# LitLeo/3m-asr-inference

Hardware: AMD Instinct MI355X
Metric: encoder frames/sec, 18Lx32e Conformer-MoE, 206-frame utterance (higher is better)
Workload: dtype f32; 1 GPU; 18-layer 32-expert fp32 (v_mfma_f32_16x16x4_f32), batch=1x206 frames per GPU, all experts local (BASELINE.json configs[1]); layers=18, experts=32, frames=206, batch_per_gpu=1, parallelism=replicas x1, streams_per_gpu=4, hip_graph=True, kernels_per_forward=263, fold_pos_proj=True, routing=balanced, route_mode=staged, packed_rows=False, fork_embed=auto

## Files before the change

3m-asr-inference_amd/csrc/api.hip:

```cpp
#include <string.h>

#include <vector>

#include "../../include/m3asr.h"
#include "common.h"
#include "kernels.h"

namespace m3 {

static thread_local char g_err[512] = "";

void set_error(const char* fmt, ...) {
  va_list ap;
  va_start(ap, fmt);
  vsnprintf(g_err, sizeof(g_err), fmt, ap);
  va_end(ap);
}
const char* last_error() { return g_err; }

struct MoeWorkspace {
  int32_t* mapping;
  int32_t* acc;
  int32_t* pos;
  float* slab;
  size_t bytes;
};
MoeWorkspace carve_moe_workspace(void* base, int S, int E, int D, int F) {
  MoeWorkspace w;
  size_t off = 0;
  char* p = (char*)base;
  w.mapping = (int32_t*)(p + off); off += align_up((size_t)S * 4, 256);
  w.acc = (int32_t*)(p + off);     off += align_up((size_t)(E + 1) * 4, 256);
  w.pos = (int32_t*)(p + off);     off += align_up((size_t)S * 4, 256);
  w.slab = (float*)(p + off);      off += align_up(expert_ffn_slab_bytes(S, D, F), 256);
  w.bytes = off;
  return w;
}

int moe_expert_ffn_dt(const float* x, const int32_t* gate_idx, const float* w1, const float* b1, const float* w2,
                      const float* b2, int S, int E, int D, int F, const float* gate_value, const float* resid,
                      float alpha, const float* ln_gamma, const float* ln_beta, float ln_eps, float* y, void* ws,
                      size_t ws_bytes, hipStream_t stream, ExpertWeights weights, const float* s1 = nullptr, const float* s2 = nullptr, float h_scale = 0.f, const void* xq = nullptr,
                      const float* xq_scale = nullptr, int ldx = 0) {
  M3_REQUIRE(S >= 0 && E > 0 && D > 0 && F > 0, "fmoe_expert: bad sizes S=%d E=%d D=%d F=%d", S, E, D, F);
  if (S == 0) return 0;
  MoeWorkspace w = carve_moe_workspace(ws, S, E, D, F);
  M3_REQUIRE(ws != nullptr && ws_bytes >= w.bytes, "fmoe_expert: workspace %zu bytes < required %zu", ws_bytes,
             w.bytes);
  int rc = launch_moe_index(gate_idx, S, E, w.mapping, w.acc, w.pos, stream);
  if (rc) return rc;
  const ExpertFfnPlan plan = plan_expert_ffn(weights, S, E, D, F);
  ExpertFfnArgs a{};
  a.x = x; a.ldx = ldx > 0 ? ldx : D; a.pos = w.pos; a.acc_hist = w.acc; a.w1 = w1; a.w2 = w2; a.s1 = s1; a.s2 = s2; a.b1 = b1;
  a.h_scale = h_scale; a.slab = w.slab; a.xq = xq; a.xq_scale = xq_scale;
  rc = launch_expert_ffn(plan, S, E, D, F, a, stream);
  if (rc) return rc;
  return launch_moe_combine(plan.rows(w.slab), plan.slices, w.mapping, gate_idx, gate_value, b2, resid, alpha, ln_gamma, ln_beta, ln_eps,
                            y, S, D, stream);
}

int moe_expert_ffn(const float* x, const int32_t* gate_idx, const float* w1, const float* b1, const float* w2,
                   const float* b2, int S, int E, int D, int F, const float* gate_value, const float* resid,
                   float alpha, const float* ln_gamma, const float* ln_beta, float ln_eps, float* y, void* ws,
                   size_t ws_bytes, hipStream_t stream) {
  return moe_expert_ffn_dt(x, gate_idx, w1, b1, w2, b2, S, E, D, F, gate_value, resid, alpha, ln_gamma, ln_beta, ln_eps,
                           y, ws, ws_bytes, stream, ExpertWeights::F32);
}

}

using namespace m3;

static bool aligned16(const void* p) { return (reinterpret_cast<uintptr_t>(p) & 15) == 0; }

extern "C" {

int m3_abi_version(void) { return M3ASR_ABI_VERSION; }
const char* m3_last_error(void) { return m3::last_error(); }

int m3_moe_scatter_mapping(const int32_t* gate_idx, int S, int num_expert, int32_t* mapping, int32_t* acc_histogram,
                           int32_t* pos, m3_stream stream) {
  M3_REQUIRE(gate_idx && mapping && acc_histogram, "moe_scatter_mapping: null pointer");
  return launch_moe_index(gate_idx, S, num_expert, mapping, acc_histogram, pos, (hipStream_t)stream);
}
int m3_moe_local_scatter(const void* x, const int32_t* mapping, int S, int row_bytes, void* out, m3_stream stream) {
  return launch_local_scatter(x, mapping, S, row_bytes, out, (hipStream_t)stream);
}
int m3_moe_local_gather(const void* buf, const int32_t* mapping, int S, int row_bytes, void* out, m3_stream stream) {
  return launch_local_gather(buf, mapping, S, row_bytes, out, (hipStream_t)stream);
}
int m3_moe_expert_slice(void) { return kExpertSlice; }
size_t m3_moe_expert_workspace_size(int S, int num_expert, int idim, int hidden_units) {
  if (S <= 0 || hidden_units % kExpertSlice) return 0;
  return carve_moe_workspace(nullptr, S, num_expert, idim, hidden_units).bytes;
}
int m3_moe_expert_ffn(const float* x, const int32_t* gate_idx, const float* w1, const float* b1, const float* w2,
                      const float* b2, int S, int num_expert, int idim, int hidden_units, const float* gate_value,
                      const float* resid, float alpha, const float* ln_gamma, const float* ln_beta, float ln_eps,
                      float* y, void* workspace, size_t workspace_bytes, m3_stream stream) {
  return moe_expert_ffn(x, gate_idx, w1, b1, w2, b2, S, num_expert, idim, hidden_units, gate_value, resid, alpha,
                        ln_gamma, ln_beta, ln_eps, y, workspace, workspace_bytes, (hipStream_t)stream);
}
int m3_moe_expert_ffn_bf16(const float* x, const int32_t* gate_idx, const void* w1, const float* b1, const void* w2,
                           const float* b2, int S, int num_expert, int idim, int hidden_units, const float* gate_value,
                           const float* resid, float alpha, const float* ln_gamma, const float* ln_beta, float ln_eps,
                           float* y, void* workspace, size_t workspace_bytes, m3_stream stream) {
  return moe_expert_ffn_dt(x, gate_idx, (const float*)w1, b1, (const float*)w2, b2, S, num_expert, idim, hidden_units,
                           gate_value, resid, alpha, ln_gamma, ln_beta, ln_eps, y, workspace, workspace_bytes,
                           (hipStream_t)stream, ExpertWeights::BF16);
}
int m3_moe_expert_ffn_fp8(const float* x, const int32_t* gate_idx, const void* w1, const float* w1_scale, const float* b1,
                          const void* w2, const float* w2_scale, const float* b2, int S, int num_expert, int idim,
                          int hidden_units, const float* gate_value, const float* resid, float alpha,
                          const float* ln_gamma, const float* ln_beta, float ln_eps, float* y, void* workspace,
                          size_t workspace_bytes, m3_stream stream) {
  M3_REQUIRE(w1_scale && w2_scale, "fmoe_expert fp8: null scale");
  return moe_expert_ffn_dt(x, gate_idx, (const float*)w1, b1, (const float*)w2, b2, S, num_expert, idim, hidden_units,
                           gate_value, resid, alpha, ln_gamma, ln_beta, ln_eps, y, workspace, workspace_bytes,
                           (hipStream_t)stream, ExpertWeights::FP8, w1_scale, w2_scale);
}
int m3_moe_expert_ffn_mxfp4_ldx(const float* x, int ldx, const int32_t* gate_idx, const void* w1, const void* w1_scale, const float* b1,
                                const void* w2, const void* w2_scale, const float* b2, int S, int num_expert, int idim,
                                int hidden_units, const float* gate_value, const float* resid, float alpha,
                                const float* ln_gamma, const float* ln_beta, float ln_eps, float* y, void* workspace,
                                size_t workspace_bytes, m3_stream stream) {
  M3_REQUIRE(x && gate_idx && w1 && w2 && b1 && y, "fmoe_expert mxfp4: null pointer");
  M3_REQUIRE(w1_scale && w2_scale, "fmoe_expert mxfp4: null scale");
  M3_REQUIRE(idim > 0 && idim % 128 == 0 && hidden_units > 0 && hidden_units % 64 == 0,
             "fmoe_expert mxfp4: idim=%d must be a multiple of 128 and hidden_units=%d of 64", idim, hidden_units);
  M3_REQUIRE(ldx >= idim && (ldx & 3) == 0, "fmoe_expert mxfp4: ldx=%d must be a multiple of 4 and at least idim=%d", ldx, idim);
  M3_REQUIRE(aligned16(x) && aligned16(w1) && aligned16(w2), "fmoe_expert mxfp4: x / w1 / w2 must be 16-byte aligned");
  return moe_expert_ffn_dt(x, gate_idx, (const float*)w1, b1, (const float*)w2, b2, S, num_expert, idim, hidden_units,
                           gate_value, resid, alpha, ln_gamma, ln_beta, ln_eps, y, workspace, workspace_bytes,
                           (hipStream_t)stream, ExpertWeights::MXFP4, (const float*)w1_scale, (const float*)w2_scale, 0.f, nullptr,
// ... 193 lines not shown
    M3_REQUIRE(!rows || d->ldy >= n_out, "linear: ldy=%d is shorter than an output row of %d", d->ldy, n_out);
    if (p.y_bf16) M3_REQUIRE(d->ldy % 4 == 0, "linear: ldy=%d must be a multiple of 4 for a bf16 y", d->ldy);
    if (d->resid) M3_REQUIRE(!rows || d->ldr >= n_out, "linear: ldr=%d is shorter than an output row of %d", d->ldr, n_out);
    if (d->y_copy_bf16) M3_REQUIRE(d->ld_copy % 4 == 0 && (!rows || d->ld_copy >= n_out), "linear: ld_copy=%d must be a multiple of 4 and >= %d", d->ld_copy, n_out);
  }
  *out = p;
  return 0;
}
static int linear_pointers(const m3_linear_desc* d) {
  M3_REQUIRE(d->a && d->w && d->y, "linear: null a / w / y");
  M3_REQUIRE(aligned16(d->a) && aligned16(d->a2) && aligned16(d->y) && aligned16(d->resid) && aligned16(d->y_copy_bf16),
             "linear: a / a2 / y / resid / y_copy_bf16 must be 16-byte aligned");
  M3_REQUIRE((const void*)d->resid != (const void*)d->y || d->ldr == d->ldy, "linear: y == resid (in-place) needs ldr=%d == ldy=%d", d->ldr, d->ldy);
  return 0;
}
const char* m3_linear_kernel(const m3_linear_desc* d, int with_workspace) {
  GemmParams p;
  if (linear_params(d, &p)) return nullptr;
  const GemmPlan plan = plan_gemm(p, with_workspace ? SIZE_MAX : 0);
  if (plan.launches == 0) set_error("%s", plan.reason);
  return plan.launches ? plan.label : nullptr;
}
int m3_linear(const m3_linear_desc* d, m3_stream stream) { return m3_linear_ws(d, nullptr, 0, stream); }
size_t m3_linear_workspace_size(const m3_linear_desc* d) {
  GemmParams p;
  return linear_params(d, &p) == 0 ? plan_gemm(p, SIZE_MAX).ws_bytes : 0;
}
int m3_linear_ws(const m3_linear_desc* d, void* workspace, size_t workspace_bytes, m3_stream stream) {
  GemmParams p;
  if (int rc = linear_params(d, &p)) return rc;
  if (int rc = linear_pointers(d)) return rc;
  return launch_gemm(gemm_launch(p, (float*)workspace, workspace_bytes), (hipStream_t)stream);
}

int m3_layer_norm(const float* x, const float* gamma, const float* beta, float eps, float* y, int rows, int dim,
                  m3_stream stream) {
  return launch_layernorm(x, gamma, beta, eps, y, rows, dim, (hipStream_t)stream);
}
int m3_relpos_attention(const float* qkv, int ldq, const float* p, int ldp, const float* pos_u, const float* pos_v,
                        const int32_t* len, int B, int T, int H, int dk, float scale, float* out, int ldo,
                        m3_stream stream) {
  return attention_single(qkv, ldq, p, ldp, pos_u, pos_v, len, B, T, H, dk, scale, 0, -1, out, ldo, 0, stream);
}
int m3_relpos_attention_bf16(const void* qkv, int ldq, const float* p, int ldp, const float* pos_u, const float* pos_v,
                             const int32_t* len, int B, int T, int H, int dk, float scale, int chunk, int left_chunks,
                             void* out, int ldo, m3_stream stream) {
  return attention_single(qkv, ldq, p, ldp, pos_u, pos_v, len, B, T, H, dk, scale, chunk, left_chunks, out, ldo, 1, stream);
}
int m3_relpos_attention_chunk(const float* qkv, int ldq, const float* p, int ldp, const float* pos_u, const float* pos_v,
                              const int32_t* len, int B, int T, int H, int dk, float scale, int chunk, int left_chunks,
                              float* out, int ldo, m3_stream stream) {
  return attention_single(qkv, ldq, p, ldp, pos_u, pos_v, len, B, T, H, dk, scale, chunk, left_chunks, out, ldo, 0, stream);
}
static int dwconv_args_from_desc(const m3_dwconv_desc* d, const char* who, const char* zname, int pair, bool strict, DwArgs* q) {
  if (pair >= 0) M3_REQUIRE(d->B > 0 && d->T > 0 && d->D > 0 && d->K > 0, "%s: empty problem %d", who, pair);
  const bool ln_ok = strict ? (d->gamma == nullptr) == (d->beta == nullptr) : (d->gamma == nullptr || d->beta != nullptr);
  M3_REQUIRE((pair < 0 && (d->B <= 0 || d->T <= 0)) || (d->z && d->w_kc && d->bias && d->out && ln_ok),
             "%s: null %s / w_kc / bias / out, or gamma without beta", who, zname);
  M3_REQUIRE(!strict || (aligned16(d->z) && aligned16(d->w_kc) && aligned16(d->bias) && aligned16(d->gamma) && aligned16(d->beta) &&
                          aligned16(d->left_fill) && aligned16(d->out)), "%s: every operand must be 16-byte aligned", who);
  if (pair >= 0) {
    M3_REQUIRE(d->ldz >= 0 && (d->ldz > 0 || !d->gate_sigmoided), "%s: ldz=%d (sigmoided gate columns belong to the GLU-on-load form)", who, d->ldz);
    M3_REQUIRE(d->left_fill == nullptr || d->K >= 2, "%s: the causal conv needs K >= 2", who);
  }
  q->z = d->z; q->glu_ldz = d->ldz; q->glu_sig = d->gate_sigmoided != 0; q->w_kc = d->w_kc; q->bias = d->bias; q->gamma = d->gamma;
  q->beta = d->beta; q->eps = d->eps; q->causal_left_fill = d->left_fill; q->B = d->B; q->T = d->T; q->D = d->D; q->K = d->K; q->out = d->out;
// ... 170 lines not shown
    M3_REQUIRE(plans[i]->launches > 0, "%s", plans[i]->reason);
    M3_REQUIRE(plans[i]->kernel == GemmKernel::SplitKF32, "%s: problem %d is no split-K problem with its workspace (it runs %s)", who, i, plans[i]->label);
  }
  M3_REQUIRE(pa.conv == pb.conv, "%s: an implicit conv pairs with an implicit conv, a plain problem with a plain one", who);
  return 0;
}
static int splitk_pair_launch(const char* who, const GemmLaunch& a, const void* out_a, size_t out_bytes_a, const GemmLaunch& b, const void* out_b,
                              size_t out_bytes_b, int which, m3_stream stream) {
  M3_REQUIRE(which >= 1 && which <= 3, "%s: which=%d (1 the GEMM launch, 2 the reduce launch, 3 both)", who, which);
  if (int rc = splitk_pair_plans(who, a.plan, b.plan)) return rc;
  M3_REQUIRE(!ranges_overlap(a.ws, a.plan.ws_bytes, b.ws, b.plan.ws_bytes), "%s: each problem needs its own workspace", who);
  M3_REQUIRE(!ranges_overlap(out_a, out_bytes_a, out_b, out_bytes_b), "%s: the two outputs overlap", who);
  return launch_gemm_f32_splitk_dual(a, b, (hipStream_t)stream, which);
}
const char* m3_linear_pair_kernel(const m3_linear_desc* a, const m3_linear_desc* b, int with_workspace) {
  GemmParams pa, pb;
  if (linear_params(a, &pa) || linear_params(b, &pb)) return nullptr;
  const size_t ws = with_workspace ? SIZE_MAX : 0;
  const GemmLaunch qa{pa, plan_gemm(pa, ws)}, qb{pb, plan_gemm(pb, ws)};
  if (with_workspace) return splitk_pair_plans("linear pair (workspaces)", qa.plan, qb.plan) ? nullptr : "gemm_f32_splitk_dual_kernel";
  return linear_pair_plans(qa, qb) ? nullptr : "gemm_f32_dual_kernel";
}
int m3_linear_pair(const m3_linear_desc* a, const m3_linear_desc* b, m3_stream stream) {
  GemmParams pa, pb;
  if (int rc = linear_params(a, &pa)) return rc;
  if (int rc = linear_params(b, &pb)) return rc;
  if (int rc = linear_pointers(a)) return rc;
  if (int rc = linear_pointers(b)) return rc;
  const GemmLaunch qa = gemm_launch(pa, nullptr, 0), qb = gemm_launch(pb, nullptr, 0);
  if (int rc = linear_pair_plans(qa, qb)) return rc;
  M3_REQUIRE(!ranges_overlap(a->y, linear_out_bytes(a), b->y, linear_out_bytes(b)), "linear pair: the two outputs overlap");
  return launch_gemm_f32_dual(qa, qb, (hipStream_t)stream);
}
int m3_linear_ws_pair(const m3_linear_desc* a, void* workspace_a, size_t bytes_a, const m3_linear_desc* b, void* workspace_b,
                      size_t bytes_b, int which, m3_stream stream) {
  GemmParams pa, pb;
  if (int rc = linear_params(a, &pa)) return rc;
  if (int rc = linear_params(b, &pb)) return rc;
  if (int rc = linear_pointers(a)) return rc;
  if (int rc = linear_pointers(b)) return rc;
  return splitk_pair_launch("linear pair (workspaces)", gemm_launch(pa, (float*)workspace_a, bytes_a), a->y, linear_out_bytes(a),
                            gemm_launch(pb, (float*)workspace_b, bytes_b), b->y, linear_out_bytes(b), which, stream);
}
int m3_conv2d_3x3s2_ws_pair(const m3_conv2d_desc* a, void* workspace_a, size_t bytes_a, const m3_conv2d_desc* b, void* workspace_b,
                            size_t bytes_b, int which, m3_stream stream) {
  M3_REQUIRE(a != nullptr && b != nullptr, "conv2d pair: null descriptor");
  GemmParams pa, pb;
  if (int rc = conv2d_params(a->in, a->w, a->bias, a->B, a->T1, a->F1, a->C, a->act, a->out, &pa)) return rc;
  if (int rc = conv2d_params(b->in, b->w, b->bias, b->B, b->T1, b->F1, b->C, b->act, b->out, &pb)) return rc;
  M3_REQUIRE(a->in && a->w && a->out && b->in && b->w && b->out, "conv2d pair: null in / w / out");
  return splitk_pair_launch("conv2d pair", gemm_launch(pa, (float*)workspace_a, bytes_a), a->out, rows_bytes(pa.M, pa.ldy, pa.N),
                            gemm_launch(pb, (float*)workspace_b, bytes_b), b->out, rows_bytes(pb.M, pb.ldy, pb.N), which, stream);
}
int m3_relpos_attention_pair(const m3_attention_desc* a, const m3_attention_desc* b, m3_stream stream) {
  M3_REQUIRE(a != nullptr && b != nullptr, "attention pair: null descriptor");
  AttArgs qa, qb;
  if (int rc = attention_args_from_desc(a, "attention pair", 0, &qa)) return rc;
  if (int rc = attention_args_from_desc(b, "attention pair", 1, &qb)) return rc;
  M3_REQUIRE(relpos_attention_dual_fusable(qa, qb),
             "attention pair: head widths %d / %d (64 or 128 each) or row strides ldq %d / %d, ldp %d / %d (multiples of 4) are not a paired instantiation",
             a->dk, b->dk, a->ldq, b->ldq, a->ldp, b->ldp);
  M3_REQUIRE(!ranges_overlap(a->out, rows_bytes((long)a->B * a->T, a->ldo, a->H * a->dk), b->out, rows_bytes((long)b->B * b->T, b->ldo, b->H * b->dk)),
             "attention pair: the two outputs overlap");
  return launch_relpos_attention_dual(qa, qb, (hipStream_t)stream);
}
int m3_dwconv_ln_silu_pair(const m3_dwconv_desc* a, const m3_dwconv_desc* b, m3_stream stream) {
// ... 345 lines not shown
```

3m-asr-inference_amd/csrc/engine.hip:

```cpp
#include <assert.h>
#include <math.h>
#include <stdlib.h>
#include <string.h>

#include <functional>
#include <memory>
#include <string>
#include <unordered_map>
#include <variant>
#include <vector>

#include "../../include/m3asr.h"
#include "common.h"
#include "kernels.h"

namespace m3 {
struct MoeWorkspace {
  int32_t* mapping; int32_t* acc; int32_t* pos; float* slab; size_t bytes;
};
MoeWorkspace carve_moe_workspace(void* base, int S, int E, int D, int F);
}

using namespace m3;

namespace {

struct Norm { const float* g = nullptr; const float* b = nullptr; };
struct Lin { const float* w = nullptr; const float* b = nullptr; const float* wsum = nullptr; const float* wbeta = nullptr; };

struct BlockW {
  Norm n_ffm, n_mha, n_conv, n_ff, n_final, n_cnn;
  Lin mac1, mac2, qkv, pos, out, pw1, pw2, ff1, ff2;
  const float* pos_u = nullptr; const float* pos_v = nullptr;
  const float* dw_w = nullptr; const float* dw_b = nullptr;
  const float* left_fill = nullptr;
  Lin router;
  Lin router_x;
  const float *ew1 = nullptr, *eb1 = nullptr, *ew2 = nullptr, *eb2 = nullptr;
  const float *es1 = nullptr, *es2 = nullptr;
  float h_scale = 0.f;
};

struct SubW { const float* c1w; const float* c1b; const float* c2w; const float* c2b; Lin out; int in_ch = 1; };

using Launch = std::variant<std::monostate, GemmLaunch, Conv1Args, DwArgs, AttArgs>;

struct Stage {
  std::string name;
  std::function<int(hipStream_t)> run;
  m3_stage_info info;
  bool reads_embed = false;
  Launch launch;
  bool pairable = false;
  bool router_prefix = false;
  std::function<int(hipStream_t)> refresh_prefix;
};
const GemmLaunch& gemm_of(const Stage& st) { return std::get<GemmLaunch>(st.launch); }
bool is_splitk(const Stage& st) { return std::holds_alternative<GemmLaunch>(st.launch) && gemm_of(st).plan.kernel == GemmKernel::SplitKF32; }

m3_stage_info stage_info(const char* kernel, int launches, double bytes, double flops, bool per_row = true) {
  m3_stage_info i;
  i.kernel = kernel; i.launches = launches; i.per_row = per_row ? 1 : 0; i.alg_bytes = bytes; i.flops = flops;
  return i;
}

struct Buf { void* ptr; size_t bytes; };

struct BindKey {
  int B = 0, T = 0;
  const float* feat = nullptr; const int32_t* feat_len = nullptr; float* logits = nullptr;
  void* ws = nullptr; size_t ws_bytes = 0;
// ... 36 lines not shown
    std::shared_ptr<float> pfold;
    std::vector<Stage> stages;
    std::unordered_map<std::string, Buf> buffers;
    int n_kernels = 0;
    hipGraphExec_t graph_exec = nullptr;
    bool graph_valid = false;
    uint64_t last_use = 0;
    bool matches(const BindKey& k) const { return !stages.empty() && key == k; }
  };
  Bound cur;
  std::vector<Bound> parked;
  uint64_t use_clock = 0;
  int n_captures = 0;
  int ep_capacity = 0;
  hipStream_t side = nullptr;
  hipEvent_t ev_fork = nullptr, ev_join = nullptr;
  std::unordered_map<int, std::weak_ptr<float>> pfold_by_tp;
};

namespace {

struct Switches {
  int gate_index_max_rows;
  bool self_route;
  bool hfuse;
  int router_min_rows;
  bool router_xq;
  bool router_skip_xn;
  bool fused8_adapt;
  bool glu_defer;
  bool front_pair;
  bool router_prefix;
  bool glu_sig_epi;
};
const Switches& switches() {
  static const Switches sw = [] {
    auto num = [](const char* name, int dflt) { const char* v = getenv(name); return v ? atoi(v) : dflt; };
    Switches w;
    w.gate_index_max_rows = num("M3_GATE_INDEX_MAX_ROWS", 512);
    w.self_route = num("M3_SELF_ROUTE", 1) != 0;
    w.hfuse = num("M3_HFUSE", 1) != 0;
    w.router_min_rows = num("M3_ROUTER_MIN_ROWS", 2048);
    w.router_xq = num("M3_ROUTER_XQ", 1) != 0;
    w.router_skip_xn = num("M3_ROUTER_SKIP_XN", 0) != 0;
    w.fused8_adapt = num("M3_FUSED8_ADAPT", 0) != 0;
    w.glu_defer = num("M3_GLU_DEFER", 1) != 0;
    w.front_pair = num("M3_FRONT_PAIR", 1) != 0;
    w.router_prefix = num("M3_ROUTER_PREFIX", 1) != 0;
    w.glu_sig_epi = num("M3_GLU_SIG_EPI", 1) != 0;
    return w;
  }();
  return sw;
}

bool lookup(const m3_engine* e, const std::string& name, int64_t numel, const float** out, int dtype = M3_F32) {
  auto it = e->table.find(name);
  if (it == e->table.end()) {
    set_error("engine: weight '%s' missing from the plan", name.c_str());
    return false;
  }
  if (numel >= 0 && it->second.numel != numel) {
    set_error("engine: weight '%s' has %lld elements, expected %lld", name.c_str(), (long long)it->second.numel,
              (long long)numel);
    return false;
  }
  if (it->second.dtype != dtype) {
    set_error("engine: weight '%s' has dtype %d, the engine (weight_dtype=%d) expects %d", name.c_str(),
              (int)it->second.dtype, (int)e->cfg.weight_dtype, dtype);
    return false;
  }
  *out = (const float*)it->second.data;
  return true;
}

#define GET(dst, name, numel) \
  do { if (!lookup(e, (name), (numel), &(dst))) return false; } while (0)
#define GETW(dst, name, numel) \
  do { if (!lookup(e, (name), (numel), &(dst), e->cfg.weight_dtype == M3_F32 ? M3_F32 : M3_BF16)) return false; } while (0)
#define GETE(dst, name, numel) \
  do { if (!lookup(e, (name), (numel), &(dst), e->cfg.weight_dtype)) return false; } while (0)

bool load_norm(const m3_engine* e, const std::string& p, int d, Norm* n) {
  GET(n->g, p + "weight", d);
  GET(n->b, p + "bias", d);
  return true;
}
bool load_lin(const m3_engine* e, const std::string& p, int64_t n_out, int64_t n_in, bool bias, Lin* l) {
  GETW(l->w, p + "weight", n_out * n_in);
  if (bias) GET(l->b, p + "bias", n_out);
  return true;
}
bool load_lin_ln(const m3_engine* e, const std::string& p, int64_t n_out, int64_t n_in, bool wbeta, Lin* l,
                 bool fp32_only = false) {
  if (fp32_only) {
    GET(l->w, p + "ln.weight", n_out * n_in);
  } else {
    GETW(l->w, p + "ln.weight", n_out * n_in);
  }
  GET(l->b, p + "ln.bias", n_out);
  GET(l->wsum, p + "ln.wsum", n_out);
  if (wbeta) GET(l->wbeta, p + "ln.wbeta", n_out);
  return true;
}

bool load_block(const m3_engine* e, const std::string& p, int D, int F, int K, bool cnn_ln, bool moe, int De, BlockW* b, bool causal) {
  const m3_engine_config& c = e->cfg;
  if (!load_norm(e, p + "norm_final.", D, &b->n_final)) return false;
  if (moe && !load_norm(e, p + "norm_ff.", D, &b->n_ff)) return false;
  if (!load_lin_ln(e, p + "feed_forward_macaron.w_1.", F, D, false, &b->mac1) ||
      !load_lin(e, p + "feed_forward_macaron.w_2.", D, F, true, &b->mac2) ||
      !load_lin_ln(e, p + "self_attn.qkv.", 3 * D, D, false, &b->qkv) ||
      !load_lin(e, p + "self_attn.linear_out.", D, D, true, &b->out) ||
      !load_lin_ln(e, p + "conv_module.pointwise_conv1.", 2 * D, D, true, &b->pw1) ||
      !load_lin(e, p + "conv_module.pointwise_conv2.", D, D, true, &b->pw2))
    return false;
  GET(b->pos_u, p + "self_attn.pos_bias_u", D);
  GET(b->pos_v, p + "self_attn.pos_bias_v", D);
  GET(b->dw_w, p + "conv_module.depthwise_conv.weight_kc", (int64_t)K * D);
  GET(b->dw_b, p + "conv_module.depthwise_conv.bias", D);
  if (cnn_ln && !load_norm(e, p + "conv_module.norm.", D, &b->n_cnn)) return false;
  if (causal) GET(b->left_fill, p + "conv_module.left_fill", D);
  if (!moe) {
    if (!load_lin_ln(e, p + "feed_forward.w_1.", F, D, false, &b->ff1) ||
        !load_lin(e, p + "feed_forward.w_2.", D, F, true, &b->ff2))
      return false;
  } else {
    const int world = c.ep_world_size > 0 ? c.ep_world_size : 1;
    const int64_t Etot = (int64_t)c.num_experts * world;
    GET(b->router.w, p + "feed_forward.router_weights_t", Etot * (D + De));
    if (c.router_with_bias) GET(b->router.b, p + "feed_forward.router_bias", Etot);
    if (c.fuse_route && !load_lin_ln(e, p + "feed_forward.router_x.", Etot, D, false, &b->router_x, true)) return false;
    const int64_t E = c.num_experts;
    const int64_t ew_numel = c.weight_dtype == M3_MXFP4 ? E * F * D / 2 : E * F * D;
    GETE(b->ew1, p + "feed_forward.experts.w_1.weight", ew_numel);
    if (c.weight_dtype == M3_MXFP4) {
      GETE(b->es1, p + "feed_forward.experts.w_1.scale", E * F * D / 32);
      GETE(b->es2, p + "feed_forward.experts.w_2.scale", E * F * D / 32);
    }
    if (c.weight_dtype == M3_FP8) {
      GET(b->es1, p + "feed_forward.experts.w_1.scale", E * F);
      GET(b->es2, p + "feed_forward.experts.w_2.scale", E * D);
      if (c.fp8_activations) {
        const float* hs = nullptr;
        GET(hs, p + "feed_forward.experts.h_scale", 1);
        if (hipMemcpy(&b->h_scale, hs, sizeof(float), hipMemcpyDeviceToHost) != hipSuccess || !(b->h_scale > 0.f)) {
          set_error("engine: '%sfeed_forward.experts.h_scale' must hold one positive number", p.c_str());
          return false;
        }
      }
    }
    GET(b->eb1, p + "feed_forward.experts.w_1.bias", E * F);
    GETE(b->ew2, p + "feed_forward.experts.w_2.weight_sliced", ew_numel);
    GET(b->eb2, p + "feed_forward.experts.w_2.bias", E * D);
  }
  return true;
}

inline int sub_fc(int idim, int in_ch) { return idim / in_ch; }
inline int sub_f1(int fc) { return (fc - 3) / 2 + 1; }
inline int sub_f2(int fc) { return (sub_f1(fc) - 3) / 2 + 1; }

bool load_sub(const m3_engine* e, const std::string& p, int D, int idim, SubW* s) {
  auto it = e->table.find(p + "conv.0.weight_9c");
  const int64_t numel = it == e->table.end() ? 9 * (int64_t)D : it->second.numel;
  s->in_ch = (int)(numel / (9 * (int64_t)D));
  if (numel % (9 * (int64_t)D) || s->in_ch < 1 || s->in_ch > 3) {
    set_error("engine: '%sconv.0.weight_9c' has %lld elements: 9 * in_ch * %d with 1 to 3 input channels expected", p.c_str(), (long long)numel, D);
    return false;
  }
  if (idim % s->in_ch || sub_fc(idim, s->in_ch) < 7) {
    set_error("engine: '%sconv.0.weight_9c' has %d input channels: input_dim=%d must be a multiple of it with at least 7 bins per channel",
              p.c_str(), s->in_ch, idim);
    return false;
  }
  const int F2 = sub_f2(sub_fc(idim, s->in_ch));
  GET(s->c1w, p + "conv.0.weight_9c", 9 * (int64_t)s->in_ch * D);
  GET(s->c1b, p + "conv.0.bias", D);
  GETW(s->c2w, p + "conv.2.weight_ohwi", 9 * (int64_t)D * D);
  GET(s->c2b, p + "conv.2.bias", D);
  return load_lin(e, p + "out.0.", D, (int64_t)D * F2, true, &s->out);
}
#undef GET
#undef GETW
#undef GETE

inline int sub_len(int t) { return ((t - 3) / 2 + 1 - 3) / 2 + 1; }
// ... 265 lines not shown
  const float *tail_ln_g = nullptr, *tail_ln_b = nullptr; float tail_ln_eps = 0.f; float* tail_ln_out = nullptr;
  float* splitk_ws = nullptr; size_t splitk_bytes = 0;
};

}

static void add_stage(StageBuilder& sb, const std::string& name, int kernels, std::function<int(hipStream_t)> fn,
                      m3_stage_info info = stage_info("", 0, 0.0, 0.0)) {
  info.launches = kernels;
  sb.bd.stages.push_back(Stage{name, std::move(fn), info});
  sb.bd.n_kernels += kernels;
}

static m3_stage_info gemm_info(const GemmParams& p, const GemmPlan& plan) {
  const bool glu = p.act == ACT_GLU;
  const double M = p.M, N = p.N, K = p.K, Nout = glu ? N / 2 : N;
  const double wsz = p.w_bf16 ? 2 : 4, asz = p.a_bf16 ? 2 : 4, ysz = p.y_bf16 ? 2 : 4;
  double a_bytes = M * K * asz;
  if (p.mode == GEMM_A_CONV3X3S2)
    a_bytes = (double)(p.M / (p.conv_T2 * p.conv_F2)) * p.conv_T1 * p.conv_F1 * p.conv_C * asz;
  double bytes = N * K * wsz + a_bytes + M * Nout * ysz;
  if (p.resid) bytes += M * Nout * 4;
  if (p.Yb) bytes += M * Nout * 2;
  if (p.ln_out) bytes += M * (K - p.K1) * 4;
  return stage_info(plan.label, 1, bytes, 2.0 * M * N * K, p.mode != GEMM_A_CONV3X3S2);
}

static void add_launch(StageBuilder& sb, const std::string& name, Launch record, const m3_stage_info& info, bool pairable = false) {
  add_stage(sb, name, info.launches, nullptr, info);
  sb.bd.stages.back().launch = std::move(record);
  sb.bd.stages.back().pairable = pairable;
}

static void add_gemm(StageBuilder& sb, const std::string& name, GemmParams p, bool fp32_weights = false) {
  p.w_bf16 = (!fp32_weights && sb.eng.cfg.weight_dtype != M3_F32) ? 1 : 0;
  const GemmLaunch g = gemm_launch(p, sb.splitk_ws, sb.splitk_bytes);
  m3_stage_info info = gemm_info(p, g.plan);
  info.launches = g.plan.launches ? g.plan.launches : 1;
  add_launch(sb, name, g, info, g.plan.launches == 1);
}

static bool stages_fusable(const Stage& a, const Stage& b) {
  if (!a.pairable || !b.pairable || a.launch.index() != b.launch.index()) return false;
  if (std::holds_alternative<GemmLaunch>(a.launch))
    return is_splitk(a) ? gemm_splitk_dual_fusable(gemm_of(a), gemm_of(b)) : gemm_dual_fusable(gemm_of(a), gemm_of(b));
  if (auto* d = std::get_if<DwArgs>(&a.launch)) return dwconv_dual_fusable(*d, std::get<DwArgs>(b.launch));
  if (auto* t = std::get_if<AttArgs>(&a.launch)) return relpos_attention_dual_fusable(*t, std::get<AttArgs>(b.launch));
  return conv1_dual_fusable(std::get<Conv1Args>(a.launch), std::get<Conv1Args>(b.launch));
}
static Stage fused_stage(const Stage& a, const Stage& b, bool reduce_half = false) {
  Stage d;
  d.name = reduce_half ? a.name + ".reduce+" + b.name + ".reduce" : a.name + "+" + b.name;
  const char* label = "";
  std::visit([&](const auto& pa) {
    using R = std::decay_t<decltype(pa)>;
    if constexpr (std::is_same_v<R, GemmLaunch>) {
      const GemmLaunch& pb = gemm_of(b);
      if (is_splitk(a)) {
        d.run = [pa, pb, which = reduce_half ? 2 : 1](hipStream_t s) { return launch_gemm_f32_splitk_dual(pa, pb, s, which); };
        label = "gemm_f32_splitk_dual_kernel";
      } else {
        d.run = [pa, pb](hipStream_t s) { return launch_gemm_f32_dual(pa, pb, s); };
        label = "gemm_f32_dual_kernel";
      }
    } else if constexpr (std::is_same_v<R, Conv1Args>) {
      d.run = [pa, pb = std::get<R>(b.launch)](hipStream_t s) { return launch_conv1_relu_dual(pa, pb, s); };
      label = "conv1_relu_dual_kernel";
    } else if constexpr (std::is_same_v<R, DwArgs>) {
      d.run = [pa, pb = std::get<R>(b.launch)](hipStream_t s) { return launch_dwconv_ln_silu_dual(pa, pb, s); };
// ... 154 lines not shown
      const GemmPlan plan = gemm_of(st).plan;
      float* prefix = pl.rprefix; const int layer = m.layer;
      st.refresh_prefix = [plan, g, prefix, layer](hipStream_t s) {
        const float* wt[kRouterPrefixMaxLayers] = {};
        wt[layer] = g.W;
        return launch_router_embed_prefix(plan, g, wt, layer, 1, prefix, s);
      };
    }
  }
  sb.bd.stages.back().reads_embed = true;
}

static void add_moe_gate_index(StageBuilder& sb, const MoeLayer& m, int32_t* map, int32_t* acc, int32_t* pos) {
  add_stage(sb, m.pfx + "moe_gate_index", 1, [=](hipStream_t s) {
    return launch_moe_gate_index(m.rl, m.Etot, m.live_len, m.live_rpb, m.S, m.gidx, m.gval, map, acc, pos, s);
  }, stage_info("moe_index_kernel", 1, (double)m.S * (m.Etot * 4 + 16) + 4.0 * (m.Etot + 1), 0.0));
}

static void add_moe_top1(StageBuilder& sb, const MoeLayer& m) {
  add_stage(sb, m.pfx + "moe_top1", 1, [m](hipStream_t s) {
    return launch_softmax_top1(m.rl, m.Etot, m.live_len, m.live_rpb, m.S, m.Etot, m.gidx, m.gval, s);
  }, stage_info("softmax_top1_kernel", 1, (double)m.S * (m.Etot * 4 + 8), 0.0));
}

static void add_moe_local_index(StageBuilder& sb, const MoeLayer& m) {
  add_stage(sb, m.pfx + "moe_local.index", 1, [m](hipStream_t s) {
    return launch_moe_index(m.gidx, m.S, m.E, m.mw.mapping, m.mw.acc, m.mw.pos, s);
  }, stage_info("moe_index_kernel", 1, 12.0 * m.S + 4.0 * (m.E + 1), 0.0));
}

static ExpertFfnArgs expert_args(const BlockW& w, const float* x, const MoeWorkspace& mw, int D) {
  ExpertFfnArgs a{};
  a.x = x; a.ldx = D; a.pos = mw.pos; a.acc_hist = mw.acc; a.w1 = w.ew1; a.w2 = w.ew2; a.s1 = w.es1; a.s2 = w.es2; a.b1 = w.eb1;
  a.w2_sliced = 1; a.h_scale = w.h_scale; a.slab = mw.slab;
  return a;
}

static void add_moe_local_expert(StageBuilder& sb, const MoeLayer& m, const MoeRoute& r, const ExpertFfnPlan& f, const Plan& pl) {
  const bool norm = r.norm_in_expert();
  const float* xin = norm ? m.x : m.xn;
  const bool self_route = r.gate == GateForm::InExpert;
  const void* xq = r.use_xq ? pl.xq : nullptr; const float* xqs = r.use_xq ? pl.xq_scale : nullptr;
  int32_t* fs = r.fs_dev ? pl.moe_fs : nullptr;
  add_stage(sb, m.pfx + "moe_local.expert", f.launches, [=](hipStream_t s) {
    const BlockW& w = *m.w;
    const float* ln_g = norm ? w.n_ff.g : nullptr; const float* ln_b = norm ? w.n_ff.b : nullptr; const float ln_eps = norm ? m.eps : 0.f;
    if (self_route)
      return launch_expert_route_ffn_f32(xin, m.D, m.rl, m.live_len, m.live_rpb, m.S, m.E, m.D, m.F, w.ew1, w.eb1, w.ew2, 1, w.eb2,
                                         m.mw.slab, m.gidx, m.gval, m.mw.mapping, m.mw.acc, m.mw.pos, s, ln_g, ln_b, ln_eps);
    ExpertFfnArgs a = expert_args(w, xin, m.mw, m.D);
    a.ln_gamma = ln_g; a.ln_beta = ln_b; a.ln_eps = ln_eps; a.xq = xq; a.xq_scale = xqs; a.fs_dev = fs;
    return launch_expert_ffn(f, m.S, m.E, m.D, m.F, a, s);
  }, stage_info(f.label, 1, -1.0, 4.0 * m.D * m.F * m.S));
}

static void add_moe_local_combine(StageBuilder& sb, const MoeLayer& m, const MoeRoute& r, const ExpertFfnPlan& f, const Plan& pl) {
  const bool self_route = r.gate == GateForm::InExpert;
  const int32_t* cmap = self_route ? nullptr : m.mw.mapping;
  const float* cb2 = self_route ? nullptr : m.w->eb2;
  const int32_t* fs = r.fs_dev ? pl.moe_fs : nullptr;
  const double S = m.S, D = m.D;
  add_stage(sb, m.pfx + "moe_local.combine", 1, [=](hipStream_t s) {
    const BlockW& w = *m.w;
    return launch_moe_combine(f.rows(m.mw.slab), fs ? kExpertFusedFp8MaxSplit : f.slices, cmap, m.gidx, m.gv, cb2, m.x, 0.5f, w.n_final.g, w.n_final.b, m.eps, m.x,
                              m.S, m.D, s, m.xb_out, m.xstats_out, fs);
  }, stage_info("moe_combine_kernel", 1, S * D * 4 * (f.slices + 2) + (m.xb_out ? 2.0 * S * D : 0.0), S * D * (f.slices + 10)));
}

static void add_moe_ep(StageBuilder& sb, const MoeLayer& m, const MoeRoute& r, const Plan& pl) {
  const int S = m.S, E = m.E, Etot = m.Etot, D = m.D, F = m.F, world = m.world;
  const int cap = pl.ep_cap, R = pl.ep_rows;
  int32_t *g_acc = pl.ep_acc, *g_map = pl.ep_mapping, *g_pos = pl.ep_pos, *map_send = pl.ep_map_send, *gate_recv = pl.ep_gate_recv;
  int32_t* ep_overflow = pl.ep_overflow;
  float *wire_a = pl.wire_a, *wire_b = pl.wire_b;
  const MoeWorkspace rw = carve_moe_workspace(m.ws, R, E, D, F);
  if (r.gate == GateForm::GateIndex) add_moe_gate_index(sb, m, g_map, g_acc, g_pos);
  if (r.gate == GateForm::Top1Index) add_moe_top1(sb, m);
  const bool one_launch = r.gate == GateForm::GateIndex;
  const int32_t* gidx = m.gidx; const float* xn = m.xn;
  add_stage(sb, m.pfx + "moe_ep.send", one_launch ? 1 : 2, [=](hipStream_t s) {
    if (!one_launch)
      if (int rc = launch_moe_index(gidx, S, Etot, g_map, g_acc, g_pos, s)) return rc;
    return launch_ep_send_rows(gidx, g_map, g_acc, S, world, E, cap, map_send, xn, wire_a, D * 4, s, ep_overflow);
  }, stage_info("ep_send_rows_kernel", 1, (double)S * D * 8 + 24.0 * S, 0.0));
  auto exchange = [=, &sb](const char* name) {
    if (world == 1) add_stage(sb, m.pfx + name, 0, [=](hipStream_t s) {
      M3_CHECK_HIP(hipMemcpyAsync(wire_b, wire_a, (size_t)R * D * 4, hipMemcpyDeviceToDevice, s));
      return 0;
    });
  };
  exchange("moe_ep.exchange1");
  const ExpertFfnPlan f = plan_expert_ffn(expert_weights(sb.eng.cfg, *m.w), R, E, D, F, EXPERT_SCATTER_ROWS);
  const bool scatter2 = f.kernel == ExpertKernel::TiledBf16;
  const BlockW* wp = m.w;
  add_stage(sb, m.pfx + "moe_ep.expert", (scatter2 ? 2 : 3) + f.launches, [=](hipStream_t s) {
    const BlockW& w = *wp;
    if (int rc = launch_ep_recv_gate(wire_b, world, E, cap, D * 4, gate_recv, s)) return rc;
    if (int rc = launch_moe_index(gate_recv, R, E, rw.mapping, rw.acc, rw.pos, s)) return rc;
    ExpertFfnArgs a = expert_args(w, wire_b, rw, D);
    if (scatter2) { a.b2 = w.eb2; a.y_scatter = wire_a; }
    if (int rc = launch_expert_ffn(f, R, E, D, F, a, s)) return rc;
    if (scatter2) return 0;
    return launch_moe_combine(f.rows(rw.slab), f.slices, rw.mapping, gate_recv, nullptr, w.eb2, nullptr, 1.f, nullptr, nullptr, 0.f, wire_a, R, D, s);
  }, stage_info(f.label, 1, -1.0, 4.0 * D * F * S));
  exchange("moe_ep.exchange2");
  add_stage(sb, m.pfx + "moe_ep.combine", 1, [=](hipStream_t s) {
    const BlockW& w = *wp;
    return launch_moe_combine(wire_b, 1, map_send, nullptr, m.gv, nullptr, m.x, 0.5f, w.n_final.g, w.n_final.b, m.eps, m.x, S, D, s,
                              m.xb_out, m.xstats_out);
  }, stage_info("moe_combine_kernel", 1, (double)S * D * 12 + (m.xb_out ? 2.0 * S * D : 0.0), (double)S * D * 11));
  sb.bd.buffers["ep.wire_a"] = Buf{wire_a, (size_t)R * D * 4};
  sb.bd.buffers["ep.wire_b"] = Buf{wire_b, (size_t)R * D * 4};
}

static void build_block(StageBuilder& sb, const std::string& pfx, const BlockW& w, int D, int F, int H, int K, bool cnn_ln,
                        bool moe, int layer, int tap_index, const Plan& pl, bool causal) {
  auto add_gemm = [&](StageBuilder&, const std::string& name, GemmParams g, bool fp32_weights = false) {
    if (sb.bd.packed) g.m_dev = pl.row0 + sb.bd.key.B;
    ::add_gemm(sb, name, g, fp32_weights);
  };
  const m3_engine_config& c = sb.eng.cfg;
  const BindKey& key = sb.bd.key;
  const int B = key.B, Tp = sb.bd.Tp, S = sb.bd.S;
  const bool streaming = key.sstate != nullptr;
  const int32_t* step = key.s_slots ? sb.st.slot_pos : sb.st.step;
  const int slot_chunks = key.s_slots ? key.s_maxf / Tp : -1;
  float* x = pl.x;
  const int32_t* lens = pl.lens;
  const float eps = 1e-12f;

  const bool a16 = sb.bd.a16;
  void* xb = pl.xb;
  const bool dma = sb.bd.dma;
  float* xstats = pl.xstats;
  auto from_xb = [&](GemmParams& g) {
    if (a16) { g.A = (const float*)xb; g.a_bf16 = 1; }
    if (dma) { g.ln_stats = xstats; g.ln_stat_parts = kXbStatParts; }
  };
  auto also_xb = [&](GemmParams& g) {
    if (a16) { g.Yb = xb; g.ldyb = D; }
    if (dma) g.Yb_stats = xstats;
  };
  const bool packed = sb.bd.packed;
  const int32_t* row0 = packed ? pl.row0 : nullptr;
  const int32_t* pad_of = packed ? pl.pad_of : nullptr;
  const int32_t* pdev = packed ? pl.row0 + B : nullptr;
  const int32_t* live_len = packed ? pdev : lens;
  const int live_rpb = packed ? S : Tp;
  {
    GemmParams g;
    g.A = x; g.lda = D; g.W = w.mac1.w; g.bias = w.mac1.b; g.Y = pl.h1; g.ldy = F; g.M = S; g.N = F; g.K = D;
    g.ln_wsum = w.mac1.wsum; g.ln_eps = eps; g.act = ACT_SILU;
    from_xb(g); g.y_bf16 = a16;
    add_gemm(sb, pfx + "ffn_macaron.w1", g);
    GemmParams h;
    h.A = pl.h1; h.lda = F; h.W = w.mac2.w; h.bias = w.mac2.b; h.Y = x; h.ldy = D; h.M = S; h.N = D; h.K = F;
    h.alpha = 0.5f; h.resid = x; h.ldr = D;
    h.a_bf16 = a16; also_xb(h);
    add_gemm(sb, pfx + "ffn_macaron.w2", h);
  }
  {
    GemmParams g;
    g.A = x; g.lda = D; g.W = w.qkv.w; g.bias = w.qkv.b; g.Y = pl.qkv; g.ldy = 3 * D; g.M = S; g.N = 3 * D; g.K = D;
    g.ln_wsum = w.qkv.wsum; g.ln_eps = eps;
    from_xb(g);
    const bool att16 = a16 && relpos_attention_bf16_supports(Tp, D / H);
    g.y_bf16 = att16;
    add_gemm(sb, pfx + "att.qkv", g);
    const int ldp = (c.num_blocks + c.embed_blocks) * D;
    const float* pmat = pl.pbuf + (size_t)tap_index * D;
    const float* qkv = pl.qkv; float* ctx = pl.ctx;
    const float* pu = w.pos_u; const float* pv = w.pos_v;
    const int dk = D / H;
    const float scale = 1.f / sqrtf((float)dk);
    const int chunk = c.static_chunk_size, left_chunks = c.num_left_chunks;
    AttArgs aa;
    aa.qkv = qkv; aa.ldq = 3 * D; aa.pmat = pmat; aa.ldp = ldp; aa.pos_u = pu; aa.pos_v = pv; aa.row_len = lens; aa.B = B; aa.T = Tp; aa.H = H;
    aa.dk = dk; aa.scale = scale; aa.out = ctx; aa.ldo = D; aa.left_chunks = left_chunks;
    const char* label = att16 ? "relpos_attention_bf16_kernel" : "relpos_attention_kernel";
    double row_bytes = att16 ? 8 : (12 + (a16 ? 2 : 4));
    if (streaming) {
      aa.streaming = 1; aa.hist = sb.st.kv[tap_index]; aa.cap = key.s_hist; aa.step = step; aa.slot_max_chunks = slot_chunks;
      label = "relpos_attention_stream_kernel"; row_bytes = 24;
    } else {
      aa.rows_bf16 = att16; aa.out_bf16 = a16; aa.row0 = row0; aa.chunk = chunk;
    }
    add_launch(sb, pfx + "att.core", aa, stage_info(label, 1, (double)S * D * row_bytes + (double)Tp * D * 4, 6.0 * Tp * D * S), !streaming && !att16);
    GemmParams o;
    o.A = pl.ctx; o.lda = D; o.W = w.out.w; o.bias = w.out.b; o.Y = x; o.ldy = D; o.M = S; o.N = D; o.K = D;
    o.resid = x; o.ldr = D;
    o.a_bf16 = a16; also_xb(o);
    add_gemm(sb, pfx + "att.out", o);
  }
  {
    GemmParams g;
    g.A = x; g.lda = D; g.W = w.pw1.w; g.bias = w.pw1.b; g.Y = pl.glu; g.ldy = D; g.M = S; g.N = 2 * D; g.K = D;
    g.ln_wsum = w.pw1.wsum; g.ln_wbeta = w.pw1.wbeta; g.ln_eps = eps; g.act = ACT_GLU;
    g.row_len = live_len; g.rows_per_batch = live_rpb; g.mask_in = 1;
    from_xb(g);
    bool glu_deferred = false;
    if (switches().glu_defer && c.weight_dtype == M3_F32 && !a16 && !causal && !streaming &&
        dwconv_glu_in_supports(D, K, false, 0, 2 * D)) {
      GemmParams r = g;
      r.act = ACT_NONE; r.ldy = 2 * D;
      const GemmPlan rp = plan_gemm(r, 0);
      if (rp.launches == 1 && rp.kernel == GemmKernel::SkinnyF32 && rp.mt == 1) { g = r; glu_deferred = true; }
    }
    const bool glu_sig = glu_deferred && switches().glu_sig_epi && (D & 15) == 0;
    if (glu_sig) g.sig_col0 = D;
    add_gemm(sb, pfx + "conv.pw1_glu", g);
    const float* glu = pl.glu; float* dw = pl.dw;
    const float* dww = w.dw_w; const float* dwb = w.dw_b;
    const float* ng = cnn_ln ? w.n_cnn.g : nullptr; const float* nb = cnn_ln ? w.n_cnn.b : nullptr;
    const float* lfill = causal ? w.left_fill : nullptr;
    DwArgs da;
    da.z = glu; da.w_kc = dww; da.bias = dwb; da.gamma = ng; da.beta = nb; da.eps = 1e-5f; da.B = B; da.T = Tp; da.D = D; da.K = K;
    da.out = dw; da.out_bf16 = a16;
    double row_bytes = (glu_deferred ? 8 : 4) + (a16 ? 2 : 4), cache_bytes = 0.0;
    if (streaming) {
      da.streaming = 1; da.cache_pair = sb.st.conv[tap_index]; da.step = step; da.chunk_len = lens; da.slot_max_chunks = slot_chunks;
      row_bytes = 8; cache_bytes = 8.0 * B * (K - 1) * D;
    } else {
      da.pad_of = pad_of; da.row0 = row0; da.row_len = lens; da.causal_left_fill = lfill;
      da.glu_ldz = glu_deferred ? 2 * D : 0; da.glu_sig = glu_sig;
    }
    add_launch(sb, pfx + "conv.dw_ln_silu", da,
               stage_info("dwconv_ln_silu_kernel", 1, (double)S * D * row_bytes + (double)K * D * 4 + cache_bytes, 2.0 * K * D * S), !streaming);
    GemmParams h;
    h.A = pl.dw; h.lda = D; h.W = w.pw2.w; h.bias = w.pw2.b; h.Y = x; h.ldy = D; h.M = S; h.N = D; h.K = D;
    h.row_len = live_len; h.rows_per_batch = live_rpb; h.mask_out = 1; h.resid = x; h.ldr = D;
    h.a_bf16 = a16; also_xb(h);
    add_gemm(sb, pfx + "conv.pw2", h);
  }
  if (!moe) {
    GemmParams g;
    g.A = x; g.lda = D; g.W = w.ff1.w; g.bias = w.ff1.b; g.Y = pl.h1; g.ldy = F; g.M = S; g.N = F; g.K = D;
    g.ln_wsum = w.ff1.wsum; g.ln_eps = eps; g.act = ACT_SILU;
    from_xb(g); g.y_bf16 = a16;
    add_gemm(sb, pfx + "ffn.w1", g);
    GemmParams h;
    h.A = pl.h1; h.lda = F; h.W = w.ff2.w; h.bias = w.ff2.b; h.Y = x; h.ldy = D; h.M = S; h.N = D; h.K = F;
    h.alpha = 0.5f; h.resid = x; h.ldr = D;
    h.a_bf16 = a16;
    add_gemm(sb, pfx + "ffn.w2", h);
    const float* fg = w.n_final.g; const float* fb = w.n_final.b;
    void* xbo = a16 ? xb : nullptr;
    float* xso = dma ? xstats : nullptr;
    const float* g2 = sb.tail_ln_g; const float* b2 = sb.tail_ln_b; float* y2 = sb.tail_ln_out;
    const float eps2 = sb.tail_ln_eps;
    sb.tail_ln_g = nullptr;
    add_stage(sb, pfx + "norm_final", 1, [=](hipStream_t s) { return launch_layernorm(x, fg, fb, eps, x, S, D, s, xbo, xso, g2, b2, eps2, y2); },
              stage_info("layernorm_kernel", 1, (double)S * D * (a16 ? 10 : 8) + (g2 ? 4.0 * S * D : 0.0), (g2 ? 16.0 : 8.0) * S * D));
  } else {
    MoeLayer m;
    m.pfx = pfx; m.w = &w; m.S = S; m.Tp = Tp; m.D = D; m.F = F; m.De = c.embed_dim; m.E = c.num_experts;
    m.world = c.ep_world_size > 0 ? c.ep_world_size : 1; m.Etot = m.E * m.world; m.eps = eps;
    m.x = x; m.xn = pl.xn; m.rl = pl.rl;
    m.gidx = pl.gate_idx + (size_t)layer * S; m.gval = pl.gate_val + (size_t)layer * S;
    m.gv = c.keep_expert_output ? nullptr : m.gval;
    m.lens = lens; m.live_len = live_len; m.live_rpb = live_rpb; m.pdev = pdev;
    m.eall = pl.eall + (size_t)layer * m.E; m.ld_eall = c.num_blocks * m.E; m.layer = layer;
    m.xb_out = a16 ? xb : nullptr; m.xstats_out = dma ? xstats : nullptr;
    m.ws = (char*)pl.moe_ws + (c.debug_taps ? (size_t)layer * pl.moe_ws_bytes : 0);
    m.mw = carve_moe_workspace(m.ws, S, m.E, D, F);
    const MoeRoute r = choose_moe_route(c, S, w, pl);
    add_moe_router(sb, m, r, pl);
    if (r.ep) {
      add_moe_ep(sb, m, r, pl);
    } else {
      if (r.gate == GateForm::GateIndex) add_moe_gate_index(sb, m, m.mw.mapping, m.mw.acc, m.mw.pos);
      if (r.gate == GateForm::Top1Index) add_moe_top1(sb, m);
      if (r.gate == GateForm::Top1Index || r.gate == GateForm::RouterTail) add_moe_local_index(sb, m);
      const ExpertFfnPlan f = plan_expert_ffn(expert_weights(c, w), S, m.E, D, F, r.norm_in_expert() ? EXPERT_NORM_IN_KERNEL : 0);
      add_moe_local_expert(sb, m, r, f, pl);
      add_moe_local_combine(sb, m, r, f, pl);
    }
    const std::string b = pfx.substr(0, pfx.size() - 1);
// ... 600 lines not shown
```

3m-asr-inference_amd/csrc/gemm.hip:

```cpp
#include "common.h"
#include "gemm_epilogue.h"
#include "kernels.h"

#ifdef M3_GEMM_DIAG
#define M3_GDIAG(...) __VA_ARGS__
#else
#define M3_GDIAG(...)
#endif

namespace m3 {

M3_GDIAG(__device__ unsigned long long g_gemm_dbg[2048 * 8];)

enum { LN_NONE = GEMM_LN_NONE, LN_EPI = GEMM_LN_EPI, LN_PRO = GEMM_LN_PRO };

template <int MT, bool GLU, int NW, bool CONV, int LN, int NBUF, bool ACCI = false>
__device__ __forceinline__ void gemm_f32_body(const GemmParams& p, const int bid) {
  constexpr int NT = GLU ? 2 : 1;
  constexpr int G = gemm_group_steps(MT, NT, NW);
  constexpr int I0 = ACCI ? G / 2 : 0;
  static_assert(!ACCI || (MT == 1 && !GLU && !CONV && NBUF == 1 && G % 2 == 0), "acc_init: the one-group 16-row concat form only");
  constexpr int RW = (16 * MT) / NW;
  static_assert(RW >= 1, "more waves than rows");
  __shared__ float red[NW][MT * NT][256];
  __shared__ float stats[16 * MT][2];
  __shared__ float rsum[LN == LN_EPI ? NW : 1][16 * MT][2];
  __shared__ __attribute__((aligned(16))) float ln_g[LN == LN_PRO ? 1024 : 4], ln_b[LN == LN_PRO ? 1024 : 4];

  M3_GDIAG(unsigned long long dg[8]; dg[0] = __builtin_amdgcn_s_memtime();)
  asm volatile("" ::"s"(p.A), "s"(p.lda), "s"(p.W), "s"(p.bias), "s"(p.Y), "s"(p.ldy), "s"(p.M), "s"(p.N), "s"(p.K), "s"(p.mode),
               "s"(p.n_tiles), "s"(p.m_tiles), "s"(p.xcd_swizzle), "s"(p.m_dev), "s"(p.resid), "s"(p.ldr), "s"(p.act), "s"(p.alpha),
               "s"(p.mask_in), "s"(p.mask_out), "s"(p.row_len), "s"(p.rows_per_batch), "s"(p.sig_col0));
  if (ACCI) asm volatile("" ::"s"(p.acc_init));
  if (LN == LN_EPI) asm volatile("" ::"s"(p.ln_wsum), "s"(p.ln_wbeta), "s"(p.ln_eps));
  if (LN == LN_PRO) asm volatile("" ::"s"(p.ln_gamma), "s"(p.ln_beta), "s"(p.ln_eps), "s"(p.ln_out), "s"(p.ld_ln_out), "s"(p.ln_on_a2));
  if (!CONV) asm volatile("" ::"s"(p.A2), "s"(p.lda2), "s"(p.K1));
  if (CONV) asm volatile("" ::"s"(p.conv_T1), "s"(p.conv_F1), "s"(p.conv_T2), "s"(p.conv_F2), "s"(p.conv_C));
  const int lane = threadIdx.x & 63, wave = threadIdx.x >> 6;
  const int col = lane & 15, kq = lane >> 4;
  const int Nout = GLU ? (p.N >> 1) : p.N;

  int n_tile, m_tile;
  {
    const int id = bid;
    if (p.xcd_swizzle) {
      const int j = id >> 3;
      m_tile = j % p.m_tiles;
      n_tile = (j / p.m_tiles) * 8 + (id & 7);
    } else {
      n_tile = id % p.n_tiles;
      m_tile = id / p.n_tiles;
    }
  }
  const int n0 = n_tile * 16;
  const int m0 = m_tile * (16 * MT);
  if (p.m_dev != nullptr && m0 > *p.m_dev) return;
  const int ln_k0 = p.ln_on_a2 ? p.K1 : 0;
  const int Kl = p.K - ln_k0;

  const float* arow[MT];
  const float* arow2[MT];
#pragma unroll
  for (int mt = 0; mt < MT; ++mt) {
    const int m = min(m0 + 16 * mt + col, p.M - 1);
    arow2[mt] = nullptr;
    if (CONV) {
      const int f2 = m % p.conv_F2;
      const int t2 = (m / p.conv_F2) % p.conv_T2;
      const int b = m / (p.conv_F2 * p.conv_T2);
      arow[mt] = p.A + ((size_t)(b * p.conv_T1 + 2 * t2) * p.conv_F1 + 2 * f2) * p.conv_C + 4 * kq;
    } else {
      arow[mt] = p.A + (size_t)m * p.lda + 4 * kq;
      if (p.mode == GEMM_A_CONCAT2) arow2[mt] = p.A2 + (size_t)m * p.lda2 + 4 * kq;
    }
  }
  const float* wrow[NT];
#pragma unroll
  for (int t = 0; t < NT; ++t)
    wrow[t] = p.W + (size_t)min(n0 + t * Nout + col, p.N - 1) * p.K + 4 * kq;

  f32x4 acc[MT][NT];
#pragma unroll
  for (int mt = 0; mt < MT; ++mt)
#pragma unroll
    for (int t = 0; t < NT; ++t) acc[mt][t] = f32x4{0.f, 0.f, 0.f, 0.f};
  constexpr bool DUAL = MT * NT <= 2;
  f32x4 acc2[MT][NT];
#pragma unroll
  for (int mt = 0; mt < MT; ++mt)
#pragma unroll
    for (int t = 0; t < NT; ++t) acc2[mt][t] = f32x4{0.f, 0.f, 0.f, 0.f};
  float s1[MT], s2[MT];
#pragma unroll
  for (int mt = 0; mt < MT; ++mt) s1[mt] = s2[mt] = 0.f;

  const int nsteps = p.K >> 4;
  auto a_offset = [&](int k) -> int {
    if (CONV) {
      const int seg = k / p.conv_C, c = k - seg * p.conv_C;
      const int kh = seg / 3, kw = seg - kh * 3;
      return (kh * p.conv_F1 + kw) * p.conv_C + c;
    }
    return k;
  };

  f32x4 wbuf[NBUF][G][NT], abuf[NBUF][G][MT];
  auto load_group = [&](int g, int buf) {
#pragma unroll
    for (int i = I0; i < G; ++i) {
      const int s = min(wave + NW * (G * g + i), nsteps - 1);
      const int k = s << 4;
#pragma unroll
      for (int t = 0; t < NT; ++t) wbuf[buf][i][t] = ldg4_w(wrow[t] + k);
      const bool second = ACCI || (!CONV && p.mode == GEMM_A_CONCAT2 && k >= p.K1);
      const int off = second ? (k - p.K1) : a_offset(k);
#pragma unroll
      for (int mt = 0; mt < MT; ++mt) abuf[buf][i][mt] = ldg4((second ? arow2[mt] : arow[mt]) + off);
    }
  };

  const int ngroups = (nsteps + NW * G - 1) / (NW * G);
  M3_GDIAG(dg[1] = __builtin_amdgcn_s_memtime();)
  f32x4 ln_v[16];
  auto load_stat_rows = [&](int c) {
    const int l16 = lane & 15;
    const int rloc = wave * RW + 4 * c + (lane >> 4);
    const int m = min(m0 + min(rloc, 16 * MT - 1), p.M - 1);
    const float* row = (p.ln_on_a2 ? p.A2 : p.A) + (size_t)m * (p.ln_on_a2 ? p.lda2 : p.lda);
#pragma unroll
    for (int j = 0; j < 8; ++j) ln_v[j] = ldg4(row + min(4 * (l16 + 16 * j), Kl - 4));
    if (Kl > 512) {
#pragma unroll
      for (int j = 8; j < 16; ++j) ln_v[j] = ldg4(row + min(4 * (l16 + 16 * j), Kl - 4));
    } else {
#pragma unroll
      for (int j = 8; j < 16; ++j) ln_v[j] = f32x4{0.f, 0.f, 0.f, 0.f};
    }
  };
  if (LN == LN_PRO && ACCI) load_stat_rows(0);
  load_group(0, 0);
  if (ACCI) {
    const float* pre = p.acc_init + ((size_t)((m_tile * p.n_tiles + n_tile) * NW + wave) * 2) * 256 + 4 * lane;
    acc[0][0] = ldg4(pre);
    acc2[0][0] = ldg4(pre + 256);
  }
  M3_GDIAG(dg[2] = __builtin_amdgcn_s_memtime();)
// ... 196 lines not shown
        const int row = 16 * mt + 4 * kq + r;
        const int m = m0 + row;
        if (m >= p.M) continue;
        float y0 = v[0][r], y1 = v[NT - 1][r];
        const bool pad = pad4[r];
        if (LN != LN_EPI && p.mask_in && pad) y0 = y1 = 0.f;
        float mean = 0.f, rstd = 1.f;
        if (LN == LN_EPI) {
          float t1 = 0.f, t2 = 0.f;
#pragma unroll
          for (int w = 0; w < NW; ++w) {
            t1 += rsum[w][row][0];
            t2 += rsum[w][row][1];
          }
          ln_mean_rstd(t1, t2, Kl, p.ln_eps, mean, rstd);
        }
        float y = gemm_epilogue<GLU, LN == LN_EPI>(y0, y1, bias0, bias1, wsum0, wsum1, wbeta0, wbeta1, mean, rstd, pad, res[r], p);
        if (!GLU && p.sig_col0 >= 0 && n0 >= p.sig_col0) y = sigmoidf(y);
        p.Y[(size_t)m * p.ldy + ep_n] = y;
      }
    }
  }
  M3_GDIAG(dg[6] = __builtin_amdgcn_s_memtime();
           asm volatile("s_waitcnt vmcnt(0)" ::: "memory");
           dg[7] = __builtin_amdgcn_s_memtime();
           if (lane == 0 && wave == 0 && bid < 2048) {
             unsigned long long* o = g_gemm_dbg + (size_t)bid * 8;
             for (int i = 0; i < 8; ++i) o[i] = dg[i];
             const unsigned hw = __builtin_amdgcn_s_getreg((31 << 11) | 4), xcc = __builtin_amdgcn_s_getreg((31 << 11) | 20);
             o[7] = (dg[7] & 0xffffffffffull) | ((unsigned long long)(hw & 0xffff) << 40) | ((unsigned long long)(xcc & 0xf) << 56);
           })
}

template <int MT, bool GLU, int NW, bool CONV, int LN, int NBUF, bool ACCI = false>
__global__ __launch_bounds__(64 * NW) void gemm_f32_kernel(const GemmParams p) {
  gemm_f32_body<MT, GLU, NW, CONV, LN, NBUF, ACCI>(p, (int)blockIdx.x);
}

struct RouterPrefixArgs {
  const float* A; int lda; int M, N, K;
  int n_tiles, m_tiles, xcd_swizzle;
  const int32_t* m_dev;
  float* prefix; long layer_floats; int layer0;
  const float* w[kRouterPrefixMaxLayers];
};
template <int NW>
__global__ __launch_bounds__(64 * NW) void router_embed_prefix_kernel(const RouterPrefixArgs a) {
  constexpr int H = gemm_group_steps(1, 1, NW) / 2;
  asm volatile("" ::"s"(a.A), "s"(a.lda), "s"(a.M), "s"(a.N), "s"(a.K), "s"(a.n_tiles), "s"(a.m_tiles), "s"(a.xcd_swizzle), "s"(a.m_dev),
               "s"(a.prefix), "s"(a.layer_floats), "s"(a.layer0));
  const int lane = threadIdx.x & 63, wave = threadIdx.x >> 6;
  const int col = lane & 15, kq = lane >> 4;
  const int layer = a.layer0 + (int)blockIdx.y;
  int n_tile, m_tile;
  {
    const int id = (int)blockIdx.x;
    if (a.xcd_swizzle) {
      const int j = id >> 3;
      m_tile = j % a.m_tiles;
      n_tile = (j / a.m_tiles) * 8 + (id & 7);
    } else {
      n_tile = id % a.n_tiles;
      m_tile = id / a.n_tiles;
    }
  }
  const int n0 = n_tile * 16, m0 = m_tile * 16;
  if (a.m_dev != nullptr && m0 > *a.m_dev) return;
  const float* arow = a.A + (size_t)min(m0 + col, a.M - 1) * a.lda + 4 * kq;
  const float* wrow = a.w[layer] + (size_t)min(n0 + col, a.N - 1) * a.K + 4 * kq;
// ... 5 lines not shown
    ab[i] = ldg4(arow + k);
  }
  f32x4 acc = f32x4{0.f, 0.f, 0.f, 0.f}, acc2 = f32x4{0.f, 0.f, 0.f, 0.f};
#pragma unroll
  for (int i = 0; i < H; ++i)
#pragma unroll
    for (int j = 0; j < 4; j += 2) {
      acc = mfma16(ab[i][j], wb[i][j], acc);
      acc2 = mfma16(ab[i][j + 1], wb[i][j + 1], acc2);
    }
  float* o = a.prefix + (size_t)layer * a.layer_floats + ((size_t)((m_tile * a.n_tiles + n_tile) * NW + wave) * 2) * 256 + 4 * lane;
  stg4(o, acc);
  stg4(o + 256, acc2);
}

size_t router_prefix_floats(const GemmPlan& plan) { return (size_t)plan.m_tiles * plan.n_tiles * plan.nw * 2 * 256; }

int launch_router_embed_prefix(const GemmPlan& plan, const GemmParams& p, const float* const* w, int layer0, int n_layers, float* prefix,
                               hipStream_t stream) {
  M3_REQUIRE(plan.launches == 1 && plan.kernel == GemmKernel::SkinnyF32 && p.acc_init != nullptr && (plan.nw == 4 || plan.nw == 8),
             "router prefix: the consumer's plan does not take an accumulator prefix");
  M3_REQUIRE(layer0 >= 0 && n_layers > 0 && layer0 + n_layers <= kRouterPrefixMaxLayers && prefix != nullptr, "router prefix: bad layer range");
  RouterPrefixArgs a;
  a.A = p.A; a.lda = p.lda; a.M = p.M; a.N = p.N; a.K = p.K;
  a.n_tiles = plan.n_tiles; a.m_tiles = plan.m_tiles; a.xcd_swizzle = plan.xcd_swizzle;
  a.m_dev = p.m_dev; a.prefix = prefix; a.layer_floats = (long)router_prefix_floats(plan); a.layer0 = layer0;
  for (int l = 0; l < kRouterPrefixMaxLayers; ++l) a.w[l] = (l >= layer0 && l < layer0 + n_layers) ? w[l] : nullptr;
  const dim3 grid(plan.n_tiles * plan.m_tiles, n_layers);
  if (plan.nw == 8) hipLaunchKernelGGL((router_embed_prefix_kernel<8>), grid, dim3(512), 0, stream, a);
  else hipLaunchKernelGGL((router_embed_prefix_kernel<4>), grid, dim3(256), 0, stream, a);
  M3_LAUNCH_CHECK();
  return 0;
}
template <int MT, bool GLU, int NW, int LN>
__global__ __launch_bounds__(64 * NW) void gemm_f32_dual_kernel(const GemmParams p0, const GemmParams p1, const int n0) {
  if ((int)blockIdx.x < n0) {
    if ((int)blockIdx.x < p0.n_tiles * p0.m_tiles) gemm_f32_body<MT, GLU, NW, false, LN, 1>(p0, (int)blockIdx.x);
  } else {
    gemm_f32_body<MT, GLU, NW, false, LN, 1>(p1, (int)blockIdx.x - n0);
  }
}

int launch_gemm_f32_dual(const GemmLaunch& a, const GemmLaunch& b, hipStream_t stream) {
  M3_REQUIRE(gemm_dual_fusable(a, b), "gemm dual: the two problems do not share an instantiation");
  GemmParams q[2] = {a.p, b.p};
  const GemmPlan& pa = a.plan;
  const GemmPlan* const plans[2] = {&a.plan, &b.plan};
  for (int i = 0; i < 2; ++i) {
    q[i].n_tiles = plans[i]->n_tiles; q[i].m_tiles = plans[i]->m_tiles; q[i].xcd_swizzle = plans[i]->xcd_swizzle;
  }
  const int n0 = (int)align_up((size_t)q[0].n_tiles * q[0].m_tiles, 8);
  dim3 grid(n0 + q[1].n_tiles * q[1].m_tiles);
#define M3_DUAL(GLU_, NW_, LN_)                                                                                             \
  hipLaunchKernelGGL((gemm_f32_dual_kernel<1, GLU_, NW_, LN_>), grid, dim3(64 * NW_), 0, stream, q[0], q[1], n0)
  if (pa.glu) {
    if (pa.nw == 8) { if (pa.ln == LN_EPI) M3_DUAL(true, 8, LN_EPI); else M3_DUAL(true, 8, LN_NONE); }
    else { if (pa.ln == LN_EPI) M3_DUAL(true, 4, LN_EPI); else M3_DUAL(true, 4, LN_NONE); }
  } else {
    if (pa.nw == 8) { if (pa.ln == LN_EPI) M3_DUAL(false, 8, LN_EPI); else M3_DUAL(false, 8, LN_NONE); }
    else { if (pa.ln == LN_EPI) M3_DUAL(false, 4, LN_EPI); else M3_DUAL(false, 4, LN_NONE); }
  }
#undef M3_DUAL
  M3_LAUNCH_CHECK();
  return 0;
}

int launch_gemm_f32_skinny(const GemmPlan& plan, const GemmParams& pin, hipStream_t stream) {
  GemmParams p = pin;
  p.n_tiles = plan.n_tiles; p.m_tiles = plan.m_tiles; p.xcd_swizzle = plan.xcd_swizzle;
  dim3 grid(p.n_tiles * p.m_tiles);
  const int mt = plan.mt, nw = plan.nw, ln = plan.ln;
  if (p.acc_init != nullptr) {
    if (nw == 8) hipLaunchKernelGGL((gemm_f32_kernel<1, false, 8, false, LN_PRO, 1, true>), grid, dim3(512), 0, stream, p);
    else hipLaunchKernelGGL((gemm_f32_kernel<1, false, 4, false, LN_PRO, 1, true>), grid, dim3(256), 0, stream, p);
    M3_LAUNCH_CHECK();
    return 0;
  }

#define M3_GEMM_LAUNCH(MT_, GLU_, NW_, CONV_, LN_)                                                              \
  do {                                                                                                          \
    if (plan.nbuf == 1)                                                                                         \
      hipLaunchKernelGGL((gemm_f32_kernel<MT_, GLU_, NW_, CONV_, LN_, 1>), grid, dim3(64 * NW_), 0, stream, p); \
    else                                                                                                        \
      hipLaunchKernelGGL((gemm_f32_kernel<MT_, GLU_, NW_, CONV_, LN_, 2>), grid, dim3(64 * NW_), 0, stream, p); \
  } while (0)
#define M3_GEMM_MT(GLU_, NW_, CONV_, LN_)                                                              \
  do {                                                                                                 \
    if (mt == 1) M3_GEMM_LAUNCH(1, GLU_, NW_, CONV_, LN_);                                             \
    else if (mt == 2) M3_GEMM_LAUNCH(2, GLU_, NW_, CONV_, LN_);                                        \
    else M3_GEMM_LAUNCH(4, GLU_, NW_, CONV_, LN_);                                                     \
  } while (0)
#define M3_GEMM_LN(GLU_, NW_)                                                                          \
  do {                                                                                                 \
    if (ln == LN_EPI) M3_GEMM_MT(GLU_, NW_, false, LN_EPI);                                            \
    else if (ln == LN_PRO) M3_GEMM_MT(GLU_, NW_, false, LN_PRO);                                       \
    else M3_GEMM_MT(GLU_, NW_, false, LN_NONE);                                                        \
  } while (0)
  if (plan.conv) {
    if (nw == 16) M3_GEMM_MT(false, 16, true, LN_NONE); else if (nw == 8) M3_GEMM_MT(false, 8, true, LN_NONE);
    else M3_GEMM_MT(false, 4, true, LN_NONE);
  } else if (nw == 16) {
    M3_GEMM_MT(false, 16, false, LN_NONE);
  } else if (plan.glu) {
    if (nw == 8) M3_GEMM_LN(true, 8); else M3_GEMM_LN(true, 4);
  } else {
    if (nw == 8) M3_GEMM_LN(false, 8); else M3_GEMM_LN(false, 4);
  }
#undef M3_GEMM_LN
#undef M3_GEMM_MT
#undef M3_GEMM_LAUNCH
  M3_LAUNCH_CHECK();
  return 0;
}

// ... 8 lines not shown
```

3m-asr-inference_amd/csrc/gemm_plan.hip:

```cpp
#include <stdlib.h>

#include "common.h"
#include "kernels.h"

namespace m3 {

static int env_int(const char* name, int dflt) {
  const char* e = getenv(name);
  return e ? atoi(e) : dflt;
}

#define M3_PLAN_REQUIRE(cond, ...)                                  \
  do {                                                              \
    if (!(cond)) {                                                  \
      snprintf(plan.reason, sizeof(plan.reason), __VA_ARGS__);      \
      return false;                                                 \
    }                                                               \
  } while (0)

static bool operands_ok(const GemmParams& p, const char* who, GemmPlan& plan) {
  const int kmult = p.w_bf16 ? 32 : 16;
  M3_PLAN_REQUIRE(p.grp_acc == nullptr, "%s: grouped (per-expert) operands belong to the expert FFN's plan", who);
  M3_PLAN_REQUIRE(p.M > 0 && p.N > 0 && p.K > 0, "%s: empty problem M=%d N=%d K=%d", who, p.M, p.N, p.K);
  M3_PLAN_REQUIRE(p.K % kmult == 0, "%s: K=%d must be a multiple of %d", who, p.K, kmult);
// ... 99 lines not shown
  if (plan.ln != GEMM_LN_NONE) {
    M3_PLAN_REQUIRE(p.mode == GEMM_A_PLAIN || (concat && p.ln_on_a2), "%s: LayerNorm needs plain A (or the A2 half of a concat)", who);
    M3_PLAN_REQUIRE((p.ln_on_a2 ? p.K - p.K1 : p.K) <= 1024, "%s: LayerNorm supports rows up to 1024 wide", who);
    M3_PLAN_REQUIRE(p.K <= 2047, "%s: LayerNorm variants are built for K < 2048", who);
  }
  M3_PLAN_REQUIRE(!p.ln_on_a2 || concat, "%s: ln_on_a2 needs concat mode", who);
  M3_PLAN_REQUIRE(p.ln_out == nullptr || plan.ln == GEMM_LN_PRO, "%s: ln_out needs the affine LayerNorm prologue", who);
  if (long_batch && (p.K & 63) == 0 && (!conv || (p.conv_C & 63) == 0)) {
    plan.kernel = GemmKernel::TiledF32; plan.label = "gemm_f32_tiled_kernel";
    if (big) tiled_grid(p, plan, 128, 128, 32); else tiled_grid(p, plan, 64, 64, 64);
    return true;
  }
  plan.kernel = GemmKernel::SkinnyF32; plan.label = "gemm_f32_kernel";
  skinny_grid(p, plan, Nout);
  plan.dual_ok = plan.mt == 1 && (plan.nw == 4 || plan.nw == 8) && plan.nbuf == 1 && p.mode == GEMM_A_PLAIN &&
                 plan.ln != GEMM_LN_PRO && p.m_dev == nullptr && p.acc_init == nullptr;
  return true;
}

static bool extras_ok(const GemmParams& p, GemmPlan& plan) {
  if (p.sig_col0 >= 0) {
    M3_PLAN_REQUIRE(plan.kernel == GemmKernel::SkinnyF32 && !plan.glu, "gemm: sig_col0 needs the skinny fp32 kernel with a plain epilogue (M=%d N=%d K=%d)",
                    p.M, p.N, p.K);
    M3_PLAN_REQUIRE((p.sig_col0 & 15) == 0, "gemm: sig_col0=%d must be a multiple of 16", p.sig_col0);
  }
  if (p.acc_init != nullptr) {
    M3_PLAN_REQUIRE(plan.kernel == GemmKernel::SkinnyF32 && plan.mt == 1 && !plan.glu && p.mode == GEMM_A_CONCAT2 && (p.K1 & 15) == 0,
                    "gemm: acc_init needs the skinny fp32 kernel, 16-row tiles, concat operands with K1 %% 16 == 0");
    M3_PLAN_REQUIRE(plan.ln == GEMM_LN_PRO && p.ln_on_a2 && (plan.nw == 4 || plan.nw == 8) && plan.nbuf == 1 && 2 * p.K1 == p.K &&
                    p.K == 16 * plan.nw * gemm_group_steps(1, 1, plan.nw),
                    "gemm: acc_init is built for K1 = K / 2 = %d with the LayerNorm prologue on the A2 half (K1=%d K=%d)",
                    8 * plan.nw * gemm_group_steps(1, 1, plan.nw), p.K1, p.K);
  }
  return true;
}

GemmPlan plan_gemm(const GemmParams& p, size_t workspace_bytes_available) {
  GemmPlan plan{};
  plan.kernel = p.w_bf16 ? GemmKernel::SkinnyBf16 : GemmKernel::SkinnyF32;
  plan.label = "";
  plan.glu = p.act == ACT_GLU; plan.conv = p.mode == GEMM_A_CONV3X3S2;
  plan.ln = p.ln_wsum ? GEMM_LN_EPI : (p.ln_gamma ? GEMM_LN_PRO : GEMM_LN_NONE);
  if (operands_ok(p, p.w_bf16 ? "gemm_bf16w" : "gemm", plan) && choose_form(p, workspace_bytes_available, plan) && extras_ok(p, plan))
    plan.launches = plan.kernel == GemmKernel::SplitKF32 ? 2 : 1;
  return plan;
}

GemmLaunch gemm_launch(const GemmParams& p, float* ws, size_t ws_bytes) { return GemmLaunch{p, plan_gemm(p, ws != nullptr ? ws_bytes : 0), ws}; }
bool gemm_dual_fusable(const GemmLaunch& ga, const GemmLaunch& gb) {
  const GemmPlan &a = ga.plan, &b = gb.plan;
  return a.launches == 1 && b.launches == 1 && a.dual_ok && b.dual_ok && a.nw == b.nw && a.ln == b.ln && a.glu == b.glu;
}

int launch_gemm(const GemmLaunch& g, hipStream_t stream) {
  const GemmPlan& plan = g.plan; const GemmParams& p = g.p; float* const ws = g.ws;
  M3_REQUIRE(plan.launches > 0, "%s", plan.reason);
  switch (plan.kernel) {
    case GemmKernel::SkinnyF32: return launch_gemm_f32_skinny(plan, p, stream);
    case GemmKernel::SkinnyBf16: return launch_gemm_bf16w_skinny(plan, p, stream);
    case GemmKernel::TiledF32: return launch_gemm_f32_tiled(plan, p, stream);
    case GemmKernel::TiledBf16: return launch_gemm_bf16w_tiled(plan, p, stream);
    case GemmKernel::DmaBf16: return launch_gemm_bf16_dma(plan, p, stream);
    case GemmKernel::SplitKF32:
      M3_REQUIRE(ws != nullptr, "gemm split-K: the plan was made for a workspace of %zu bytes, none given", plan.ws_bytes);
      return launch_gemm_f32_splitk(plan, p, ws, stream);
  }
  return -2;
}

}
```

3m-asr-inference_amd/csrc/kernels.h:

```cpp
#pragma once
#include <hip/hip_runtime.h>
#include <stdint.h>

#include "../../include/m3asr.h"

namespace m3 {

enum { ACT_NONE = 0, ACT_RELU = 1, ACT_SILU = 2, ACT_GLU = 3 };
enum { GEMM_A_PLAIN = 0, GEMM_A_CONCAT2 = 1, GEMM_A_CONV3X3S2 = 2 };

struct GemmParams {
  const float* A = nullptr; int lda = 0;
  const float* A2 = nullptr; int lda2 = 0; int K1 = 0;
  const float* W = nullptr;
  int w_bf16 = 0;
  const float* bias = nullptr;
  float* Y = nullptr; int ldy = 0;
  int M = 0, N = 0, K = 0;
  int mode = GEMM_A_PLAIN;
  const float* ln_gamma = nullptr; const float* ln_beta = nullptr; float ln_eps = 0.f;
  const float* ln_wsum = nullptr; const float* ln_wbeta = nullptr;
  int ln_on_a2 = 0;
  float* ln_out = nullptr; int ld_ln_out = 0;
  const int32_t* row_len = nullptr; int rows_per_batch = 0;
  int mask_in = 0, mask_out = 0;
  int conv_T1 = 0, conv_F1 = 0, conv_T2 = 0, conv_F2 = 0, conv_C = 0;
  int act = ACT_NONE;
  float alpha = 1.f;
  const float* resid = nullptr; int ldr = 0;
  const int32_t* grp_acc = nullptr; int grp_E = 0; const int32_t* grp_pos = nullptr; int w_sliced = 0;
  const float* w_scale = nullptr;
  int a_bf16 = 0, y_bf16 = 0; void* Yb = nullptr; int ldyb = 0;
  float* Yb_stats = nullptr; const float* ln_stats = nullptr; int ln_stat_parts = 0;
  const int32_t* m_dev = nullptr;
  const int32_t* y_rows = nullptr;
  const int32_t* conv_len = nullptr;
  int sig_col0 = -1;
  const float* acc_init = nullptr;
  int n_tiles = 0, m_tiles = 0, xcd_swizzle = 0;
};
enum { GEMM_LN_NONE = 0, GEMM_LN_EPI = 1, GEMM_LN_PRO = 2 };
enum class GemmKernel { SkinnyF32, SkinnyBf16, TiledF32, TiledBf16, DmaBf16, SplitKF32 };
struct GemmPlan {
  GemmKernel kernel;
  const char* label;
  int launches;
  bool glu, conv; int ln;
  int mt, nw, nbuf;
  bool dual_ok;
  int bm, bn, bk;
  int stages;
  int m_tiles, n_tiles, xcd_swizzle;
  int splits; size_t ws_bytes;
  char reason[192];
};
GemmPlan plan_gemm(const GemmParams& p, size_t workspace_bytes_available);
struct GemmLaunch { GemmParams p; GemmPlan plan; float* ws = nullptr; };
GemmLaunch gemm_launch(const GemmParams& p, float* ws, size_t ws_bytes);
int launch_gemm(const GemmLaunch& g, hipStream_t stream);
bool gemm_dual_fusable(const GemmLaunch& a, const GemmLaunch& b);
int launch_gemm_f32_dual(const GemmLaunch& a, const GemmLaunch& b, hipStream_t stream);
constexpr int kRouterPrefixMaxLayers = 64;
size_t router_prefix_floats(const GemmPlan& plan);
int launch_router_embed_prefix(const GemmPlan& plan, const GemmParams& p, const float* const* w, int layer0, int n_layers, float* prefix,
                               hipStream_t stream);
constexpr int gemm_group_steps(int MT, int NT, int NW) {
  if (NW == 16) return MT == 1 ? (NT == 1 ? 4 : 2) : (MT == 2 ? 2 : 1);
  if (NW == 8) return MT == 1 ? 8 : (MT == 2 ? (NT == 1 ? 6 : 4) : (NT == 1 ? 3 : 2));
  return MT == 1 ? 8 : (MT == 2 ? 6 : 4);
}
constexpr int gemm16_group_steps(int MT, int NW) { return NW == 16 ? 2 : (MT == 4 ? 2 : 4); }
// ... 27 lines not shown
int launch_moe_router(const float* emb, int lde, int De, const float* x, int ldx, int D, const float* W, const float* bias,
                      const float* gamma, const float* beta, float eps, float* xn, int ldxn, float* Y, int ldy, int M, int N,
                      const int32_t* m_dev, hipStream_t stream, int32_t* gate_idx = nullptr, float* gate_val = nullptr,
                      const int32_t* row_len = nullptr, int rows_per_batch = 0, void* xq = nullptr, float* xq_scale = nullptr);
int launch_local_scatter(const void* x, const int32_t* mapping, int S, int row_bytes, void* out, hipStream_t stream);
int launch_local_gather(const void* buf, const int32_t* mapping, int S, int row_bytes, void* out, hipStream_t stream);

int launch_ep_send_map(const int32_t* gate_idx, const int32_t* mapping, const int32_t* acc_hist, int S, int world, int e_loc,
                       int capacity, int32_t* map_send, void* wire, int row_bytes, hipStream_t stream, int32_t* overflow = nullptr);
int launch_ep_send_rows(const int32_t* gate_idx, const int32_t* mapping, const int32_t* acc_hist, int S, int world, int e_loc,
                        int capacity, int32_t* map_send, const void* x, void* wire, int row_bytes, hipStream_t stream, int32_t* overflow = nullptr);
int launch_ep_recv_gate(const void* wire, int world, int e_loc, int capacity, int row_bytes, int32_t* gate_recv,
                        hipStream_t stream);

#ifndef M3_EXPERT_SLICE
#define M3_EXPERT_SLICE 64
#endif
constexpr int kExpertSliceW16 = 64;
constexpr int kExpertSlice = M3_EXPERT_SLICE;
size_t expert_ffn_slab_bytes(int S, int D, int F);
enum class ExpertWeights { F32, BF16, FP8, FP8A8, MXFP4 };
enum class ExpertKernel { SlabF32, TiledF32, SlabBf16, TiledBf16, G256Bf16, SlabW8, TiledW8, FusedFp8, SlabW4, TiledW4 };
struct ExpertFfnPlan {
  ExpertWeights weights; ExpertKernel kernel;
  const char* label;
  int launches, slices;
  int fsplit;
  size_t h_off, rows_off, xb_off;
  float* rows(float* slab) const { return (float*)((char*)slab + rows_off); }
};
enum { EXPERT_NORM_IN_KERNEL = 1,
       EXPERT_SCATTER_ROWS = 2 };
ExpertFfnPlan plan_expert_ffn(ExpertWeights w, int S, int E, int D, int F, unsigned flags = 0);
struct ExpertFfnArgs { const float* x; int ldx; const int32_t *pos, *acc_hist; const void *w1, *w2; const float *s1, *s2, *b1, *b2;
                       int w2_sliced; float h_scale; float* slab; const float *ln_gamma, *ln_beta; float ln_eps;
                       const void* xq; const float* xq_scale; int32_t* fs_dev; float* y_scatter; };
int launch_expert_ffn(const ExpertFfnPlan& plan, int S, int E, int D, int F, const ExpertFfnArgs& a, hipStream_t stream);
int init_expert_ffn_kernels();
int launch_expert_ffn_f32_slab(const float* x, int ldx, const int32_t* pos, const int32_t* acc_hist, int S, int E,
                               int D, int F, const float* w1, const float* b1, const float* w2, int w2_sliced, float* slab,
                               const float* ln_gamma, const float* ln_beta, float ln_eps, hipStream_t stream);
int init_expert_ffn_f32_tiled_kernels();
int launch_expert_tiled_f32(const float* x, int ldx, const int32_t* pos, const int32_t* acc_hist, int S, int E,
                            int D, int F, const float* w1, const float* b1, const float* w2, int w2_sliced,
                            float* hbuf, float* ybuf, hipStream_t stream);
int init_expert_ffn_bf16_kernels();
int launch_expert_ffn_bf16w_slab(const float* x, int ldx, const int32_t* pos, const int32_t* acc_hist, int S, int E,
                                 int D, int F, const void* w1, const float* b1, const void* w2, int w2_sliced, float* slab,
                                 hipStream_t stream);
int init_expert_ffn_w8_kernels();
int launch_expert_ffn_w8_slab(const float* x, int ldx, const int32_t* pos, const int32_t* acc_hist, int S, int E, int D, int F,
                              const void* w1, const float* s1, const float* b1, const void* w2, const float* s2, int w2_sliced,
                              float* slab, hipStream_t stream);
int init_expert_ffn_w4_kernels();
int launch_expert_ffn_w4_slab(const float* x, int ldx, const int32_t* pos, const int32_t* acc_hist, int S, int E, int D, int F,
                              const void* w1, const void* s1, const float* b1, const void* w2, const void* s2, int w2_sliced,
                              float* slab, hipStream_t stream);
constexpr int kExpertFusedFp8MaxSplit = 4;
int expert_ffn_fused_fp8_fsplit(int S, int E, int D, int F);
int init_expert_ffn_fused_fp8_kernels();
int launch_expert_ffn_fused_fp8(const float* x, int ldx, const int32_t* pos, const int32_t* acc_hist, int S, int E, int D, int F,
                                const void* w1, const float* s1, const float* b1, const void* w2, const float* s2, int w2_sliced,
                                float h_scale, int fsplit, float* ybuf, hipStream_t stream, const void* xq = nullptr,
                                const float* xq_scale = nullptr, int32_t* fs_dev = nullptr);
int launch_quantize_rows_e4m3(const float* x, int ldx, int S, int D, void* xq, float* scale, hipStream_t stream);
int launch_expert_tiled_w16(int w_fp8, const float* x, int ldx, const int32_t* pos, const int32_t* acc_hist, int S, int E,
// ... 317 lines not shown
```

3m-asr-inference_amd/csrc/moe_expert.hip:

```cpp
#include <stdlib.h>

#include "common.h"
#include "kernels.h"
#include "moe_gate.h"

namespace m3 {

struct ExpertRoute {
  const float* logits = nullptr;
  const int32_t* row_len = nullptr; int rows_per_batch = 0;
  int32_t* gate_idx = nullptr; float* gate_value = nullptr;
  int32_t* mapping = nullptr; int32_t* acc_hist = nullptr; int32_t* pos = nullptr;
  const float* b2 = nullptr;
  int wave_route = 0;
};

struct ExpertSwitches {
  bool route_wave;
};
static const ExpertSwitches& expert_switches() {
  static const ExpertSwitches sw = [] {
    auto num = [](const char* name, int dflt) { const char* v = getenv(name); return v ? atoi(v) : dflt; };
    ExpertSwitches w;
    w.route_wave = num("M3_ROUTE_WAVE", 1) != 0;
    return w;
  }();
  return sw;
}

template <int MT, bool LNS, int RE = 0>
__global__ __launch_bounds__(64 * (kExpertSlice / 16)) void expert_ffn_f32_kernel(const float* __restrict__ x, int ldx,
                                                             const int32_t* __restrict__ pos,
                                                             const int32_t* __restrict__ acc_hist, int S, int D,
                                                             int F, const float* __restrict__ w1,
                                                             const float* __restrict__ b1,
                                                             const float* __restrict__ w2, int w2_row_stride,
                                                             int w2_slice_stride, float* __restrict__ slab,
                                                             const float* __restrict__ ln_gamma,
                                                             const float* __restrict__ ln_beta, float ln_eps, ExpertRoute rt) {
  extern __shared__ __attribute__((aligned(16))) float lds[];
  const int e = blockIdx.y, slice = blockIdx.x;
  const int lane = threadIdx.x & 63, wave = threadIdx.x >> 6;
  const int col = lane & 15, kq = lane >> 4;

  const int xs_ld = D + 8;
  constexpr int hs_ld = kExpertSlice + 8;
  constexpr int NWV = kExpertSlice / 16;
  constexpr int KS2 = kExpertSlice / 16;
  constexpr int SPG = 8 / KS2;
  constexpr int NB = 2;
  static_assert(kExpertSlice == 16 || kExpertSlice == 32 || kExpertSlice == 64, "slice must be 16/32/64");
  float* xs = lds;
  float* hs = lds + 16 * MT * xs_ld;
  const int f0 = slice * kExpertSlice;
  const int ksteps1 = D >> 4;

  const float* w1row = w1 + ((size_t)e * F + f0 + 16 * wave + col) * D + 4 * kq;
  const float bias1 = b1[(size_t)e * F + f0 + 16 * wave + col];
  const int nsub = D >> 4;
  const float* w2_slice = w2 + (size_t)e * D * F + (size_t)slice * w2_slice_stride;

  const int g1 = (ksteps1 + 7) >> 3;
  const int g2 = ((nsub + NWV - 1) / NWV + SPG - 1) / SPG;
  const int total = g1 + g2;

  f32x4 wb[NB][8];
  float bb[NB][SPG];
  const bool add_b2 = RE > 0 && slice == 0 && rt.b2 != nullptr;
  auto load_group = [&](int g, int buf) {
    if (g < g1) {
#pragma unroll
      for (int i = 0; i < 8; ++i) {
        const int s = min(8 * g + i, ksteps1 - 1);
        wb[buf][i] = ldg4_w(w1row + (s << 4));
      }
    } else {
#pragma unroll
      for (int j = 0; j < SPG; ++j) {
        const int sub = min(wave + NWV * (SPG * (g - g1) + j), nsub - 1);
        const float* p = w2_slice + (size_t)(16 * sub + col) * w2_row_stride + 4 * kq;
#pragma unroll
        for (int st = 0; st < KS2; ++st) wb[buf][KS2 * j + st] = ldg4_w(p + 16 * st);
        if (RE > 0) bb[buf][j] = add_b2 ? rt.b2[(size_t)e * D + 16 * sub + col] : 0.f;
      }
    }
  };
  constexpr int REW = RE > 0 ? RE : 8;
  f32x4 lrow[REW / 4];
  const bool wroute = RE > 0 && MT == 1 && rt.wave_route != 0;
  const int rt_r = wroute ? lane : 64 * wave + lane;
  bool rt_live = false;
  if (RE > 0) {
    rt_live = rt_r < S && (rt.row_len == nullptr || (rt_r % rt.rows_per_batch) < rt.row_len[rt_r / rt.rows_per_batch]);
    const float* lp = rt.logits + (size_t)min(rt_r, S - 1) * RE;
#pragma unroll
    for (int j = 0; j < REW / 4; ++j) lrow[j] = ldg4(lp + 4 * j);
  }
  int row_lo, row_hi;
  int wrow = 0;
  __shared__ int32_t route_rows[RE > 0 ? 64 * (kExpertSlice / 16) : 1];
  __shared__ int route_cnt[RE > 0 ? 2 * (kExpertSlice / 16) : 1];
  if (wroute) {
    const int r = rt_r;
    const bool live = rt_live, taps = slice == 0 && wave == 0;
    int gi = -1;
    float gv = 0.f;
    gate_top1_regs<REW>(lrow, &gi, &gv, taps);
    if (!live) { gi = -1; gv = 0.f; }
    const unsigned long long mine = __ballot(gi == e), below = __ballot(live && gi < e);
    const unsigned long long lower = (1ull << lane) - 1ull;
    const int n_e = __popcll(mine), acc_e = __popcll(below);
    const int rank = __popcll(mine & lower);
    const int dest = gi == e ? rank : n_e + __popcll(~mine & lower);
    wrow = __builtin_amdgcn_ds_permute(dest << 2, lane);
    if (taps) {
// ... 181 lines not shown
                  if (i < nrows) slab_base[(size_t)i * D + 16 * sub + col] = acc2[r];
                }
              }
            }
          }
        }
      }
    };

#pragma unroll
    for (int b = 1; b < NB - 1; ++b)
      if (b < total) load_group(b, b);
    for (int g0 = 0; g0 < total; g0 += NB) {
#pragma unroll
      for (int b = 0; b < NB; ++b) {
        const int g = g0 + b;
        if (g < total) {
          if (g + NB - 1 < total) load_group(g + NB - 1, (b + NB - 1) % NB);
          if (g == g1) transition();
          compute(g, b);
        }
      }
    }
  }
}

int init_expert_ffn_kernels() {
  static PerDeviceOnce once;
  if (once.done()) return 0;
  M3_CHECK_HIP(hipFuncSetAttribute((const void*)expert_ffn_f32_kernel<2, false>, hipFuncAttributeMaxDynamicSharedMemorySize, 160 * 1024));
  M3_CHECK_HIP(hipFuncSetAttribute((const void*)expert_ffn_f32_kernel<4, false>, hipFuncAttributeMaxDynamicSharedMemorySize, 160 * 1024));
  M3_CHECK_HIP(hipFuncSetAttribute((const void*)expert_ffn_f32_kernel<2, true>, hipFuncAttributeMaxDynamicSharedMemorySize, 160 * 1024));
  M3_CHECK_HIP(hipFuncSetAttribute((const void*)expert_ffn_f32_kernel<4, true>, hipFuncAttributeMaxDynamicSharedMemorySize, 160 * 1024));
  once.mark();
  return 0;
}

size_t expert_ffn_slab_bytes(int S, int D, int F) {
  return (size_t)(F / kExpertSlice) * (size_t)S * (size_t)D * sizeof(float);
}

int launch_expert_ffn_f32_slab(const float* x, int ldx, const int32_t* pos, const int32_t* acc_hist, int S, int E, int D,
                               int F, const float* w1, const float* b1, const float* w2, int w2_sliced, float* slab,
                               const float* ln_gamma, const float* ln_beta, float ln_eps, hipStream_t stream) {
  M3_REQUIRE(S > 0 && E > 0, "expert_ffn: empty problem S=%d E=%d", S, E);
  M3_REQUIRE((D & 15) == 0 && D <= 2048, "expert_ffn: idim=%d must be a multiple of 16 (<=2048)", D);
  M3_REQUIRE(F % kExpertSlice == 0, "expert_ffn: hidden_units=%d must be a multiple of %d", F, kExpertSlice);
  M3_REQUIRE((ldx & 3) == 0, "expert_ffn: ldx=%d must be a multiple of 4", ldx);
  const int mt = S <= 64 ? 1 : (S <= 512 ? 2 : 4);
  const size_t lds_bytes = (size_t)16 * mt * ((D + 8) + (kExpertSlice + 8)) * sizeof(float);
  M3_REQUIRE(lds_bytes <= 160 * 1024, "expert_ffn: LDS tile of %zu bytes does not fit", lds_bytes);
  int zt = cdiv(S, 16 * mt);
  dim3 grid(F / kExpertSlice, E, zt < 8 ? zt : 8);
  const int w2_row_stride = w2_sliced ? kExpertSlice : F;
  const int w2_slice_stride = w2_sliced ? D * kExpertSlice : kExpertSlice;
  if (int rc = init_expert_ffn_kernels()) return rc;
#define M3_EXPERT_CASE2(MT_, LNS_)                                                                      \
  hipLaunchKernelGGL((expert_ffn_f32_kernel<MT_, LNS_>), grid, dim3(64 * (kExpertSlice / 16)), lds_bytes, stream, x, ldx, pos,    \
                     acc_hist, S, D, F, w1, b1, w2, w2_row_stride, w2_slice_stride, slab, ln_gamma, ln_beta, ln_eps, ExpertRoute())
#define M3_EXPERT_CASE(MT_) do { if (ln_gamma) M3_EXPERT_CASE2(MT_, true); else M3_EXPERT_CASE2(MT_, false); } while (0)
  if (mt == 1) M3_EXPERT_CASE(1); else if (mt == 2) M3_EXPERT_CASE(2); else M3_EXPERT_CASE(4);
#undef M3_EXPERT_CASE
#undef M3_EXPERT_CASE2
  M3_LAUNCH_CHECK();
  return 0;
}

bool expert_ffn_f32_self_routing(int S, int E) { return S >= 1 && S <= 64 * (kExpertSlice / 16) && (E == 8 || E == 16 || E == 32 || E == 64); }

int launch_expert_route_ffn_f32(const float* x, int ldx, const float* logits, const int32_t* row_len, int rows_per_batch, int S, int E,
                                int D, int F, const float* w1, const float* b1, const float* w2, int w2_sliced, const float* b2,
                                float* slab, int32_t* gate_idx, float* gate_value, int32_t* mapping, int32_t* acc_hist, int32_t* pos,
                                hipStream_t stream, const float* ln_gamma, const float* ln_beta, float ln_eps) {
  M3_REQUIRE(expert_ffn_f32_self_routing(S, E), "expert_route_ffn: needs 1 <= S <= %d rows and 8/16/32/64 experts (S=%d E=%d)", 64 * (kExpertSlice / 16), S, E);
  M3_REQUIRE((D & 15) == 0 && D <= 2048 && F % kExpertSlice == 0 && (ldx & 3) == 0, "expert_route_ffn: bad dims D=%d F=%d ldx=%d", D, F, ldx);
  M3_REQUIRE(logits && gate_idx && gate_value && slab, "expert_route_ffn: null pointer");
  M3_REQUIRE(row_len == nullptr || rows_per_batch > 0, "expert_route_ffn: rows_per_batch missing");
  const int mt = S <= 64 ? 1 : 2;
  const size_t lds_bytes = (size_t)16 * mt * ((D + 8) + (kExpertSlice + 8)) * sizeof(float);
  M3_REQUIRE(lds_bytes <= 150 * 1024, "expert_route_ffn: LDS tile of %zu bytes does not fit", lds_bytes);
  static PerDeviceOnce once;
  if (!once.done()) {
#define M3_ROUTE_ATTR(MT_, E_)                                                                                                                            \
  M3_CHECK_HIP(hipFuncSetAttribute((const void*)expert_ffn_f32_kernel<MT_, false, E_>, hipFuncAttributeMaxDynamicSharedMemorySize, 150 * 1024)); \
  M3_CHECK_HIP(hipFuncSetAttribute((const void*)expert_ffn_f32_kernel<MT_, true, E_>, hipFuncAttributeMaxDynamicSharedMemorySize, 150 * 1024))
    M3_ROUTE_ATTR(2, 8); M3_ROUTE_ATTR(2, 16); M3_ROUTE_ATTR(2, 32); M3_ROUTE_ATTR(2, 64);
#undef M3_ROUTE_ATTR
    once.mark();
  }
  ExpertRoute rt;
  rt.logits = logits; rt.row_len = row_len; rt.rows_per_batch = rows_per_batch; rt.gate_idx = gate_idx; rt.gate_value = gate_value;
  rt.mapping = mapping; rt.acc_hist = acc_hist; rt.pos = pos; rt.b2 = b2;
  rt.wave_route = S <= 64 && expert_switches().route_wave;
  dim3 grid(F / kExpertSlice, E, 1);
  const int w2_row_stride = w2_sliced ? kExpertSlice : F;
  const int w2_slice_stride = w2_sliced ? D * kExpertSlice : kExpertSlice;
#define M3_ROUTE_CASE(MT_, E_)                                                                                              \
  do {                                                                                                                      \
    if (ln_gamma != nullptr)                                                                                                \
      hipLaunchKernelGGL((expert_ffn_f32_kernel<MT_, true, E_>), grid, dim3(64 * (kExpertSlice / 16)), lds_bytes, stream, x, ldx, \
                         nullptr, nullptr, S, D, F, w1, b1, w2, w2_row_stride, w2_slice_stride, slab, ln_gamma, ln_beta, ln_eps, rt); \
    else                                                                                                                    \
      hipLaunchKernelGGL((expert_ffn_f32_kernel<MT_, false, E_>), grid, dim3(64 * (kExpertSlice / 16)), lds_bytes, stream, x, ldx, \
                         nullptr, nullptr, S, D, F, w1, b1, w2, w2_row_stride, w2_slice_stride, slab, nullptr, nullptr, 0.f, rt); \
  } while (0)
#define M3_ROUTE_E(E_) do { if (mt == 1) M3_ROUTE_CASE(1, E_); else M3_ROUTE_CASE(2, E_); } while (0)
  switch (E) {
    case 8: M3_ROUTE_E(8); break;
    case 16: M3_ROUTE_E(16); break;
    case 32: M3_ROUTE_E(32); break;
    default: M3_ROUTE_E(64); break;
  }
#undef M3_ROUTE_E
#undef M3_ROUTE_CASE
  M3_LAUNCH_CHECK();
  return 0;
}

template <int NV>
__global__ __launch_bounds__(256) void moe_combine_kernel(const float* __restrict__ slab, int n_slices,
                                                          const int32_t* __restrict__ mapping,
                                                          const int32_t* __restrict__ gate_idx,
                                                          const float* __restrict__ gate_value,
                                                          const float* __restrict__ b2,
                                                          const float* resid, float alpha,
                                                          const float* __restrict__ ln_gamma,
                                                          const float* __restrict__ ln_beta, float ln_eps,
                                                          float* out, int S, int D, bf16_t* out_b, float* out_stats,
                                                          const int32_t* __restrict__ n_slices_dev) {
  const int lane = threadIdx.x & 63, wave = threadIdx.x >> 6;
  const int s = blockIdx.x * 4 + wave;
  if (s >= S) return;
  if (n_slices_dev != nullptr) n_slices = min(n_slices, *n_slices_dev);
  constexpr int NG = NV <= 2 ? NV : 1;
  const bool one_trip = NV <= 2 && mapping == nullptr && n_slices_dev == nullptr && n_slices >= 1 && n_slices <= 16;
  const int g = gate_idx ? gate_idx[s] : 0;
  const float gv_early = (one_trip && gate_value) ? gate_value[s] : 1.f;
  const int m = mapping ? mapping[s] : (g >= 0 ? s : -1);
  const float gate = (m >= 0) ? (one_trip ? gv_early : (gate_value ? gate_value[s] : 1.f)) : 0.f;
  f32x4 v[NV];
  float sum = 0.f;
  f32x4 ga[NG], be[NG];
  if (NV <= 2 && one_trip) {
    f32x4 t[NG][16], rs[NG];
#pragma unroll
    for (int i = 0; i < NG; ++i) {
// ... 130 lines not shown
```

3m-asr-inference_amd/csrc/moe_expert_plan.hip:

```cpp
#include <stdlib.h>

#include "common.h"
#include "kernels.h"

namespace m3 {

static int env_int(const char* name, int dflt) {
  const char* e = getenv(name);
  return e ? atoi(e) : dflt;
}

ExpertFfnPlan plan_expert_ffn(ExpertWeights w, int S, int E, int D, int F, unsigned flags) {
  static const int tiled_min_rows = env_int("M3_EXPERT_TILED_MIN_ROWS", 1024);
  static const int fused_min_rows = env_int("M3_EXPERT_FUSED_FP8_MIN_ROWS", 4096);
  static const int g256_min_rows_per_expert = env_int("M3_G256_MIN_ROWS_PER_EXPERT", 512);
  const bool f32 = w == ExpertWeights::F32, bf16 = w == ExpertWeights::BF16, w4 = w == ExpertWeights::MXFP4;
  ExpertFfnPlan p{};
  p.weights = w;
  p.label = "";
  if (S <= 0 || E <= 0 || D <= 0 || F <= 0) return p;
  const size_t room = expert_ffn_slab_bytes(S, D, F);

  if (w == ExpertWeights::FP8A8 && S >= fused_min_rows) {
    if (const int fs = expert_ffn_fused_fp8_fsplit(S, E, D, F)) {
// ... 1 lines not shown
      p.launches = 1; p.slices = p.fsplit = fs;
      return p;
    }
  }
  const size_t h_bytes = align_up((size_t)S * F * (f32 ? 4 : 2), 256), y_bytes = (size_t)S * D * 4;
  const int tile = f32 ? 64 : 128;
  const bool norm_in_kernel = f32 && (flags & EXPERT_NORM_IN_KERNEL);
  if (!norm_in_kernel && S >= tiled_min_rows && D % tile == 0 && F % tile == 0 && h_bytes + y_bytes <= room) {
    p.launches = 2; p.slices = 1; p.rows_off = h_bytes;
    const size_t xb_off = h_bytes + align_up(y_bytes, 256);
    if (bf16 && !(flags & EXPERT_SCATTER_ROWS) && expert_gemm_g256_takes(S, E, D, F) && S / E >= g256_min_rows_per_expert &&
        xb_off + (size_t)S * D * 2 <= room) {
      p.kernel = ExpertKernel::G256Bf16; p.label = "expert_gemm_g256_kernel";
      p.launches = 3; p.xb_off = xb_off;
    } else if (f32) {
      p.kernel = ExpertKernel::TiledF32; p.label = "expert_gemm_f32_tiled_kernel";
    } else {
      p.kernel = bf16 ? ExpertKernel::TiledBf16 : w4 ? ExpertKernel::TiledW4 : ExpertKernel::TiledW8;
      p.label = bf16 ? "gemm_bf16w_tiled_kernel<grouped>" : w4 ? "gemm_bf16w_tiled_kernel<grouped,mxfp4>" : "gemm_bf16w_tiled_kernel<grouped,fp8>";
    }
    return p;
  }
  p.kernel = f32 ? ExpertKernel::SlabF32 : bf16 ? ExpertKernel::SlabBf16 : w4 ? ExpertKernel::SlabW4 : ExpertKernel::SlabW8;
  p.label = f32 ? "expert_ffn_f32_kernel" : bf16 ? "expert_ffn_bf16w_kernel" : w4 ? "expert_ffn_w4_kernel" : "expert_ffn_w8_kernel";
  const int slice = f32 ? kExpertSlice : kExpertSliceW16, d_mult = f32 ? 16 : bf16 ? 32 : w4 ? 128 : 64;
  p.slices = F / slice;
  p.launches = D % d_mult == 0 && D <= 2048 && F % slice == 0 ? 1 : 0;
  return p;
}

int launch_expert_ffn(const ExpertFfnPlan& plan, int S, int E, int D, int F, const ExpertFfnArgs& a, hipStream_t stream) {
  M3_REQUIRE(a.ln_gamma == nullptr || plan.kernel == ExpertKernel::SlabF32, "expert_ffn: LayerNorm while gathering exists in the fp32 slab form only (S=%d E=%d)", S, E);
  M3_REQUIRE(a.y_scatter == nullptr || plan.kernel == ExpertKernel::TiledBf16, "expert_ffn: the scattering epilogue exists in the bf16 tiled form only (S=%d E=%d)", S, E);
  char* const region = (char*)a.slab;
  void* const hbuf = region + plan.h_off;
  float* const ybuf = (float*)(region + plan.rows_off);
  switch (plan.kernel) {
    case ExpertKernel::SlabF32:
      return launch_expert_ffn_f32_slab(a.x, a.ldx, a.pos, a.acc_hist, S, E, D, F, (const float*)a.w1, a.b1, (const float*)a.w2, a.w2_sliced,
                                        ybuf, a.ln_gamma, a.ln_beta, a.ln_eps, stream);
    case ExpertKernel::TiledF32:
      return launch_expert_tiled_f32(a.x, a.ldx, a.pos, a.acc_hist, S, E, D, F, (const float*)a.w1, a.b1, (const float*)a.w2, a.w2_sliced,
                                     (float*)hbuf, ybuf, stream);
    case ExpertKernel::SlabBf16:
      return launch_expert_ffn_bf16w_slab(a.x, a.ldx, a.pos, a.acc_hist, S, E, D, F, a.w1, a.b1, a.w2, a.w2_sliced, ybuf, stream);
    case ExpertKernel::TiledBf16:
      return launch_expert_tiled_w16(0, a.x, a.ldx, a.pos, a.acc_hist, S, E, D, F, a.w1, nullptr, a.b1, a.w2, nullptr, a.w2_sliced,
                                     hbuf, ybuf, stream, a.b2, a.y_scatter);
    case ExpertKernel::G256Bf16: {
      void* const xb = region + plan.xb_off;
      if (int rc = launch_rows_to_bf16(a.x, a.ldx, S, D, xb, stream)) return rc;
      return launch_expert_ffn_bf16_g256(xb, D, a.pos, a.acc_hist, S, E, D, F, a.w1, a.b1, a.w2, a.w2_sliced, hbuf, ybuf, stream);
    }
    case ExpertKernel::SlabW8:
      return launch_expert_ffn_w8_slab(a.x, a.ldx, a.pos, a.acc_hist, S, E, D, F, a.w1, a.s1, a.b1, a.w2, a.s2, a.w2_sliced, ybuf, stream);
    case ExpertKernel::TiledW8:
      return launch_expert_tiled_w16(1, a.x, a.ldx, a.pos, a.acc_hist, S, E, D, F, a.w1, a.s1, a.b1, a.w2, a.s2, a.w2_sliced, hbuf,
                                     ybuf, stream);
    case ExpertKernel::SlabW4:
      return launch_expert_ffn_w4_slab(a.x, a.ldx, a.pos, a.acc_hist, S, E, D, F, a.w1, a.s1, a.b1, a.w2, a.s2, a.w2_sliced, ybuf, stream);
    case ExpertKernel::TiledW4:
      return launch_expert_tiled_w16(2, a.x, a.ldx, a.pos, a.acc_hist, S, E, D, F, a.w1, a.s1, a.b1, a.w2, a.s2, a.w2_sliced, hbuf,
                                     ybuf, stream);
    case ExpertKernel::FusedFp8:
      return launch_expert_ffn_fused_fp8(a.x, a.ldx, a.pos, a.acc_hist, S, E, D, F, a.w1, a.s1, a.b1, a.w2, a.s2, a.w2_sliced, a.h_scale,
                                         plan.fsplit, ybuf, stream, a.xq, a.xq_scale, a.fs_dev);
// ... 6 lines not shown
```

3m-asr-inference_amd/m3asr/_lib.py:

```python
import ctypes as C
import os

_HERE = os.path.dirname(os.path.abspath(__file__))
LIB_PATH = os.environ.get("M3ASR_LIB") or os.path.join(_HERE, "libm3asr_hip.so")


class M3Error(RuntimeError):
    pass


class Tensor(C.Structure):
    _fields_ = [("data", C.c_void_p), ("dtype", C.c_int32), ("ndim", C.c_int32), ("shape", C.c_int64 * 8)]


class Field(C.Structure):
    _fields_ = [("name", C.c_char_p), ("data", C.c_void_p), ("type", C.c_int32), ("length", C.c_int32)]


class LinearDesc(C.Structure):
    _fields_ = [("a", C.c_void_p), ("lda", C.c_int32),
                ("a2", C.c_void_p), ("lda2", C.c_int32), ("k1", C.c_int32),
                ("w", C.c_void_p), ("bias", C.c_void_p),
                ("y", C.c_void_p), ("ldy", C.c_int32),
                ("M", C.c_int32), ("N", C.c_int32), ("K", C.c_int32),
# ... 96 lines not shown

_vp, _i, _f, _sz, _i64, _cp, _d = C.c_void_p, C.c_int, C.c_float, C.c_size_t, C.c_int64, C.c_char_p, C.c_double
_P = C.POINTER

class StageInfo(C.Structure):
    _fields_ = [("kernel", C.c_char_p), ("launches", C.c_int32), ("per_row", C.c_int32),
                ("alg_bytes", C.c_double), ("flops", C.c_double)]


SIGNATURES = {
    "m3_abi_version": (_i, []),
    "m3_last_error": (_cp, []),
    "m3_registry_lookup": (_i, [_cp, _cp]),
    "m3_registry_count": (_i, []),
    "m3_registry_name": (_cp, [_i]),
    "m3_plugin_create": (_vp, [_cp, _cp, _P(Field), _i]),
    "m3_plugin_clone": (_vp, [_vp]),
    "m3_plugin_destroy": (None, [_vp]),
    "m3_plugin_type": (_cp, [_vp]),
    "m3_plugin_num_outputs": (_i, [_vp]),
    "m3_plugin_output_dims": (_i, [_vp, _P(Tensor), _i, _P(Tensor), _i]),
    "m3_plugin_workspace_size": (_sz, [_vp, _P(Tensor), _i, _P(Tensor), _i]),
    "m3_plugin_enqueue": (_i, [_vp, _P(Tensor), _i, _P(Tensor), _i, _vp, _sz, _vp]),
    "m3_plugin_serialization_size": (_sz, [_vp]),
    "m3_plugin_serialize": (_i, [_vp, _vp, _sz]),
    "m3_plugin_deserialize": (_vp, [_cp, _cp, _vp, _sz]),
    "m3_moe_scatter_mapping": (_i, [_vp, _i, _i, _vp, _vp, _vp, _vp]),
    "m3_moe_local_scatter": (_i, [_vp, _vp, _i, _i, _vp, _vp]),
    "m3_moe_local_gather": (_i, [_vp, _vp, _i, _i, _vp, _vp]),
    "m3_moe_expert_slice": (_i, []),
    "m3_moe_expert_workspace_size": (_sz, [_i, _i, _i, _i]),
    "m3_moe_expert_ffn": (_i, [_vp, _vp, _vp, _vp, _vp, _vp, _i, _i, _i, _i, _vp, _vp, _f, _vp, _vp, _f, _vp,
                               _vp, _sz, _vp]),
    "m3_moe_expert_ffn_bf16": (_i, [_vp, _vp, _vp, _vp, _vp, _vp, _i, _i, _i, _i, _vp, _vp, _f, _vp, _vp, _f, _vp,
                                    _vp, _sz, _vp]),
    "m3_moe_expert_ffn_fp8": (_i, [_vp, _vp, _vp, _vp, _vp, _vp, _vp, _vp, _i, _i, _i, _i, _vp, _vp, _f, _vp, _vp, _f, _vp,
                                   _vp, _sz, _vp]),
    "m3_moe_expert_ffn_mxfp4": (_i, [_vp, _vp, _vp, _vp, _vp, _vp, _vp, _vp, _i, _i, _i, _i, _vp, _vp, _f, _vp, _vp, _f, _vp,
                                     _vp, _sz, _vp]),
    "m3_moe_expert_ffn_mxfp4_ldx": (_i, [_vp, _i, _vp, _vp, _vp, _vp, _vp, _vp, _vp, _i, _i, _i, _i, _vp, _vp, _f, _vp, _vp, _f, _vp,
                                         _vp, _sz, _vp]),
    "m3_moe_expert_ffn_fp8a8": (_i, [_vp, _vp, _vp, _vp, _vp, _vp, _vp, _vp, _f, _i, _i, _i, _i, _vp, _vp, _f, _vp, _vp, _f, _vp,
                                     _vp, _sz, _vp]),
    "m3_moe_expert_ffn_fp8a8_active": (_i, [_i, _i, _i, _i]),
    "m3_moe_expert_ffn_kernel": (C.c_char_p, [_i, _i, _i, _i, _i, _i, _vp, _vp]),
    "m3_moe_expert_ffn_fp8a8_xq": (_i, [_vp, _vp, _vp, _vp, _vp, _vp, _vp, _vp, _vp, _vp, _f, _i, _i, _i, _i, _vp, _vp, _f, _vp, _vp,
                                        _f, _vp, _vp, _sz, _vp]),
    "m3_quantize_rows_e4m3": (_i, [_vp, _i, _i, _i, _vp, _vp, _vp]),
    "m3_moe_combine": (_i, [_vp, _vp, _vp, _vp, _f, _vp, _vp, _f, _vp, _i, _i, _vp]),
    "m3_moe_combine_bf16": (_i, [_vp, _vp, _vp, _vp, _f, _vp, _vp, _f, _vp, _vp, _i, _i, _vp]),
    "m3_softmax_top1": (_i, [_vp, _i, _vp, _i, _i, _i, _vp, _vp, _vp]),
    "m3_moe_router": (_i, [_vp, _i, _i, _vp, _i, _i, _vp, _vp, _vp, _vp, _f, _vp, _i, _vp, _i, _i, _i, _vp]),
    "m3_moe_gate_index": (_i, [_vp, _vp, _i, _i, _i, _vp, _vp, _vp, _vp, _vp, _vp]),
    "m3_moe_route": (_i, [_vp, _i, _i, _vp, _vp, _vp, _vp, _i, _f, _vp, _i, _i, _i, _vp, _vp, _vp, _vp, _vp, _vp]),
    "m3_moe_route_expert_workspace_size": (_sz, [_i, _i, _i, _i]),
    "m3_moe_route_expert_ffn": (_i, [_vp, _i, _vp, _vp, _i, _vp, _vp, _vp, _i, _vp, _i, _i, _i, _i, _vp, _vp, _f, _i, _vp, _f,
                                     _vp, _vp, _f, _vp, _vp, _vp, _vp, _vp, _vp, _vp, _sz, _vp]),
    "m3_linear": (_i, [_P(LinearDesc), _vp]),
    "m3_linear_workspace_size": (_sz, [_P(LinearDesc)]),
    "m3_linear_kernel": (C.c_char_p, [_P(LinearDesc), _i]),
    "m3_linear_ws": (_i, [_P(LinearDesc), _vp, _sz, _vp]),
    "m3_linear_pair": (_i, [_P(LinearDesc), _P(LinearDesc), _vp]),
    "m3_linear_ws_pair": (_i, [_P(LinearDesc), _vp, _sz, _P(LinearDesc), _vp, _sz, _i, _vp]),
    "m3_linear_pair_kernel": (C.c_char_p, [_P(LinearDesc), _P(LinearDesc), _i]),
    "m3_conv2d_3x3s2_workspace_size": (_sz, [_i, _i, _i, _i, _i]),
    "m3_conv2d_3x3s2_ws": (_i, [_vp, _vp, _vp, _i, _i, _i, _i, _i, _vp, _vp, _sz, _vp]),
    "m3_conv2d_3x3s2_ws_pair": (_i, [_P(Conv2dDesc), _vp, _sz, _P(Conv2dDesc), _vp, _sz, _i, _vp]),
    "m3_relpos_attention_pair": (_i, [_P(AttentionDesc), _P(AttentionDesc), _vp]),
    "m3_dwconv_ln_silu_pair": (_i, [_P(DwconvDesc), _P(DwconvDesc), _vp]),
    "m3_subsample_conv1_pair": (_i, [_P(Conv1Desc), _P(Conv1Desc), _vp]),
    "m3_subsample_conv1_ch": (_i, [_P(Conv1ChDesc), _vp]),
    "m3_subsample_conv1_ch_pair": (_i, [_P(Conv1ChDesc), _P(Conv1ChDesc), _vp]),
    "m3_conv2d_3x3s2_first": (_i, [_vp, _vp, _vp, _i, _i, _i, _i, _i, _vp, _vp]),
    "m3_conv2d_3x3s2": (_i, [_vp, _vp, _vp, _i, _i, _i, _i, _i, _vp, _vp]),
    "m3_layer_norm": (_i, [_vp, _vp, _vp, _f, _vp, _i, _i, _vp]),
    "m3_relpos_attention": (_i, [_vp, _i, _vp, _i, _vp, _vp, _vp, _i, _i, _i, _i, _f, _vp, _i, _vp]),
    "m3_relpos_attention_bf16": (_i, [_vp, _i, _vp, _i, _vp, _vp, _vp, _i, _i, _i, _i, _f, _i, _i, _vp, _i, _vp]),
    "m3_relpos_attention_chunk": (_i, [_vp, _i, _vp, _i, _vp, _vp, _vp, _i, _i, _i, _i, _f, _i, _i, _vp, _i, _vp]),
    "m3_dwconv_ln_silu": (_i, [_vp, _vp, _vp, _vp, _vp, _f, _i, _i, _i, _i, _vp, _vp]),
    "m3_dwconv_glu_ln_silu": (_i, [_vp, _i, _vp, _vp, _vp, _vp, _f, _i, _i, _i, _i, _vp, _vp]),
    "m3_relpos_attention_stream": (_i, [_vp, _i, _vp, _i, _vp, _i, _i, _vp, _vp, _vp, _vp, _i, _i, _i, _i, _f, _i, _i, _vp, _i, _vp]),
    "m3_dwconv_ln_silu_stream": (_i, [_vp, _vp, _vp, _vp, _vp, _f, _i, _i, _i, _i, _vp, _vp, _vp, _i, _vp, _vp]),
    "m3_dwconv_ln_silu_causal": (_i, [_vp, _vp, _vp, _vp, _vp, _f, _vp, _i, _i, _i, _i, _vp, _vp]),
    "m3_subsample_conv1": (_i, [_vp, _vp, _vp, _i, _i, _i, _i, _vp, _vp]),
    "m3_subsample_conv1_cmvn": (_i, [_vp, _vp, _vp, _vp, _vp, _i, _i, _i, _i, _vp, _vp]),
    "m3_cmvn": (_i, [_vp, _vp, _vp, _vp, _i, _i, _i, _vp, _vp]),
    "m3_log_softmax_bias": (_i, [_vp, _vp, _vp, _sz, _i, _vp]),
    "m3_subsample_conv2": (_i, [_vp, _vp, _vp, _i, _i, _i, _i, _vp, _vp]),
    "m3_ctc_greedy": (_i, [_vp, _vp, _i, _i, _i, _i, _vp, _vp, _vp, _vp]),
    "m3_ctc_topk": (_i, [_vp, _sz, _i, _i, _vp, _vp, _vp]),
    "m3_ctc_prefix_beam_search": (_i, [_vp, _vp, _i, _i, _i, _i, _vp, _vp, _vp, _vp]),
    "m3_ctc_beam_state_size": (_sz, [_P(CtcBeamDesc)]),
    "m3_ctc_beam_reset": (_i, [_P(CtcBeamDesc), _vp, _sz, _vp]),
    "m3_ctc_beam_reset_slots": (_i, [_P(CtcBeamDesc), _vp, _sz, _vp, _i, _vp]),
# ... 148 lines not shown
```

3m-asr-inference_amd/m3asr/config.py:

```python
from dataclasses import dataclass, field, asdict
import json


@dataclass
class EncoderConfig:
    input_dim: int = 40
    output_dim: int = 1434
    attention_dim: int = 512
    attention_heads: int = 8
    num_blocks: int = 18
    cnn_module_kernel: int = 15
    cnn_module_norm: str = "layer_norm"
    embed_heads: int = 4
    embed_dim: int = 512
    embed_linear_units: int = 1024
    embed_blocks: int = 6
    embed_cnn_module_norm: str = "layer_norm"
    num_experts: int = 32
    hidden_units: int = 1024
    router_with_bias: bool = False
    keep_expert_output: bool = False
    ep_world_size: int = 1
    ep_rank: int = 0
    max_len: int = 5000
    weight_dtype: str = "f32"
    fp8_activations: bool = False
    log_softmax_out: bool = False
    static_chunk_size: int = 0
    num_decoding_left_chunks: int = -1
    causal: bool = False
    embed_causal: bool = False
    conv_subsample_in_ch: int = 1
    embed_conv_subsample_in_ch: int = 1
    delta_order: int = 0
    delta_window: int = 2

    _LATE_FIELDS = ("conv_subsample_in_ch", "embed_conv_subsample_in_ch", "delta_order", "delta_window")

    def __post_init__(self):
        if not 0 <= self.delta_order <= 2:
            raise ValueError("EncoderConfig: delta_order=%d outside [0, 2]" % self.delta_order)
        if not 1 <= self.delta_window <= 4:
            raise ValueError("EncoderConfig: delta_window=%d outside [1, 4]" % self.delta_window)
        if self.input_dim % (1 + self.delta_order):
            raise ValueError("EncoderConfig: input_dim=%d is no multiple of 1 + delta_order = %d blocks of mel bins" % (
                self.input_dim, 1 + self.delta_order))
        for name in ("conv_subsample_in_ch", "embed_conv_subsample_in_ch"):
            ch = getattr(self, name)
            if not 1 <= ch <= 3:
                raise ValueError("EncoderConfig: %s=%d outside [1, 3]" % (name, ch))
            if self.input_dim % ch or self.input_dim // ch < 7:
                raise ValueError("EncoderConfig: %s=%d: input_dim=%d must be a multiple of it with at least 7 bins per channel" % (
                    name, ch, self.input_dim))
        if self.weight_dtype == "mxfp4" and self.fp8_activations:
            raise ValueError("EncoderConfig: fp8_activations needs weight_dtype 'fp8'; 'mxfp4' is a weight-only mode (W4A16)")

    def fp8_label(self):
        if self.fp8_activations:
            return ("fp8 arithmetic (e4m3 weights x e4m3 activations, v_mfma_f32_32x32x16_fp8_fp8) in the grouped expert FFN where "
                    "the fused fp8 kernel applies, e4m3 weight-only (W8A16) elsewhere")
        return "fp8 e4m3 weight-only (W8A16: dequantised to bf16 at the MFMA input, bf16 MFMA)"

    @property
    def d_k(self):
        return self.attention_dim // self.attention_heads

    @property
    def sub_freq(self):
        return ((self.input_dim // self.conv_subsample_in_ch - 1) // 2 - 1) // 2

# ... 102 lines not shown
```

3m-asr-inference_amd/m3asr/engine.py:

```python
import collections
import ctypes as C

import torch

from . import _lib
from ._lib import check
from .config import EncoderConfig, subsampled_len
from .plan import pack_weights


_TORCH_DTYPE = {torch.float32: _lib.F32, torch.bfloat16: _lib.BF16, torch.int32: _lib.I32, torch.float8_e4m3fn: _lib.FP8,
                torch.uint8: _lib.MXFP4}


def _engine_config(cfg: EncoderConfig, fold_pos_proj, debug_taps, fuse_route=False, bf16_activations=True, packed_rows=None,
                   ep_stages=False, fork_embed=None):
    ec = _lib.EngineConfig()
    ec.input_dim, ec.output_dim = cfg.input_dim, cfg.output_dim
    ec.attention_dim, ec.attention_heads, ec.num_blocks = cfg.attention_dim, cfg.attention_heads, cfg.num_blocks
    ec.embed_dim, ec.embed_heads = cfg.embed_dim, cfg.embed_heads
    ec.embed_linear_units, ec.embed_blocks = cfg.embed_linear_units, cfg.embed_blocks
    ec.num_experts, ec.hidden_units = cfg.num_experts, cfg.hidden_units
    ec.cnn_module_kernel = cfg.cnn_module_kernel
    ec.cnn_layer_norm = int(cfg.cnn_module_norm == "layer_norm")
    ec.embed_cnn_layer_norm = int(cfg.embed_cnn_module_norm == "layer_norm")
    ec.router_with_bias, ec.keep_expert_output = int(cfg.router_with_bias), int(cfg.keep_expert_output)
    ec.ep_world_size, ec.ep_rank = cfg.ep_world_size, cfg.ep_rank
    ec.fold_pos_proj, ec.debug_taps, ec.fuse_route = int(fold_pos_proj), int(debug_taps), int(fuse_route)
    ec.log_softmax_out = int(cfg.log_softmax_out)
    ec.bf16_activations = 0 if bf16_activations else -1
    ec.weight_dtype = {"f32": _lib.F32, "bf16": _lib.BF16, "fp8": _lib.FP8, "mxfp4": _lib.MXFP4}[cfg.weight_dtype]
    ec.packed_rows = 0 if packed_rows is None else (1 if packed_rows else -1)
    ec.fp8_activations = int(bool(getattr(cfg, "fp8_activations", False)) and cfg.weight_dtype == "fp8")
    ec.ep_stages = int(bool(ep_stages))
    ec.fork_embed = 0 if fork_embed is None else (1 if fork_embed else -1)
    ec.static_chunk_size = int(getattr(cfg, "static_chunk_size", 0))
    ec.num_left_chunks = int(getattr(cfg, "num_decoding_left_chunks", -1))
    ec.causal, ec.embed_causal = int(bool(getattr(cfg, "causal", False))), int(bool(getattr(cfg, "embed_causal", False)))
    return ec


class Engine:
    def __init__(self, cfg: EncoderConfig, packed, device="cuda:0", fold_pos_proj=True, debug_taps=False,
                 fuse_route=False, bf16_activations=True, packed_rows=None, max_shapes=8, ep_stages=False, fork_embed=None):
        self.lib = _lib.load()
        from .plan import EXPERT_SLICE
        assert self.lib.m3_moe_expert_slice() == EXPERT_SLICE, "plan.EXPERT_SLICE out of sync with libm3asr_hip.so"
        self.cfg = cfg
        self.device = torch.device(device)
        torch.cuda.set_device(self.device)
        self.weights = {k: (v if v.is_cuda else v.to(self.device, non_blocking=False)).contiguous() for k, v in packed.items()
                        if not k.startswith("decoder.")}
        names = [n for n in self.weights if not n.startswith("after_norm.")]
        table = (_lib.WeightEntry * len(names))()
        self._keep = [n.encode() for n in names]
        for i, n in enumerate(names):
            table[i].name = self._keep[i]
            table[i].data = self.weights[n].data_ptr()
            table[i].numel = self.weights[n].numel()
            table[i].dtype = _TORCH_DTYPE[self.weights[n].dtype]
        self.ep_stages = bool(ep_stages) or cfg.ep_world_size > 1
        ec = _engine_config(cfg, fold_pos_proj, debug_taps, int(fuse_route) if not self.ep_stages else 0, bf16_activations, packed_rows,
                            ep_stages=ep_stages, fork_embed=fork_embed)
        self.handle = self.lib.m3_engine_create(C.byref(ec), table, len(names))
        if not self.handle:
            raise _lib.M3Error("m3_engine_create failed: " + _lib.last_error())
        self.stream = torch.cuda.Stream(device=self.device)
        self.max_shapes = max(1, int(max_shapes))
        self._ws = collections.OrderedDict()
        self._static = collections.OrderedDict()
        self._bound = None
        self._ep_capacity = 0

    def set_ep_capacity(self, rows_per_chunk):
        check(self.lib.m3_engine_set_ep_capacity(self.handle, int(rows_per_chunk)), "m3_engine_set_ep_capacity")
        self._ep_capacity = int(rows_per_chunk)

    @classmethod
    def from_state_dict(cls, cfg, state_dict, **kw):
        return cls(cfg, pack_weights(state_dict, cfg), **kw)

    def clone_context(self, **kw):
        return Engine(self.cfg, self.weights, device=str(self.device), **kw)

    def __del__(self):
# ... 304 lines not shown
```

3m-asr-inference_amd/m3asr/ops.py:

```python
import ctypes as C
import math

import torch

from . import _lib
from ._lib import check


def _stream():
    return C.c_void_p(torch.cuda.current_stream().cuda_stream)


def _p(t):
    if t is None:
        return None
    assert t.is_cuda and t.is_contiguous(), "m3asr ops need contiguous device tensors"
    return C.c_void_p(t.data_ptr())


def _f32(t):
    assert t is None or t.dtype == torch.float32, "fp32 tensor expected"
    return _p(t)


# ... 48 lines not shown
    row_bytes = wire.shape[-1] * wire.element_size()
    check(lib.m3_ep_recv_gate(_p(wire), world, e_loc, capacity, row_bytes, _p(gate_recv), _stream()), "m3_ep_recv_gate")
    return gate_recv


def moe_local_gather(buf, mapping):
    lib = _lib.load()
    S = mapping.numel()
    row_bytes = buf[0].numel() * buf.element_size()
    out = torch.empty((S,) + tuple(buf.shape[1:]), dtype=buf.dtype, device=buf.device)
    check(lib.m3_moe_local_gather(_p(buf), _i32(mapping), S, row_bytes, _p(out), _stream()), "m3_moe_local_gather")
    return out


def moe_expert_workspace_size(S, E, D, F):
    return _lib.load().m3_moe_expert_workspace_size(S, E, D, F)


def quantize_rows_e4m3(x):
    lib = _lib.load()
    S, D = x.shape
    xp, ldx = _rows(x)
    xq = torch.empty(S, D, dtype=torch.uint8, device=x.device)
    scale = torch.empty(S, dtype=torch.float32, device=x.device)
    check(lib.m3_quantize_rows_e4m3(xp, ldx, S, D, _p(xq), _p(scale), _stream()), "m3_quantize_rows_e4m3")
    return xq, scale


def moe_expert_ffn(x, gate_idx, w1, b1, w2, b2, gate_value=None, resid=None, alpha=1.0, ln=None, workspace=None,
                   w1_scale=None, w2_scale=None, out=None, h_scale=None, xq=None, xq_scale=None):
    lib = _lib.load()
    assert w1.dtype == w2.dtype and w1.is_contiguous() and w2.is_contiguous()
    S, D = x.shape
    E, F = w1.shape[0], w1.shape[1]
    if workspace is None:
        workspace = torch.empty(max(moe_expert_workspace_size(S, E, D, F), 1), dtype=torch.uint8, device=x.device)
    y = out if out is not None else torch.empty_like(x)
    g, b, eps = ln if ln is not None else (None, None, 0.0)
    gate = _f32(gate_value.reshape(-1) if gate_value is not None else None)
    tail = (S, E, D, F, gate, _f32(resid), float(alpha), _f32(g), _f32(b), float(eps), _p(y), _p(workspace),
            workspace.numel(), _stream())
    xi, gi = _f32(x), _i32(gate_idx.reshape(-1))
    if w1.dtype == torch.float8_e4m3fn and h_scale is not None:
        assert w1_scale is not None and w2_scale is not None, "fp8 expert weights need their per-row scales"
        if xq is not None:
            assert xq.dtype in (torch.uint8, torch.float8_e4m3fn) and xq.is_contiguous() and xq.shape == x.shape and xq_scale is not None
            check(lib.m3_moe_expert_ffn_fp8a8_xq(xi, _p(xq), _f32(xq_scale), gi, _p(w1), _f32(w1_scale), _f32(b1), _p(w2),
                                                 _f32(w2_scale), _f32(b2), float(h_scale), *tail), "m3_moe_expert_ffn_fp8a8_xq")
            return y
        check(lib.m3_moe_expert_ffn_fp8a8(xi, gi, _p(w1), _f32(w1_scale), _f32(b1), _p(w2), _f32(w2_scale), _f32(b2),
                                          float(h_scale), *tail), "m3_moe_expert_ffn_fp8a8")
    elif w1.dtype == torch.float8_e4m3fn:
        assert w1_scale is not None and w2_scale is not None, "fp8 expert weights need their per-row scales"
        check(lib.m3_moe_expert_ffn_fp8(xi, gi, _p(w1), _f32(w1_scale), _f32(b1), _p(w2), _f32(w2_scale), _f32(b2), *tail),
              "m3_moe_expert_ffn_fp8")
    elif w1.dtype == torch.uint8:
        assert w1_scale is not None and w2_scale is not None and w1_scale.dtype == torch.uint8 and w2_scale.dtype == torch.uint8, \
            "mxfp4 expert weights need their uint8 block scales"
        assert w1.shape[2] * 2 == D and tuple(w2.shape) == (E, D, F // 2), "mxfp4 expert weights: two codes per byte along K"
        assert tuple(w1_scale.shape) == (E, F, D // 32) and tuple(w2_scale.shape) == (E, D, F // 32)
        assert w1_scale.is_contiguous() and w2_scale.is_contiguous()
        check(lib.m3_moe_expert_ffn_mxfp4(xi, gi, _p(w1), _p(w1_scale), _f32(b1), _p(w2), _p(w2_scale), _f32(b2), *tail),
              "m3_moe_expert_ffn_mxfp4")
    elif w1.dtype == torch.bfloat16:
        check(lib.m3_moe_expert_ffn_bf16(xi, gi, _p(w1), _f32(b1), _p(w2), _f32(b2), *tail), "m3_moe_expert_ffn_bf16")
    else:
        check(lib.m3_moe_expert_ffn(xi, gi, _f32(w1), _f32(b1), _f32(w2), _f32(b2), *tail), "m3_moe_expert_ffn")
    return y


def moe_combine(rows, mapping, gate_value=None, resid=None, alpha=1.0, ln=None, out=None, out_bf16=None):
    lib = _lib.load()
    S, D = mapping.numel(), rows.shape[-1]
    y = out if out is not None else torch.empty(S, D, dtype=torch.float32, device=rows.device)
    g, b, eps = ln if ln is not None else (None, None, 0.0)
    if out_bf16 is not None:
        assert out_bf16.dtype == torch.bfloat16 and out_bf16.numel() >= S * D and out_bf16.is_contiguous()
        check(lib.m3_moe_combine_bf16(_f32(rows), _i32(mapping), _f32(gate_value.reshape(-1) if gate_value is not None else None),
                                      _f32(resid), float(alpha), _f32(g), _f32(b), float(eps), _p(y), _p(out_bf16), S, D, _stream()),
              "m3_moe_combine_bf16")
        return y
    check(lib.m3_moe_combine(_f32(rows), _i32(mapping), _f32(gate_value.reshape(-1) if gate_value is not None else None),
                             _f32(resid), float(alpha), _f32(g), _f32(b), float(eps), _p(y), S, D, _stream()),
          "m3_moe_combine")
    return y


def moe_router(embed, x, w, ln, bias=None, want_xn=True, out=None, xn_out=None):
    lib = _lib.load()
    S, De = embed.shape
    D = x.shape[1]
    E = w.shape[0]
    assert w.shape[1] == De + D and w.is_contiguous()
    logits = out if out is not None else torch.empty(S, E, dtype=torch.float32, device=x.device)
    xn = xn_out if xn_out is not None else (torch.empty(S, D, dtype=torch.float32, device=x.device) if want_xn else None)
    assert tuple(logits.shape) == (S, E) and (xn is None or tuple(xn.shape) == (S, D))
    (ep, lde), (xp, ldx), (lp, ldl) = _rows(embed), _rows(x), _rows(logits)
    xnp, ldxn = _rows(xn) if xn is not None else (None, D)
# ... 24 lines not shown
    return taps, (_i32(gi), _f32(gv), _i32(mp), _i32(acc), _i32(pos))


def moe_gate_index(logits, row_len=None, rows_per_batch=0, taps=None):
    lib = _lib.load()
    S, E = logits.shape
    taps, ptrs = _route_taps(S, E, logits.device, taps)
    check(lib.m3_moe_gate_index(_f32(logits), _i32(row_len), rows_per_batch, S, E, *ptrs, _stream()), "m3_moe_gate_index")
    return taps


def moe_route(x, wx, wsum, bias=None, eall=None, ln_eps=1e-12, row_len=None, rows_per_batch=0, taps=None):
    lib = _lib.load()
    S, D = x.shape
    E = wx.shape[0]
    assert tuple(wx.shape) == (E, D) and wsum.numel() == E and (bias is None or bias.numel() == E)
    xp, ldx = _rows(x)
    ep, lde = _rows(eall) if eall is not None else (None, E)
    assert eall is None or tuple(eall.shape) == (S, E)
    taps, ptrs = _route_taps(S, E, x.device, taps)
    check(lib.m3_moe_route(xp, ldx, D, _f32(wx), _f32(wsum), _f32(bias), ep, lde, float(ln_eps), _i32(row_len), rows_per_batch,
                           S, E, *ptrs, _stream()), "m3_moe_route")
    return taps


def moe_route_expert_workspace_size(S, E, D, F):
    return _lib.load().m3_moe_route_expert_workspace_size(S, E, D, F)


def moe_route_expert_ffn(x, logits, w1, b1, w2, b2, row_len=None, rows_per_batch=0, w2_sliced=False, norm=None,
                         use_gate_value=True, resid=None, alpha=1.0, ln=None, workspace=None, out=None, taps=None):
    lib = _lib.load()
    S, D = x.shape
    E, F = w1.shape[0], w1.shape[1]
    assert tuple(logits.shape) == (S, E) and w1.is_contiguous()
    if w2_sliced and w2.dim() == 3:
        from .plan import slice_major_w2
        w2 = slice_major_w2(w2)
    if workspace is None:
        workspace = torch.empty(max(moe_route_expert_workspace_size(S, E, D, F), 1), dtype=torch.uint8, device=x.device)
    y = out if out is not None else torch.empty(S, D, dtype=torch.float32, device=x.device)
    xp, ldx = _rows(x)
    ng, nb, neps = norm if norm is not None else (None, None, 0.0)
    g, b, eps = ln if ln is not None else (None, None, 0.0)
    taps, ptrs = _route_taps(S, E, x.device, taps)
    check(lib.m3_moe_route_expert_ffn(xp, ldx, _f32(logits), _i32(row_len), rows_per_batch, _f32(w1), _f32(b1), _f32(w2),
                                      1 if w2_sliced else 0, _f32(b2), S, E, D, F, _f32(ng), _f32(nb), float(neps),
                                      1 if use_gate_value else 0, _f32(resid), float(alpha), _f32(g), _f32(b), float(eps),
                                      *ptrs, _p(y), _p(workspace), workspace.numel() * workspace.element_size(), _stream()),
          "m3_moe_route_expert_ffn")
    return y, taps


def linear(a, w, bias=None, act=_lib.ACT_NONE, a2=None, ln=None, lens=None, rows_per_batch=0, mask_in=False,
           mask_out=False, alpha=1.0, resid=None, out=None, ln_folded=None, split_k=False, out_dtype=torch.float32,
           copy_bf16=None, copy_stats=None, ln_stats=None, workspace=None, _kernel_only=False, _desc_only=False):
    lib = _lib.load()
    M, K1 = a.shape
    N, K = w.shape
    n_out = N // 2 if act == _lib.ACT_GLU else N
    y = out if out is not None else torch.empty(M, n_out, dtype=out_dtype, device=a.device)
    for t in (a, a2, y, resid, copy_bf16):
        assert t is None or (t.is_cuda and t.dim() == 2 and t.stride(1) == 1), "row-strided 2-D device tensor expected"
    assert tuple(y.shape) == (M, n_out) and (resid is None or tuple(resid.shape) == (M, n_out))
    d = _lib.LinearDesc()
    d.a, d.lda = a.data_ptr(), a.stride(0)
    assert a.dtype in (torch.float32, torch.bfloat16) and y.dtype in (torch.float32, torch.bfloat16)
    d.a_dtype = _lib.BF16 if a.dtype == torch.bfloat16 else _lib.F32
    d.y_dtype = _lib.BF16 if y.dtype == torch.bfloat16 else _lib.F32
    if copy_bf16 is not None:
        assert copy_bf16.dtype == torch.bfloat16 and tuple(copy_bf16.shape) == (M, n_out)
        d.y_copy_bf16, d.ld_copy = copy_bf16.data_ptr(), copy_bf16.stride(0)
    if copy_stats is not None:
        assert copy_bf16 is not None and copy_stats.dtype == torch.float32 and copy_stats.is_contiguous()
        d.y_copy_stats = copy_stats.data_ptr()
    if ln_stats is not None:
        assert ln_stats.dtype == torch.float32 and ln_stats.is_contiguous() and ln_stats.shape[0] == M
        d.ln_stats, d.ln_stat_parts = ln_stats.data_ptr(), ln_stats.shape[1]
    if a2 is not None:
        d.a2, d.lda2, d.k1 = a2.data_ptr(), a2.stride(0), K1
        assert K1 + a2.shape[1] == K
    else:
        assert K1 == K
    assert w.dtype in (torch.float32, torch.bfloat16) and w.is_contiguous()
    d.w, d.bias = w.data_ptr(), (bias.data_ptr() if bias is not None else None)
    d.weight_dtype = _lib.BF16 if w.dtype == torch.bfloat16 else _lib.F32
    d.y, d.ldy = y.data_ptr(), y.stride(0)
    d.M, d.N, d.K = M, N, K
    if ln is not None:
        d.ln_gamma, d.ln_beta, d.ln_eps = ln[0].data_ptr(), ln[1].data_ptr(), float(ln[2])
    if ln_folded is not None:
        d.ln_wsum, d.ln_eps = ln_folded[0].data_ptr(), float(ln_folded[2])
        if ln_folded[1] is not None:
            d.ln_wbeta = ln_folded[1].data_ptr()
    if lens is not None:
        d.len, d.rows_per_batch = lens.data_ptr(), rows_per_batch
    d.mask_in, d.mask_out = int(mask_in), int(mask_out)
    d.act, d.alpha = act, float(alpha)
    if resid is not None:
        d.resid, d.ldr = resid.data_ptr(), resid.stride(0)
    if _desc_only:
        return d, y
    if _kernel_only:
        name = lib.m3_linear_kernel(C.byref(d), int(bool(split_k)))
        return name.decode() if name else None
    if split_k:
        need = lib.m3_linear_workspace_size(C.byref(d))
        ws = workspace if workspace is not None else torch.empty(max(need, 1), dtype=torch.uint8, device=a.device)
        assert ws.dtype == torch.uint8 and ws.numel() >= need
        check(lib.m3_linear_ws(C.byref(d), _p(ws), need, _stream()), "m3_linear_ws")
        return y
    check(lib.m3_linear(C.byref(d), _stream()), "m3_linear")
    return y


def linear_kernel(*args, **kw):
    return linear(*args, _kernel_only=True, **kw)


def _linear_desc(kw):
    kw = dict(kw)
    return linear(kw.pop("a"), kw.pop("w"), _desc_only=True, **kw)


def linear_workspace_size(**kw):
    return _lib.load().m3_linear_workspace_size(C.byref(_linear_desc(kw)[0]))


def linear_pair(a, b):
    (da, ya), (db, yb) = _linear_desc(a), _linear_desc(b)
    check(_lib.load().m3_linear_pair(C.byref(da), C.byref(db), _stream()), "m3_linear_pair")
    return ya, yb


def linear_pair_kernel(a, b, with_workspace=False):
    name = _lib.load().m3_linear_pair_kernel(C.byref(_linear_desc(a)[0]), C.byref(_linear_desc(b)[0]), int(bool(with_workspace)))
    return name.decode() if name else None


def linear_ws_pair(a, ws_a, b, ws_b, which=3):
    (da, ya), (db, yb) = _linear_desc(a), _linear_desc(b)
    check(_lib.load().m3_linear_ws_pair(C.byref(da), _p(ws_a), ws_a.numel(), C.byref(db), _p(ws_b), ws_b.numel(), int(which), _stream()),
          "m3_linear_ws_pair")
    return ya, yb


def _attention_desc(qkv, p, pos_u, pos_v, lens, B, T, H, dk, chunk=0, left_chunks=-1, out=None):
    D = H * dk
    if out is None:
        out = torch.empty(B * T, D, dtype=torch.float32, device=qkv.device)
    assert tuple(qkv.shape) == (B * T, 3 * D) and tuple(p.shape)[1] == D and p.shape[0] >= T and tuple(out.shape) == (B * T, D)
    d = _lib.AttentionDesc()
    (d.qkv, d.ldq), (d.p, d.ldp), (d.out, d.ldo) = [(q.value, ld) for q, ld in (_rows(qkv), _rows(p), _rows(out))]
    d.pos_u, d.pos_v, d.len = _f32(pos_u).value, _f32(pos_v).value, (_i32(lens).value if lens is not None else None)
    d.B, d.T, d.H, d.dk, d.scale, d.chunk, d.left_chunks = B, T, H, dk, 1.0 / math.sqrt(dk), int(chunk), int(left_chunks)
    return d, out


def relpos_attention_pair(a, b):
    (da, oa), (db, ob) = _attention_desc(**a), _attention_desc(**b)
    check(_lib.load().m3_relpos_attention_pair(C.byref(da), C.byref(db), _stream()), "m3_relpos_attention_pair")
    return oa, ob


# ... 1090 lines not shown
```

3m-asr-inference_amd/m3asr/plan.py:

```python
import json
import re
import math
import struct
from collections import OrderedDict

import numpy as np
import torch

from .config import DecoderConfig, EncoderConfig

MAGIC = b"M3ASRPL1"
EXPERT_SLICE = 64


def positional_table(max_len, d):
    pe = torch.zeros(max_len, d)
    position = torch.arange(0, max_len, dtype=torch.float32).unsqueeze(1)
    div_term = torch.exp(torch.arange(0, d, 2, dtype=torch.float32) * -(math.log(10000.0) / d))
    pe[:, 0::2] = torch.sin(position * div_term)
    pe[:, 1::2] = torch.cos(position * div_term)
    return pe


def slice_major_w2(t):
    E_, D_, F_ = t.shape
    return t.reshape(E_, D_, F_ // EXPERT_SLICE, EXPERT_SLICE).permute(0, 2, 1, 3).contiguous()


def _pack_subsampling(sd, p, out):
    w0 = sd[p + "conv.0.weight"]
    C = w0.shape[0]
    out[p + "conv.0.weight_9c"] = w0.reshape(C, w0.shape[1] * 9).t().contiguous()
    out[p + "conv.0.bias"] = sd[p + "conv.0.bias"]
    out[p + "conv.2.weight_ohwi"] = sd[p + "conv.2.weight"].permute(0, 2, 3, 1).contiguous()
    out[p + "conv.2.bias"] = sd[p + "conv.2.bias"]
    wl = sd[p + "out.0.weight"]
    F2 = wl.shape[1] // C
    out[p + "out.0.weight"] = wl.view(-1, C, F2).permute(0, 2, 1).reshape(wl.shape[0], F2 * C).contiguous()
    out[p + "out.0.bias"] = sd[p + "out.0.bias"]


def fold_layernorm(weight, bias, gamma, beta):
    w64, g64, b64 = weight.double(), gamma.double(), beta.double()
    wf = (w64 * g64.unsqueeze(0)).float()
    return {"ln.weight": wf, "ln.bias": (bias.double() + w64 @ b64).float(),
            "ln.wsum": wf.double().sum(1).float(),
            "ln.wbeta": (w64 @ b64).float()}


def _put_folded(out, prefix, folded, keep_wbeta=False):
    for k, v in folded.items():
        if k != "ln.wbeta" or keep_wbeta:
            out[prefix + k] = v


def _pack_block(sd, p, out, norm, moe, cfg):
    folded = ["norm_ff_macaron", "norm_mha", "norm_conv"] + ([] if moe else ["norm_ff"])
    for n in ("norm_ff_macaron", "norm_mha", "norm_conv", "norm_ff", "norm_final"):
        if n not in folded:
# ... 236 lines not shown

def cast_gemm_weights(packed, cfg: EncoderConfig):
    if cfg.weight_dtype == "f32":
        return packed
    assert cfg.weight_dtype in ("bf16", "fp8", "mxfp4"), cfg.weight_dtype
    out = OrderedDict()
    for k, v in packed.items():
        if cfg.weight_dtype == "mxfp4" and v.dtype == torch.float32 and k.endswith("experts.w_1.weight"):
            out[k], out[k[:-len("weight")] + "scale"] = quantize_mxfp4(v, dim=2)
        elif cfg.weight_dtype == "mxfp4" and v.dtype == torch.float32 and k.endswith("experts.w_2.weight_sliced"):
            out[k], out[k[:-len("weight_sliced")] + "scale"] = quantize_mxfp4(v, dim=3)
        elif cfg.weight_dtype == "fp8" and v.dtype == torch.float32 and k.endswith("experts.w_1.weight"):
            q, sc = quantize_fp8_rows(v, dims=(2,))
            out[k], out[k[:-len("weight")] + "scale"] = q, sc
        elif cfg.weight_dtype == "fp8" and v.dtype == torch.float32 and k.endswith("experts.w_2.weight_sliced"):
            q, sc = quantize_fp8_rows(v, dims=(1, 3))
            out[k], out[k[:-len("weight_sliced")] + "scale"] = q, sc
        elif is_gemm_weight(k) and v.dtype == torch.float32:
            out[k] = v.to(torch.bfloat16).contiguous()
        else:
            out[k] = v
    for k in list(out):
        if k.endswith(".ln.weight") and out[k].dtype == torch.bfloat16:
            out[k[:-len("weight")] + "wsum"] = out[k].double().sum(1).float()
    return out


_DTYPES = {"f32": (torch.float32, "<f4", 4), "bf16": (torch.bfloat16, "<u2", 2), "i32": (torch.int32, "<i4", 4),
           "fp8": (torch.float8_e4m3fn, "u1", 1), "u8": (torch.uint8, "u1", 1)}
_DTYPE_NAME = {torch.float32: "f32", torch.bfloat16: "bf16", torch.int32: "i32", torch.float8_e4m3fn: "fp8", torch.uint8: "u8"}


def save_plan(path, cfg: EncoderConfig, packed, extra=None):
    index, off = {}, 0
    for k, v in packed.items():
        name = _DTYPE_NAME[v.dtype]
        index[k] = [off, list(v.shape)] + ([name] if name != "f32" else [])
        off += (v.numel() * _DTYPES[name][2] + 255) // 256 * 256
    header = json.dumps({"config": json.loads(cfg.to_json()), "tensors": index, "extra": extra or {}}).encode()
    with open(path, "wb") as f:
        f.write(MAGIC)
        f.write(struct.pack("<Q", len(header)))
        f.write(header)
        pad = (-(16 + len(header))) % 256
        f.write(b"\0" * pad)
        for k, v in packed.items():
            if v.dtype == torch.bfloat16:
                b = v.contiguous().view(torch.int16).numpy().astype("<i2", copy=False).tobytes()
            elif v.dtype == torch.float8_e4m3fn:
                b = v.contiguous().view(torch.uint8).numpy().tobytes()
            else:
                b = v.contiguous().numpy().astype(_DTYPES[_DTYPE_NAME[v.dtype]][1], copy=False).tobytes()
            f.write(b)
            f.write(b"\0" * ((-len(b)) % 256))


def load_plan(path):
    with open(path, "rb") as f:
        if f.read(8) != MAGIC:
            raise ValueError("%s is not an m3asr plan" % path)
        (hl,) = struct.unpack("<Q", f.read(8))
        header = json.loads(f.read(hl).decode())
    base = 16 + hl
    base += (-base) % 256
    mm = np.memmap(path, dtype=np.uint8, mode="r")
    packed = OrderedDict()
# ... 15 lines not shown
```

include/m3asr.h:

```cpp
#ifndef M3ASR_H_
#define M3ASR_H_
#include <stddef.h>
#include <stdint.h>

#ifdef __cplusplus
extern "C" {
#endif

#define M3ASR_ABI_VERSION 10

typedef void* m3_stream;

enum m3_dtype { M3_F32 = 0, M3_F16 = 1, M3_I8 = 2, M3_I32 = 3, M3_BF16 = 4, M3_FP8 = 5 ,
                M3_MXFP4 = 6  };

enum m3_act { M3_ACT_NONE = 0, M3_ACT_RELU = 1, M3_ACT_SILU = 2, M3_ACT_GLU = 3, M3_ACT_SIGMOID = 4, M3_ACT_LOG = 5 };
enum m3_binop { M3_OP_SUM = 0, M3_OP_PROD = 1 };

int m3_abi_version(void);
const char* m3_last_error(void);
int m3_registry_lookup(const char* plugin_name, const char* plugin_version);
int m3_registry_count(void);
const char* m3_registry_name(int index);

// ... 14 lines not shown

typedef struct m3_plugin m3_plugin;

m3_plugin* m3_plugin_create(const char* plugin_name, const char* plugin_version, const m3_field* fields,
                            int n_fields);
m3_plugin* m3_plugin_clone(const m3_plugin* plugin);
void m3_plugin_destroy(m3_plugin* plugin);
const char* m3_plugin_type(const m3_plugin* plugin);
int m3_plugin_num_outputs(const m3_plugin* plugin);
int m3_plugin_output_dims(const m3_plugin* plugin, const m3_tensor* inputs, int n_in, m3_tensor* outputs,
                          int n_out);
size_t m3_plugin_workspace_size(const m3_plugin* plugin, const m3_tensor* inputs, int n_in,
                                const m3_tensor* outputs, int n_out);
int m3_plugin_enqueue(m3_plugin* plugin, const m3_tensor* inputs, int n_in, m3_tensor* outputs, int n_out,
                      void* workspace, size_t workspace_bytes, m3_stream stream);
size_t m3_plugin_serialization_size(const m3_plugin* plugin);
int m3_plugin_serialize(const m3_plugin* plugin, void* buffer, size_t bytes);
m3_plugin* m3_plugin_deserialize(const char* plugin_name, const char* plugin_version, const void* buffer,
                                 size_t bytes);

int m3_moe_scatter_mapping(const int32_t* gate_idx, int S, int num_expert, int32_t* mapping,
                           int32_t* acc_histogram, int32_t* pos, m3_stream stream);
int m3_moe_local_scatter(const void* x, const int32_t* mapping, int S, int row_bytes, void* out,
                         m3_stream stream);
int m3_moe_local_gather(const void* buf, const int32_t* mapping, int S, int row_bytes, void* out,
                        m3_stream stream);
int m3_moe_expert_slice(void);
size_t m3_moe_expert_workspace_size(int S, int num_expert, int idim, int hidden_units);
int m3_moe_expert_ffn(const float* x, const int32_t* gate_idx, const float* w1, const float* b1,
                      const float* w2, const float* b2, int S, int num_expert, int idim, int hidden_units,
                      const float* gate_value, const float* resid, float alpha, const float* ln_gamma,
                      const float* ln_beta, float ln_eps, float* y, void* workspace, size_t workspace_bytes,
                      m3_stream stream);
int m3_moe_expert_ffn_bf16(const float* x, const int32_t* gate_idx, const void* w1, const float* b1,
                           const void* w2, const float* b2, int S, int num_expert, int idim, int hidden_units,
                           const float* gate_value, const float* resid, float alpha, const float* ln_gamma,
                           const float* ln_beta, float ln_eps, float* y, void* workspace, size_t workspace_bytes,
                           m3_stream stream);
int m3_moe_expert_ffn_fp8(const float* x, const int32_t* gate_idx, const void* w1, const float* w1_scale,
                          const float* b1, const void* w2, const float* w2_scale, const float* b2, int S, int num_expert,
                          int idim, int hidden_units, const float* gate_value, const float* resid, float alpha,
                          const float* ln_gamma, const float* ln_beta, float ln_eps, float* y, void* workspace,
                          size_t workspace_bytes, m3_stream stream);
int m3_moe_expert_ffn_mxfp4(const float* x, const int32_t* gate_idx, const void* w1, const void* w1_scale,
                            const float* b1, const void* w2, const void* w2_scale, const float* b2, int S, int num_expert,
                            int idim, int hidden_units, const float* gate_value, const float* resid, float alpha,
                            const float* ln_gamma, const float* ln_beta, float ln_eps, float* y, void* workspace,
                            size_t workspace_bytes, m3_stream stream);
int m3_moe_expert_ffn_mxfp4_ldx(const float* x, int ldx, const int32_t* gate_idx, const void* w1, const void* w1_scale,
                                const float* b1, const void* w2, const void* w2_scale, const float* b2, int S, int num_expert,
                                int idim, int hidden_units, const float* gate_value, const float* resid, float alpha,
                                const float* ln_gamma, const float* ln_beta, float ln_eps, float* y, void* workspace,
                                size_t workspace_bytes, m3_stream stream);
int m3_moe_expert_ffn_fp8a8(const float* x, const int32_t* gate_idx, const void* w1, const float* w1_scale,
                            const float* b1, const void* w2, const float* w2_scale, const float* b2, float h_scale, int S,
                            int num_expert, int idim, int hidden_units, const float* gate_value, const float* resid,
                            float alpha, const float* ln_gamma, const float* ln_beta, float ln_eps, float* y,
                            void* workspace, size_t workspace_bytes, m3_stream stream);
int m3_moe_expert_ffn_fp8a8_active(int S, int num_expert, int idim, int hidden_units);
const char* m3_moe_expert_ffn_kernel(int weight_dtype, int fp8_activations, int S, int num_expert, int idim, int hidden_units,
                                     int32_t* launches, int32_t* slices);
int m3_moe_expert_ffn_fp8a8_xq(const float* x, const void* xq, const float* xq_scale, const int32_t* gate_idx, const void* w1,
                               const float* w1_scale, const float* b1, const void* w2, const float* w2_scale, const float* b2,
                               float h_scale, int S, int num_expert, int idim, int hidden_units, const float* gate_value,
                               const float* resid, float alpha, const float* ln_gamma, const float* ln_beta, float ln_eps,
                               float* y, void* workspace, size_t workspace_bytes, m3_stream stream);
// ... 19 lines not shown
                 int ld_e, float ln_eps, const int32_t* row_len, int rows_per_batch, int S, int num_expert, int32_t* gate_idx,
                 float* gate_value, int32_t* mapping, int32_t* acc_histogram, int32_t* pos, m3_stream stream);
size_t m3_moe_route_expert_workspace_size(int S, int num_expert, int idim, int hidden_units);
int m3_moe_route_expert_ffn(const float* x, int ldx, const float* logits, const int32_t* row_len, int rows_per_batch,
                            const float* w1, const float* b1, const float* w2, int w2_sliced, const float* b2, int S,
                            int num_expert, int idim, int hidden_units, const float* norm_gamma, const float* norm_beta,
                            float norm_eps, int use_gate_value, const float* resid, float alpha, const float* ln_gamma,
                            const float* ln_beta, float ln_eps, int32_t* gate_idx, float* gate_value, int32_t* mapping,
                            int32_t* acc_histogram, int32_t* pos, float* y, void* workspace, size_t workspace_bytes,
                            m3_stream stream);

typedef struct m3_linear_desc {
  const float* a; int32_t lda;
  const float* a2; int32_t lda2; int32_t k1;
  const void* w;
  const float* bias;
  float* y; int32_t ldy;
  int32_t M, N, K;
  const float* ln_gamma; const float* ln_beta; float ln_eps;
  const float* ln_wsum; const float* ln_wbeta;
  const int32_t* len; int32_t rows_per_batch; int32_t mask_in; int32_t mask_out;
  int32_t act; float alpha;
  const float* resid; int32_t ldr;
  int32_t weight_dtype;
  int32_t a_dtype, y_dtype;
  void* y_copy_bf16; int32_t ld_copy;
  float* y_copy_stats;
  const float* ln_stats; int32_t ln_stat_parts;
} m3_linear_desc;
int m3_linear(const m3_linear_desc* desc, m3_stream stream);
size_t m3_linear_workspace_size(const m3_linear_desc* desc);
const char* m3_linear_kernel(const m3_linear_desc* desc, int with_workspace);
int m3_linear_ws(const m3_linear_desc* desc, void* workspace, size_t workspace_bytes, m3_stream stream);

int m3_layer_norm(const float* x, const float* gamma, const float* beta, float eps, float* y, int rows, int dim,
                  m3_stream stream);
int m3_relpos_attention(const float* qkv, int ldq, const float* p, int ldp, const float* pos_u,
                        const float* pos_v, const int32_t* len, int B, int T, int H, int dk, float scale,
                        float* out, int ldo, m3_stream stream);
int m3_relpos_attention_bf16(const void* qkv, int ldq, const float* p, int ldp, const float* pos_u, const float* pos_v,
                             const int32_t* len, int B, int T, int H, int dk, float scale, int chunk, int left_chunks,
                             void* out, int ldo, m3_stream stream);
int m3_relpos_attention_chunk(const float* qkv, int ldq, const float* p, int ldp, const float* pos_u, const float* pos_v,
                              const int32_t* len, int B, int T, int H, int dk, float scale, int chunk, int left_chunks,
                              float* out, int ldo, m3_stream stream);
int m3_dwconv_ln_silu(const float* z, const float* w_kc, const float* bias, const float* gamma,
                      const float* beta, float eps, int B, int T, int D, int K, float* out, m3_stream stream);
int m3_dwconv_glu_ln_silu(const float* vg, int ldz, const float* w_kc, const float* bias, const float* gamma,
                          const float* beta, float eps, int B, int T, int D, int K, float* out, m3_stream stream);
int m3_relpos_attention_stream(const float* qkv, int ldq, float* hist, int cap, const float* p, int ldp, int p_rows, const float* pos_u,
                               const float* pos_v, const int32_t* chunk_len, const int32_t* step, int B, int C, int H, int dk,
                               float scale, int left_chunks, int slot_max_chunks, float* out, int ldo, m3_stream stream);
int m3_dwconv_ln_silu_stream(const float* z, const float* w_kc, const float* bias, const float* gamma, const float* beta, float eps, int B,
                             int T, int D, int K, float* cache_pair, const int32_t* step, const int32_t* chunk_len, int slot_max_chunks,
                             float* out, m3_stream stream);
int m3_dwconv_ln_silu_causal(const float* z, const float* w_kc, const float* bias, const float* gamma, const float* beta, float eps,
                             const float* left_fill, int B, int T, int D, int K, float* out, m3_stream stream);
int m3_subsample_conv1(const float* feat, const float* w9c, const float* bias, int B, int T, int idim, int C,
                       float* out, m3_stream stream);
int m3_subsample_conv1_cmvn(const float* feat, const float* w9c, const float* bias, const float* cmvn_mean,
                            const float* cmvn_istd, int B, int T, int idim, int C, float* out, m3_stream stream);
int m3_conv2d_3x3s2_first(const float* feat, const float* w9c, const float* bias, int B, int T, int idim, int C, int act,
                          float* out, m3_stream stream);
int m3_conv2d_3x3s2(const float* in, const float* w, const float* bias, int B, int T1, int F1, int C, int act, float* out,
                    m3_stream stream);
int m3_subsample_conv2(const float* in, const float* w, const float* bias, int B, int T1, int F1, int C,
// ... 396 lines not shown
```

Measured before the change: 158,400 frames/s.

## Add fragment-ordered fp32 weight layout for skinny GEMMs and expert FFN

Result: faster. 171,500 frames/s (median of 6 runs) (+8.3%).

```diff
diff --git a/3m-asr-inference_amd/csrc/api.hip b/3m-asr-inference_amd/csrc/api.hip
--- a/3m-asr-inference_amd/csrc/api.hip
+++ b/3m-asr-inference_amd/csrc/api.hip
@@ -41,7 +41,7 @@
                       const float* b2, int S, int E, int D, int F, const float* gate_value, const float* resid,
                       float alpha, const float* ln_gamma, const float* ln_beta, float ln_eps, float* y, void* ws,
                       size_t ws_bytes, hipStream_t stream, ExpertWeights weights, const float* s1 = nullptr, const float* s2 = nullptr, float h_scale = 0.f, const void* xq = nullptr,
-                      const float* xq_scale = nullptr, int ldx = 0) {
+                      const float* xq_scale = nullptr, int ldx = 0, int w_layout = EXPERT_W_REF) {
   M3_REQUIRE(S >= 0 && E > 0 && D > 0 && F > 0, "fmoe_expert: bad sizes S=%d E=%d D=%d F=%d", S, E, D, F);
   if (S == 0) return 0;
   MoeWorkspace w = carve_moe_workspace(ws, S, E, D, F);
@@ -52,7 +52,7 @@
   const ExpertFfnPlan plan = plan_expert_ffn(weights, S, E, D, F);
   ExpertFfnArgs a{};
   a.x = x; a.ldx = ldx > 0 ? ldx : D; a.pos = w.pos; a.acc_hist = w.acc; a.w1 = w1; a.w2 = w2; a.s1 = s1; a.s2 = s2; a.b1 = b1;
-  a.h_scale = h_scale; a.slab = w.slab; a.xq = xq; a.xq_scale = xq_scale;
+  a.h_scale = h_scale; a.slab = w.slab; a.xq = xq; a.xq_scale = xq_scale; a.w2_sliced = w_layout;
   rc = launch_expert_ffn(plan, S, E, D, F, a, stream);
   if (rc) return rc;
   return launch_moe_combine(plan.rows(w.slab), plan.slices, w.mapping, gate_idx, gate_value, b2, resid, alpha, ln_gamma, ln_beta, ln_eps,
@@ -100,6 +100,14 @@
                       float* y, void* workspace, size_t workspace_bytes, m3_stream stream) {
   return moe_expert_ffn(x, gate_idx, w1, b1, w2, b2, S, num_expert, idim, hidden_units, gate_value, resid, alpha,
                         ln_gamma, ln_beta, ln_eps, y, workspace, workspace_bytes, (hipStream_t)stream);
+}
+int m3_moe_expert_ffn_wfrag(const float* x, const int32_t* gate_idx, const float* w1, const float* b1, const float* w2,
+                            const float* b2, int S, int num_expert, int idim, int hidden_units, const float* gate_value,
+                            const float* resid, float alpha, const float* ln_gamma, const float* ln_beta, float ln_eps,
+                            float* y, void* workspace, size_t workspace_bytes, m3_stream stream) {
+  return moe_expert_ffn_dt(x, gate_idx, w1, b1, w2, b2, S, num_expert, idim, hidden_units, gate_value, resid, alpha, ln_gamma, ln_beta,
+                           ln_eps, y, workspace, workspace_bytes, (hipStream_t)stream, ExpertWeights::F32, nullptr, nullptr, 0.f, nullptr,
+                           nullptr, 0, EXPERT_W_FRAG);
 }
 int m3_moe_expert_ffn_bf16(const float* x, const int32_t* gate_idx, const void* w1, const float* b1, const void* w2,
                            const float* b2, int S, int num_expert, int idim, int hidden_units, const float* gate_value,
@@ -359,6 +367,34 @@
   if (int rc = linear_pointers(d)) return rc;
   return launch_gemm(gemm_launch(p, (float*)workspace, workspace_bytes), (hipStream_t)stream);
 }
+int m3_linear_wfrag(const m3_linear_desc* d, m3_stream stream) {
+  GemmParams p;
+  if (int rc = linear_params(d, &p)) return rc;
+  if (int rc = linear_pointers(d)) return rc;
+  M3_REQUIRE(aligned16(d->w), "linear: fragment-ordered w must be 16-byte aligned");
+  p.w_frag = 1;
+  return launch_gemm(gemm_launch(p, nullptr, 0), (hipStream_t)stream);
+}
+const char* m3_linear_wfrag_kernel(const m3_linear_desc* d) {
+  GemmParams p;
+  if (linear_params(d, &p)) return nullptr;
+  p.w_frag = 1;
+  const GemmPlan plan = plan_gemm(p, 0);
+  if (plan.launches == 0) set_error("%s", plan.reason);
+  return plan.launches ? plan.label : nullptr;
+}
+int m3_pack_wfrag_host(const float* w, int N, int K, float* wf) {
+  M3_REQUIRE(w != nullptr && wf != nullptr && N > 0 && K > 0 && N % 16 == 0 && K % 16 == 0,
+             "pack_wfrag: N=%d and K=%d must be positive multiples of 16", N, K);
+  const int nsteps = K / 16;
+  for (int nt = 0; nt < N / 16; ++nt)
+    for (int s = 0; s < nsteps; ++s)
+      for (int kq = 0; kq < 4; ++kq)
+        for (int col = 0; col < 16; ++col)
+          for (int j = 0; j < 4; ++j)
+            wf[((((size_t)nt * nsteps + s) * 4 + kq) * 16 + col) * 4 + j] = w[(size_t)(16 * nt + col) * K + 16 * s + 4 * kq + j];
+  return 0;
+}
 
 int m3_layer_norm(const float* x, const float* gamma, const float* beta, float eps, float* y, int rows, int dim,
                   m3_stream stream) {
@@ -595,6 +631,19 @@
   M3_REQUIRE(!ranges_overlap(a->y, linear_out_bytes(a), b->y, linear_out_bytes(b)), "linear pair: the two outputs overlap");
   return launch_gemm_f32_dual(qa, qb, (hipStream_t)stream);
 }
+int m3_linear_pair_wfrag(const m3_linear_desc* a, const m3_linear_desc* b, m3_stream stream) {
+  GemmParams pa, pb;
+  if (int rc = linear_params(a, &pa)) return rc;
+  if (int rc = linear_params(b, &pb)) return rc;
+  if (int rc = linear_pointers(a)) return rc;
+  if (int rc = linear_pointers(b)) return rc;
+  M3_REQUIRE(aligned16(a->w) && aligned16(b->w), "linear pair: fragment-ordered w must be 16-byte aligned");
+  pa.w_frag = pb.w_frag = 1;
+  const GemmLaunch qa = gemm_launch(pa, nullptr, 0), qb = gemm_launch(pb, nullptr, 0);
+  if (int rc = linear_pair_plans(qa, qb)) return rc;
+  M3_REQUIRE(!ranges_overlap(a->y, linear_out_bytes(a), b->y, linear_out_bytes(b)), "linear pair: the two outputs overlap");
+  return launch_gemm_f32_dual(qa, qb, (hipStream_t)stream);
+}
 int m3_linear_ws_pair(const m3_linear_desc* a, void* workspace_a, size_t bytes_a, const m3_linear_desc* b, void* workspace_b,
                       size_t bytes_b, int which, m3_stream stream) {
   GemmParams pa, pb;
diff --git a/3m-asr-inference_amd/csrc/engine.hip b/3m-asr-inference_amd/csrc/engine.hip
--- a/3m-asr-inference_amd/csrc/engine.hip
+++ b/3m-asr-inference_amd/csrc/engine.hip
@@ -26,7 +26,7 @@
 namespace {
 
 struct Norm { const float* g = nullptr; const float* b = nullptr; };
-struct Lin { const float* w = nullptr; const float* b = nullptr; const float* wsum = nullptr; const float* wbeta = nullptr; };
+struct Lin { const float* w = nullptr; const float* b = nullptr; const float* wsum = nullptr; const float* wbeta = nullptr; const float* wf = nullptr; };
 
 struct BlockW {
   Norm n_ffm, n_mha, n_conv, n_ff, n_final, n_cnn;
@@ -37,6 +37,7 @@
   Lin router;
   Lin router_x;
   const float *ew1 = nullptr, *eb1 = nullptr, *ew2 = nullptr, *eb2 = nullptr;
+  const float *ew1f = nullptr, *ew2f = nullptr;
   const float *es1 = nullptr, *es2 = nullptr;
   float h_scale = 0.f;
 };
@@ -139,6 +140,7 @@
   bool front_pair;
   bool router_prefix;
   bool glu_sig_epi;
+  bool w_frag;
 };
 const Switches& switches() {
   static const Switches sw = [] {
@@ -155,6 +157,7 @@
     w.front_pair = num("M3_FRONT_PAIR", 1) != 0;
     w.router_prefix = num("M3_ROUTER_PREFIX", 1) != 0;
     w.glu_sig_epi = num("M3_GLU_SIG_EPI", 1) != 0;
+    w.w_frag = num("M3_W_FRAG", 1) != 0;
     return w;
   }();
   return sw;
@@ -192,8 +195,14 @@
   GET(n->b, p + "bias", d);
   return true;
 }
+const float* lookup_frag(const m3_engine* e, const std::string& name, int64_t numel) {
+  if (!switches().w_frag || e->cfg.weight_dtype != M3_F32) return nullptr;
+  auto it = e->table.find(name + "_frag");
+  return it != e->table.end() && it->second.numel == numel && it->second.dtype == M3_F32 ? (const float*)it->second.data : nullptr;
+}
 bool load_lin(const m3_engine* e, const std::string& p, int64_t n_out, int64_t n_in, bool bias, Lin* l) {
   GETW(l->w, p + "weight", n_out * n_in);
+  l->wf = lookup_frag(e, p + "weight", n_out * n_in);
   if (bias) GET(l->b, p + "bias", n_out);
   return true;
 }
@@ -204,6 +213,7 @@
   } else {
     GETW(l->w, p + "ln.weight", n_out * n_in);
   }
+  if (!fp32_only) l->wf = lookup_frag(e, p + "ln.weight", n_out * n_in);
   GET(l->b, p + "ln.bias", n_out);
   GET(l->wsum, p + "ln.wsum", n_out);
   if (wbeta) GET(l->wbeta, p + "ln.wbeta", n_out);
@@ -259,6 +269,9 @@
     GET(b->eb1, p + "feed_forward.experts.w_1.bias", E * F);
     GETE(b->ew2, p + "feed_forward.experts.w_2.weight_sliced", ew_numel);
     GET(b->eb2, p + "feed_forward.experts.w_2.bias", E * D);
+    b->ew1f = lookup_frag(e, p + "feed_forward.experts.w_1.weight", ew_numel);
+    b->ew2f = lookup_frag(e, p + "feed_forward.experts.w_2.weight", ew_numel);
+    if (!b->ew1f || !b->ew2f) b->ew1f = b->ew2f = nullptr;
   }
   return true;
 }
@@ -590,9 +603,15 @@
   sb.bd.stages.back().pairable = pairable;
 }
 
-static void add_gemm(StageBuilder& sb, const std::string& name, GemmParams p, bool fp32_weights = false) {
+static void add_gemm(StageBuilder& sb, const std::string& name, GemmParams p, bool fp32_weights = false, const float* wfrag = nullptr) {
   p.w_bf16 = (!fp32_weights && sb.eng.cfg.weight_dtype != M3_F32) ? 1 : 0;
-  const GemmLaunch g = gemm_launch(p, sb.splitk_ws, sb.splitk_bytes);
+  GemmLaunch g = gemm_launch(p, sb.splitk_ws, sb.splitk_bytes);
+  if (wfrag != nullptr && g.plan.launches == 1 && g.plan.kernel == GemmKernel::SkinnyF32) {
+    GemmParams q = p;
+    q.W = wfrag; q.w_frag = 1;
+    const GemmLaunch gf = gemm_launch(q, sb.splitk_ws, sb.splitk_bytes);
+    if (gf.plan.launches == 1) g = gf;
+  }
   m3_stage_info info = gemm_info(p, g.plan);
   info.launches = g.plan.launches ? g.plan.launches : 1;
   add_launch(sb, name, g, info, g.plan.launches == 1);
@@ -813,7 +832,7 @@
 static ExpertFfnArgs expert_args(const BlockW& w, const float* x, const MoeWorkspace& mw, int D) {
   ExpertFfnArgs a{};
   a.x = x; a.ldx = D; a.pos = mw.pos; a.acc_hist = mw.acc; a.w1 = w.ew1; a.w2 = w.ew2; a.s1 = w.es1; a.s2 = w.es2; a.b1 = w.eb1;
-  a.w2_sliced = 1; a.h_scale = w.h_scale; a.slab = mw.slab;
+  a.w2_sliced = EXPERT_W2_SLICED; a.h_scale = w.h_scale; a.slab = mw.slab;
   return a;
 }
 
@@ -826,11 +845,13 @@
   add_stage(sb, m.pfx + "moe_local.expert", f.launches, [=](hipStream_t s) {
     const BlockW& w = *m.w;
     const float* ln_g = norm ? w.n_ff.g : nullptr; const float* ln_b = norm ? w.n_ff.b : nullptr; const float ln_eps = norm ? m.eps : 0.f;
+    const bool wf = w.ew1f != nullptr;
     if (self_route)
-      return launch_expert_route_ffn_f32(xin, m.D, m.rl, m.live_len, m.live_rpb, m.S, m.E, m.D, m.F, w.ew1, w.eb1, w.ew2, 1, w.eb2,
-                                         m.mw.slab, m.gidx, m.gval, m.mw.mapping, m.mw.acc, m.mw.pos, s, ln_g, ln_b, ln_eps);
+      return launch_expert_route_ffn_f32(xin, m.D, m.rl, m.live_len, m.live_rpb, m.S, m.E, m.D, m.F, wf ? w.ew1f : w.ew1, w.eb1,
+                                         wf ? w.ew2f : w.ew2, wf ? EXPERT_W_FRAG : EXPERT_W2_SLICED, w.eb2, m.mw.slab, m.gidx, m.gval, m.mw.mapping, m.mw.acc, m.mw.pos, s, ln_g, ln_b, ln_eps);
     ExpertFfnArgs a = expert_args(w, xin, m.mw, m.D);
     a.ln_gamma = ln_g; a.ln_beta = ln_b; a.ln_eps = ln_eps; a.xq = xq; a.xq_scale = xqs; a.fs_dev = fs;
+    if (wf && f.kernel == ExpertKernel::SlabF32) { a.w1 = w.ew1f; a.w2 = w.ew2f; a.w2_sliced = EXPERT_W_FRAG; }
     return launch_expert_ffn(f, m.S, m.E, m.D, m.F, a, s);
   }, stage_info(f.label, 1, -1.0, 4.0 * m.D * m.F * m.S));
 }
@@ -896,9 +917,9 @@
 
 static void build_block(StageBuilder& sb, const std::string& pfx, const BlockW& w, int D, int F, int H, int K, bool cnn_ln,
                         bool moe, int layer, int tap_index, const Plan& pl, bool causal) {
-  auto add_gemm = [&](StageBuilder&, const std::string& name, GemmParams g, bool fp32_weights = false) {
+  auto add_gemm = [&](StageBuilder&, const std::string& name, GemmParams g, bool fp32_weights = false, const float* wfrag = nullptr) {
     if (sb.bd.packed) g.m_dev = pl.row0 + sb.bd.key.B;
-    ::add_gemm(sb, name, g, fp32_weights);
+    ::add_gemm(sb, name, g, fp32_weights, wfrag);
   };
   const m3_engine_config& c = sb.eng.cfg;
   const BindKey& key = sb.bd.key;
@@ -933,12 +954,12 @@
     g.A = x; g.lda = D; g.W = w.mac1.w; g.bias = w.mac1.b; g.Y = pl.h1; g.ldy = F; g.M = S; g.N = F; g.K = D;
     g.ln_wsum = w.mac1.wsum; g.ln_eps = eps; g.act = ACT_SILU;
     from_xb(g); g.y_bf16 = a16;
-    add_gemm(sb, pfx + "ffn_macaron.w1", g);
+    add_gemm(sb, pfx + "ffn_macaron.w1", g, false, w.mac1.wf);
     GemmParams h;
     h.A = pl.h1; h.lda = F; h.W = w.mac2.w; h.bias = w.mac2.b; h.Y = x; h.ldy = D; h.M = S; h.N = D; h.K = F;
     h.alpha = 0.5f; h.resid = x; h.ldr = D;
     h.a_bf16 = a16; also_xb(h);
-    add_gemm(sb, pfx + "ffn_macaron.w2", h);
+    add_gemm(sb, pfx + "ffn_macaron.w2", h, false, w.mac2.wf);
   }
   {
     GemmParams g;
@@ -947,7 +968,7 @@
     from_xb(g);
     const bool att16 = a16 && relpos_attention_bf16_supports(Tp, D / H);
     g.y_bf16 = att16;
-    add_gemm(sb, pfx + "att.qkv", g);
+    add_gemm(sb, pfx + "att.qkv", g, false, w.qkv.wf);
     const int ldp = (c.num_blocks + c.embed_blocks) * D;
     const float* pmat = pl.pbuf + (size_t)tap_index * D;
     const float* qkv = pl.qkv; float* ctx = pl.ctx;
@@ -971,7 +992,7 @@
     o.A = pl.ctx; o.lda = D; o.W = w.out.w; o.bias = w.out.b; o.Y = x; o.ldy = D; o.M = S; o.N = D; o.K = D;
     o.resid = x; o.ldr = D;
     o.a_bf16 = a16; also_xb(o);
-    add_gemm(sb, pfx + "att.out", o);
+    add_gemm(sb, pfx + "att.out", o, false, w.out.wf);
   }
   {
     GemmParams g;
@@ -989,7 +1010,7 @@
     }
     const bool glu_sig = glu_deferred && switches().glu_sig_epi && (D & 15) == 0;
     if (glu_sig) g.sig_col0 = D;
-    add_gemm(sb, pfx + "conv.pw1_glu", g);
+    add_gemm(sb, pfx + "conv.pw1_glu", g, false, w.pw1.wf);
     const float* glu = pl.glu; float* dw = pl.dw;
     const float* dww = w.dw_w; const float* dwb = w.dw_b;
     const float* ng = cnn_ln ? w.n_cnn.g : nullptr; const float* nb = cnn_ln ? w.n_cnn.b : nullptr;
@@ -1011,19 +1032,19 @@
     h.A = pl.dw; h.lda = D; h.W = w.pw2.w; h.bias = w.pw2.b; h.Y = x; h.ldy = D; h.M = S; h.N = D; h.K = D;
     h.row_len = live_len; h.rows_per_batch = live_rpb; h.mask_out = 1; h.resid = x; h.ldr = D;
     h.a_bf16 = a16; also_xb(h);
-    add_gemm(sb, pfx + "conv.pw2", h);
+    add_gemm(sb, pfx + "conv.pw2", h, false, w.pw2.wf);
   }
   if (!moe) {
     GemmParams g;
     g.A = x; g.lda = D; g.W = w.ff1.w; g.bias = w.ff1.b; g.Y = pl.h1; g.ldy = F; g.M = S; g.N = F; g.K = D;
     g.ln_wsum = w.ff1.wsum; g.ln_eps = eps; g.act = ACT_SILU;
     from_xb(g); g.y_bf16 = a16;
-    add_gemm(sb, pfx + "ffn.w1", g);
+    add_gemm(sb, pfx + "ffn.w1", g, false, w.ff1.wf);
     GemmParams h;
     h.A = pl.h1; h.lda = F; h.W = w.ff2.w; h.bias = w.ff2.b; h.Y = x; h.ldy = D; h.M = S; h.N = D; h.K = F;
     h.alpha = 0.5f; h.resid = x; h.ldr = D;
     h.a_bf16 = a16;
-    add_gemm(sb, pfx + "ffn.w2", h);
+    add_gemm(sb, pfx + "ffn.w2", h, false, w.ff2.wf);
     const float* fg = w.n_final.g; const float* fb = w.n_final.b;
     void* xbo = a16 ? xb : nullptr;
     float* xso = dma ? xstats : nullptr;
diff --git a/3m-asr-inference_amd/csrc/gemm.hip b/3m-asr-inference_amd/csrc/gemm.hip
--- a/3m-asr-inference_amd/csrc/gemm.hip
+++ b/3m-asr-inference_amd/csrc/gemm.hip
@@ -14,8 +14,9 @@
 
 enum { LN_NONE = GEMM_LN_NONE, LN_EPI = GEMM_LN_EPI, LN_PRO = GEMM_LN_PRO };
 
-template <int MT, bool GLU, int NW, bool CONV, int LN, int NBUF, bool ACCI = false>
+template <int MT, bool GLU, int NW, bool CONV, int LN, int NBUF, bool ACCI = false, bool WF = false>
 __device__ __forceinline__ void gemm_f32_body(const GemmParams& p, const int bid) {
+  static_assert(!WF || (!CONV && !ACCI), "fragment-ordered W: plain A only");
   constexpr int NT = GLU ? 2 : 1;
   constexpr int G = gemm_group_steps(MT, NT, NW);
   constexpr int I0 = ACCI ? G / 2 : 0;
@@ -77,7 +78,8 @@
   const float* wrow[NT];
 #pragma unroll
   for (int t = 0; t < NT; ++t)
-    wrow[t] = p.W + (size_t)min(n0 + t * Nout + col, p.N - 1) * p.K + 4 * kq;
+    wrow[t] = WF ? p.W + (size_t)(n_tile + t * (Nout >> 4)) * ((size_t)p.K << 4) + 4 * lane
+                 : p.W + (size_t)min(n0 + t * Nout + col, p.N - 1) * p.K + 4 * kq;
 
   f32x4 acc[MT][NT];
 #pragma unroll
@@ -111,7 +113,7 @@
       const int s = min(wave + NW * (G * g + i), nsteps - 1);
       const int k = s << 4;
 #pragma unroll
-      for (int t = 0; t < NT; ++t) wbuf[buf][i][t] = ldg4_w(wrow[t] + k);
+      for (int t = 0; t < NT; ++t) wbuf[buf][i][t] = ldg4_w(wrow[t] + (WF ? (s << 8) : k));
       const bool second = ACCI || (!CONV && p.mode == GEMM_A_CONCAT2 && k >= p.K1);
       const int off = second ? (k - p.K1) : a_offset(k);
 #pragma unroll
@@ -374,9 +376,9 @@
            })
 }
 
-template <int MT, bool GLU, int NW, bool CONV, int LN, int NBUF, bool ACCI = false>
+template <int MT, bool GLU, int NW, bool CONV, int LN, int NBUF, bool ACCI = false, bool WF = false>
 __global__ __launch_bounds__(64 * NW) void gemm_f32_kernel(const GemmParams p) {
-  gemm_f32_body<MT, GLU, NW, CONV, LN, NBUF, ACCI>(p, (int)blockIdx.x);
+  gemm_f32_body<MT, GLU, NW, CONV, LN, NBUF, ACCI, WF>(p, (int)blockIdx.x);
 }
 
 struct RouterPrefixArgs {
@@ -448,12 +450,12 @@
   M3_LAUNCH_CHECK();
   return 0;
 }
-template <int MT, bool GLU, int NW, int LN>
+template <int MT, bool GLU, int NW, int LN, bool WF = false>
 __global__ __launch_bounds__(64 * NW) void gemm_f32_dual_kernel(const GemmParams p0, const GemmParams p1, const int n0) {
   if ((int)blockIdx.x < n0) {
-    if ((int)blockIdx.x < p0.n_tiles * p0.m_tiles) gemm_f32_body<MT, GLU, NW, false, LN, 1>(p0, (int)blockIdx.x);
+    if ((int)blockIdx.x < p0.n_tiles * p0.m_tiles) gemm_f32_body<MT, GLU, NW, false, LN, 1, false, WF>(p0, (int)blockIdx.x);
   } else {
-    gemm_f32_body<MT, GLU, NW, false, LN, 1>(p1, (int)blockIdx.x - n0);
+    gemm_f32_body<MT, GLU, NW, false, LN, 1, false, WF>(p1, (int)blockIdx.x - n0);
   }
 }
 
@@ -468,7 +470,10 @@
   const int n0 = (int)align_up((size_t)q[0].n_tiles * q[0].m_tiles, 8);
   dim3 grid(n0 + q[1].n_tiles * q[1].m_tiles);
 #define M3_DUAL(GLU_, NW_, LN_)                                                                                             \
-  hipLaunchKernelGGL((gemm_f32_dual_kernel<1, GLU_, NW_, LN_>), grid, dim3(64 * NW_), 0, stream, q[0], q[1], n0)
+  do {                                                                                                                      \
+    if (q[0].w_frag) hipLaunchKernelGGL((gemm_f32_dual_kernel<1, GLU_, NW_, LN_, true>), grid, dim3(64 * NW_), 0, stream, q[0], q[1], n0); \
+    else hipLaunchKernelGGL((gemm_f32_dual_kernel<1, GLU_, NW_, LN_>), grid, dim3(64 * NW_), 0, stream, q[0], q[1], n0);    \
+  } while (0)
   if (pa.glu) {
     if (pa.nw == 8) { if (pa.ln == LN_EPI) M3_DUAL(true, 8, LN_EPI); else M3_DUAL(true, 8, LN_NONE); }
     else { if (pa.ln == LN_EPI) M3_DUAL(true, 4, LN_EPI); else M3_DUAL(true, 4, LN_NONE); }
@@ -495,7 +500,12 @@
 
 #define M3_GEMM_LAUNCH(MT_, GLU_, NW_, CONV_, LN_)                                                              \
   do {                                                                                                          \
-    if (plan.nbuf == 1)                                                                                         \
+    constexpr bool kWf = !(CONV_);         \
+    if (p.w_frag && plan.nbuf == 1)                                                                              \
+      hipLaunchKernelGGL((gemm_f32_kernel<MT_, GLU_, NW_, CONV_, LN_, 1, false, kWf>), grid, dim3(64 * NW_), 0, stream, p); \
+    else if (p.w_frag)                                                                                           \
+      hipLaunchKernelGGL((gemm_f32_kernel<MT_, GLU_, NW_, CONV_, LN_, 2, false, kWf>), grid, dim3(64 * NW_), 0, stream, p); \
+    else if (plan.nbuf == 1)                                                                                    \
       hipLaunchKernelGGL((gemm_f32_kernel<MT_, GLU_, NW_, CONV_, LN_, 1>), grid, dim3(64 * NW_), 0, stream, p); \
     else                                                                                                        \
       hipLaunchKernelGGL((gemm_f32_kernel<MT_, GLU_, NW_, CONV_, LN_, 2>), grid, dim3(64 * NW_), 0, stream, p); \
diff --git a/3m-asr-inference_amd/csrc/gemm_plan.hip b/3m-asr-inference_amd/csrc/gemm_plan.hip
--- a/3m-asr-inference_amd/csrc/gemm_plan.hip
+++ b/3m-asr-inference_amd/csrc/gemm_plan.hip
@@ -155,6 +155,15 @@
                     "gemm: acc_init is built for K1 = K / 2 = %d with the LayerNorm prologue on the A2 half (K1=%d K=%d)",
                     8 * plan.nw * gemm_group_steps(1, 1, plan.nw), p.K1, p.K);
   }
+  if (p.w_frag) {
+    M3_PLAN_REQUIRE(!p.w_bf16, "gemm: fragment-ordered weights are fp32-only");
+    M3_PLAN_REQUIRE(p.mode == GEMM_A_PLAIN, "gemm: fragment-ordered weights need plain A (no concat, no implicit conv)");
+    const int Nout = plan.glu ? p.N / 2 : p.N;
+    M3_PLAN_REQUIRE((Nout & 15) == 0 && (p.K & 15) == 0, "gemm: fragment-ordered weights need N%s=%d and K=%d to be multiples of 16",
+                    plan.glu ? " / 2" : "", Nout, p.K);
+    M3_PLAN_REQUIRE(plan.kernel == GemmKernel::SkinnyF32, "gemm: fragment-ordered weights need the skinny fp32 kernel; M=%d N=%d K=%d plans as %s",
+                    p.M, p.N, p.K, plan.label);
+  }
   return true;
 }
 
@@ -172,7 +181,8 @@
 GemmLaunch gemm_launch(const GemmParams& p, float* ws, size_t ws_bytes) { return GemmLaunch{p, plan_gemm(p, ws != nullptr ? ws_bytes : 0), ws}; }
 bool gemm_dual_fusable(const GemmLaunch& ga, const GemmLaunch& gb) {
   const GemmPlan &a = ga.plan, &b = gb.plan;
-  return a.launches == 1 && b.launches == 1 && a.dual_ok && b.dual_ok && a.nw == b.nw && a.ln == b.ln && a.glu == b.glu;
+  return a.launches == 1 && b.launches == 1 && a.dual_ok && b.dual_ok && a.nw == b.nw && a.ln == b.ln && a.glu == b.glu &&
+         !ga.p.w_frag == !gb.p.w_frag;
 }
 
 int launch_gemm(const GemmLaunch& g, hipStream_t stream) {
diff --git a/3m-asr-inference_amd/csrc/kernels.h b/3m-asr-inference_amd/csrc/kernels.h
--- a/3m-asr-inference_amd/csrc/kernels.h
+++ b/3m-asr-inference_amd/csrc/kernels.h
@@ -37,6 +37,7 @@
   const int32_t* conv_len = nullptr;
   int sig_col0 = -1;
   const float* acc_init = nullptr;
+  int w_frag = 0;
   int n_tiles = 0, m_tiles = 0, xcd_swizzle = 0;
 };
 enum { GEMM_LN_NONE = 0, GEMM_LN_EPI = 1, GEMM_LN_PRO = 2 };
@@ -130,6 +131,7 @@
 enum { EXPERT_NORM_IN_KERNEL = 1,
        EXPERT_SCATTER_ROWS = 2 };
 ExpertFfnPlan plan_expert_ffn(ExpertWeights w, int S, int E, int D, int F, unsigned flags = 0);
+enum { EXPERT_W_REF = 0, EXPERT_W2_SLICED = 1, EXPERT_W_FRAG = 2 };
 struct ExpertFfnArgs { const float* x; int ldx; const int32_t *pos, *acc_hist; const void *w1, *w2; const float *s1, *s2, *b1, *b2;
                        int w2_sliced; float h_scale; float* slab; const float *ln_gamma, *ln_beta; float ln_eps;
                        const void* xq; const float* xq_scale; int32_t* fs_dev; float* y_scatter; };
diff --git a/3m-asr-inference_amd/csrc/moe_expert.hip b/3m-asr-inference_amd/csrc/moe_expert.hip
--- a/3m-asr-inference_amd/csrc/moe_expert.hip
+++ b/3m-asr-inference_amd/csrc/moe_expert.hip
@@ -28,7 +28,7 @@
   return sw;
 }
 
-template <int MT, bool LNS, int RE = 0>
+template <int MT, bool LNS, int RE = 0, bool WF = false>
 __global__ __launch_bounds__(64 * (kExpertSlice / 16)) void expert_ffn_f32_kernel(const float* __restrict__ x, int ldx,
                                                              const int32_t* __restrict__ pos,
                                                              const int32_t* __restrict__ acc_hist, int S, int D,
@@ -55,7 +55,8 @@
   const int f0 = slice * kExpertSlice;
   const int ksteps1 = D >> 4;
 
-  const float* w1row = w1 + ((size_t)e * F + f0 + 16 * wave + col) * D + 4 * kq;
+  const float* w1row = WF ? w1 + (size_t)e * F * D + (size_t)((f0 >> 4) + wave) * ((size_t)D << 4) + 4 * lane
+                          : w1 + ((size_t)e * F + f0 + 16 * wave + col) * D + 4 * kq;
   const float bias1 = b1[(size_t)e * F + f0 + 16 * wave + col];
   const int nsub = D >> 4;
   const float* w2_slice = w2 + (size_t)e * D * F + (size_t)slice * w2_slice_stride;
@@ -72,15 +73,15 @@
 #pragma unroll
       for (int i = 0; i < 8; ++i) {
         const int s = min(8 * g + i, ksteps1 - 1);
-        wb[buf][i] = ldg4_w(w1row + (s << 4));
+        wb[buf][i] = ldg4_w(w1row + (s << (WF ? 8 : 4)));
       }
     } else {
 #pragma unroll
       for (int j = 0; j < SPG; ++j) {
         const int sub = min(wave + NWV * (SPG * (g - g1) + j), nsub - 1);
-        const float* p = w2_slice + (size_t)(16 * sub + col) * w2_row_stride + 4 * kq;
-#pragma unroll
-        for (int st = 0; st < KS2; ++st) wb[buf][KS2 * j + st] = ldg4_w(p + 16 * st);
+        const float* p = WF ? w2_slice + (size_t)sub * (KS2 * 256) + 4 * lane : w2_slice + (size_t)(16 * sub + col) * w2_row_stride + 4 * kq;
+#pragma unroll
+        for (int st = 0; st < KS2; ++st) wb[buf][KS2 * j + st] = ldg4_w(p + (WF ? 256 : 16) * st);
         if (RE > 0) bb[buf][j] = add_b2 ? rt.b2[(size_t)e * D + 16 * sub + col] : 0.f;
       }
     }
@@ -328,6 +329,10 @@
   M3_CHECK_HIP(hipFuncSetAttribute((const void*)expert_ffn_f32_kernel<4, false>, hipFuncAttributeMaxDynamicSharedMemorySize, 160 * 1024));
   M3_CHECK_HIP(hipFuncSetAttribute((const void*)expert_ffn_f32_kernel<2, true>, hipFuncAttributeMaxDynamicSharedMemorySize, 160 * 1024));
   M3_CHECK_HIP(hipFuncSetAttribute((const void*)expert_ffn_f32_kernel<4, true>, hipFuncAttributeMaxDynamicSharedMemorySize, 160 * 1024));
+  M3_CHECK_HIP(hipFuncSetAttribute((const void*)expert_ffn_f32_kernel<2, false, 0, true>, hipFuncAttributeMaxDynamicSharedMemorySize, 160 * 1024));
+  M3_CHECK_HIP(hipFuncSetAttribute((const void*)expert_ffn_f32_kernel<4, false, 0, true>, hipFuncAttributeMaxDynamicSharedMemorySize, 160 * 1024));
+  M3_CHECK_HIP(hipFuncSetAttribute((const void*)expert_ffn_f32_kernel<2, true, 0, true>, hipFuncAttributeMaxDynamicSharedMemorySize, 160 * 1024));
+  M3_CHECK_HIP(hipFuncSetAttribute((const void*)expert_ffn_f32_kernel<4, true, 0, true>, hipFuncAttributeMaxDynamicSharedMemorySize, 160 * 1024));
   once.mark();
   return 0;
 }
@@ -350,12 +355,16 @@
   dim3 grid(F / kExpertSlice, E, zt < 8 ? zt : 8);
   const int w2_row_stride = w2_sliced ? kExpertSlice : F;
   const int w2_slice_stride = w2_sliced ? D * kExpertSlice : kExpertSlice;
+  const bool wf = w2_sliced == EXPERT_W_FRAG;
+  M3_REQUIRE(!wf || (((uintptr_t)w1 | (uintptr_t)w2) & 15) == 0, "expert_ffn: fragment-ordered weights must be 16-byte aligned");
   if (int rc = init_expert_ffn_kernels()) return rc;
-#define M3_EXPERT_CASE2(MT_, LNS_)                                                                      \
-  hipLaunchKernelGGL((expert_ffn_f32_kernel<MT_, LNS_>), grid, dim3(64 * (kExpertSlice / 16)), lds_bytes, stream, x, ldx, pos,    \
+#define M3_EXPERT_CASE2(MT_, LNS_, WF_)                                                                      \
+  hipLaunchKernelGGL((expert_ffn_f32_kernel<MT_, LNS_, 0, WF_>), grid, dim3(64 * (kExpertSlice / 16)), lds_bytes, stream, x, ldx, pos,    \
                      acc_hist, S, D, F, w1, b1, w2, w2_row_stride, w2_slice_stride, slab, ln_gamma, ln_beta, ln_eps, ExpertRoute())
-#define M3_EXPERT_CASE(MT_) do { if (ln_gamma) M3_EXPERT_CASE2(MT_, true); else M3_EXPERT_CASE2(MT_, false); } while (0)
+#define M3_EXPERT_CASE3(MT_, WF_) do { if (ln_gamma) M3_EXPERT_CASE2(MT_, true, WF_); else M3_EXPERT_CASE2(MT_, false, WF_); } while (0)
+#define M3_EXPERT_CASE(MT_) do { if (wf) M3_EXPERT_CASE3(MT_, true); else M3_EXPERT_CASE3(MT_, false); } while (0)
   if (mt == 1) M3_EXPERT_CASE(1); else if (mt == 2) M3_EXPERT_CASE(2); else M3_EXPERT_CASE(4);
+#undef M3_EXPERT_CASE3
 #undef M3_EXPERT_CASE
 #undef M3_EXPERT_CASE2
   M3_LAUNCH_CHECK();
@@ -379,7 +388,9 @@
   if (!once.done()) {
 #define M3_ROUTE_ATTR(MT_, E_)                                                                                                                            \
   M3_CHECK_HIP(hipFuncSetAttribute((const void*)expert_ffn_f32_kernel<MT_, false, E_>, hipFuncAttributeMaxDynamicSharedMemorySize, 150 * 1024)); \
-  M3_CHECK_HIP(hipFuncSetAttribute((const void*)expert_ffn_f32_kernel<MT_, true, E_>, hipFuncAttributeMaxDynamicSharedMemorySize, 150 * 1024))
+  M3_CHECK_HIP(hipFuncSetAttribute((const void*)expert_ffn_f32_kernel<MT_, true, E_>, hipFuncAttributeMaxDynamicSharedMemorySize, 150 * 1024)); \
+  M3_CHECK_HIP(hipFuncSetAttribute((const void*)expert_ffn_f32_kernel<MT_, false, E_, true>, hipFuncAttributeMaxDynamicSharedMemorySize, 150 * 1024)); \
+  M3_CHECK_HIP(hipFuncSetAttribute((const void*)expert_ffn_f32_kernel<MT_, true, E_, true>, hipFuncAttributeMaxDynamicSharedMemorySize, 150 * 1024))
     M3_ROUTE_ATTR(2, 8); M3_ROUTE_ATTR(2, 16); M3_ROUTE_ATTR(2, 32); M3_ROUTE_ATTR(2, 64);
 #undef M3_ROUTE_ATTR
     once.mark();
@@ -391,16 +402,19 @@
   dim3 grid(F / kExpertSlice, E, 1);
   const int w2_row_stride = w2_sliced ? kExpertSlice : F;
   const int w2_slice_stride = w2_sliced ? D * kExpertSlice : kExpertSlice;
-#define M3_ROUTE_CASE(MT_, E_)                                                                                              \
+  const bool wf = w2_sliced == EXPERT_W_FRAG;
+  M3_REQUIRE(!wf || (((uintptr_t)w1 | (uintptr_t)w2) & 15) == 0, "expert_route_ffn: fragment-ordered weights must be 16-byte aligned");
+#define M3_ROUTE_CASE(MT_, E_, WF_)                                                                                         \
   do {                                                                                                                      \
     if (ln_gamma != nullptr)                                                                                                \
-      hipLaunchKernelGGL((expert_ffn_f32_kernel<MT_, true, E_>), grid, dim3(64 * (kExpertSlice / 16)), lds_bytes, stream, x, ldx, \
+      hipLaunchKernelGGL((expert_ffn_f32_kernel<MT_, true, E_, WF_>), grid, dim3(64 * (kExpertSlice / 16)), lds_bytes, stream, x, ldx, \
                          nullptr, nullptr, S, D, F, w1, b1, w2, w2_row_stride, w2_slice_stride, slab, ln_gamma, ln_beta, ln_eps, rt); \
     else                                                                                                                    \
-      hipLaunchKernelGGL((expert_ffn_f32_kernel<MT_, false, E_>), grid, dim3(64 * (kExpertSlice / 16)), lds_bytes, stream, x, ldx, \
+      hipLaunchKernelGGL((expert_ffn_f32_kernel<MT_, false, E_, WF_>), grid, dim3(64 * (kExpertSlice / 16)), lds_bytes, stream, x, ldx, \
                          nullptr, nullptr, S, D, F, w1, b1, w2, w2_row_stride, w2_slice_stride, slab, nullptr, nullptr, 0.f, rt); \
   } while (0)
-#define M3_ROUTE_E(E_) do { if (mt == 1) M3_ROUTE_CASE(1, E_); else M3_ROUTE_CASE(2, E_); } while (0)
+#define M3_ROUTE_MT(MT_, E_) do { if (wf) M3_ROUTE_CASE(MT_, E_, true); else M3_ROUTE_CASE(MT_, E_, false); } while (0)
+#define M3_ROUTE_E(E_) do { if (mt == 1) M3_ROUTE_MT(1, E_); else M3_ROUTE_MT(2, E_); } while (0)
   switch (E) {
     case 8: M3_ROUTE_E(8); break;
     case 16: M3_ROUTE_E(16); break;
@@ -408,6 +422,7 @@
     default: M3_ROUTE_E(64); break;
   }
 #undef M3_ROUTE_E
+#undef M3_ROUTE_MT
 #undef M3_ROUTE_CASE
   M3_LAUNCH_CHECK();
   return 0;
diff --git a/3m-asr-inference_amd/csrc/moe_expert_plan.hip b/3m-asr-inference_amd/csrc/moe_expert_plan.hip
--- a/3m-asr-inference_amd/csrc/moe_expert_plan.hip
+++ b/3m-asr-inference_amd/csrc/moe_expert_plan.hip
@@ -57,6 +57,8 @@
 int launch_expert_ffn(const ExpertFfnPlan& plan, int S, int E, int D, int F, const ExpertFfnArgs& a, hipStream_t stream) {
   M3_REQUIRE(a.ln_gamma == nullptr || plan.kernel == ExpertKernel::SlabF32, "expert_ffn: LayerNorm while gathering exists in the fp32 slab form only (S=%d E=%d)", S, E);
   M3_REQUIRE(a.y_scatter == nullptr || plan.kernel == ExpertKernel::TiledBf16, "expert_ffn: the scattering epilogue exists in the bf16 tiled form only (S=%d E=%d)", S, E);
+  M3_REQUIRE(a.w2_sliced != EXPERT_W_FRAG || plan.kernel == ExpertKernel::SlabF32,
+             "expert_ffn: fragment-ordered weights exist for the fp32 slab form only; S=%d E=%d D=%d F=%d runs %s", S, E, D, F, plan.label);
   char* const region = (char*)a.slab;
   void* const hbuf = region + plan.h_off;
   float* const ybuf = (float*)(region + plan.rows_off);
diff --git a/3m-asr-inference_amd/m3asr/_lib.py b/3m-asr-inference_amd/m3asr/_lib.py
--- a/3m-asr-inference_amd/m3asr/_lib.py
+++ b/3m-asr-inference_amd/m3asr/_lib.py
@@ -152,6 +152,8 @@
     "m3_moe_expert_workspace_size": (_sz, [_i, _i, _i, _i]),
     "m3_moe_expert_ffn": (_i, [_vp, _vp, _vp, _vp, _vp, _vp, _i, _i, _i, _i, _vp, _vp, _f, _vp, _vp, _f, _vp,
                                _vp, _sz, _vp]),
+    "m3_moe_expert_ffn_wfrag": (_i, [_vp, _vp, _vp, _vp, _vp, _vp, _i, _i, _i, _i, _vp, _vp, _f, _vp, _vp, _f, _vp,
+                                     _vp, _sz, _vp]),
     "m3_moe_expert_ffn_bf16": (_i, [_vp, _vp, _vp, _vp, _vp, _vp, _i, _i, _i, _i, _vp, _vp, _f, _vp, _vp, _f, _vp,
                                     _vp, _sz, _vp]),
     "m3_moe_expert_ffn_fp8": (_i, [_vp, _vp, _vp, _vp, _vp, _vp, _vp, _vp, _i, _i, _i, _i, _vp, _vp, _f, _vp, _vp, _f, _vp,
@@ -180,6 +182,10 @@
     "m3_linear_workspace_size": (_sz, [_P(LinearDesc)]),
     "m3_linear_kernel": (C.c_char_p, [_P(LinearDesc), _i]),
     "m3_linear_ws": (_i, [_P(LinearDesc), _vp, _sz, _vp]),
+    "m3_pack_wfrag_host": (_i, [_vp, _i, _i, _vp]),
+    "m3_linear_wfrag": (_i, [_P(LinearDesc), _vp]),
+    "m3_linear_wfrag_kernel": (C.c_char_p, [_P(LinearDesc)]),
+    "m3_linear_pair_wfrag": (_i, [_P(LinearDesc), _P(LinearDesc), _vp]),
     "m3_linear_pair": (_i, [_P(LinearDesc), _P(LinearDesc), _vp]),
     "m3_linear_ws_pair": (_i, [_P(LinearDesc), _vp, _sz, _P(LinearDesc), _vp, _sz, _i, _vp]),
     "m3_linear_pair_kernel": (C.c_char_p, [_P(LinearDesc), _P(LinearDesc), _i]),
diff --git a/3m-asr-inference_amd/m3asr/config.py b/3m-asr-inference_amd/m3asr/config.py
--- a/3m-asr-inference_amd/m3asr/config.py
+++ b/3m-asr-inference_amd/m3asr/config.py
@@ -34,8 +34,9 @@
     embed_conv_subsample_in_ch: int = 1
     delta_order: int = 0
     delta_window: int = 2
+    weights_frag: bool = True
 
-    _LATE_FIELDS = ("conv_subsample_in_ch", "embed_conv_subsample_in_ch", "delta_order", "delta_window")
+    _LATE_FIELDS = ("conv_subsample_in_ch", "embed_conv_subsample_in_ch", "delta_order", "delta_window", "weights_frag")
 
     def __post_init__(self):
         if not 0 <= self.delta_order <= 2:
diff --git a/3m-asr-inference_amd/m3asr/engine.py b/3m-asr-inference_amd/m3asr/engine.py
--- a/3m-asr-inference_amd/m3asr/engine.py
+++ b/3m-asr-inference_amd/m3asr/engine.py
@@ -1,4 +1,5 @@
 import collections
+import os
 import ctypes as C
 
 import torch
@@ -6,7 +7,7 @@
 from . import _lib
 from ._lib import check
 from .config import EncoderConfig, subsampled_len
-from .plan import pack_weights
+from .plan import add_frag_weights, pack_weights
 
 
 _TORCH_DTYPE = {torch.float32: _lib.F32, torch.bfloat16: _lib.BF16, torch.int32: _lib.I32, torch.float8_e4m3fn: _lib.FP8,
@@ -40,6 +41,9 @@
     return ec
 
 
+_W_FRAG_SWITCH = os.environ.get("M3_W_FRAG", "1") != "0"
+
+
 class Engine:
     def __init__(self, cfg: EncoderConfig, packed, device="cuda:0", fold_pos_proj=True, debug_taps=False,
                  fuse_route=False, bf16_activations=True, packed_rows=None, max_shapes=8, ep_stages=False, fork_embed=None):
@@ -51,6 +55,8 @@
         torch.cuda.set_device(self.device)
         self.weights = {k: (v if v.is_cuda else v.to(self.device, non_blocking=False)).contiguous() for k, v in packed.items()
                         if not k.startswith("decoder.")}
+        if _W_FRAG_SWITCH:
+            add_frag_weights(self.weights, cfg)
         names = [n for n in self.weights if not n.startswith("after_norm.")]
         table = (_lib.WeightEntry * len(names))()
         self._keep = [n.encode() for n in names]
diff --git a/3m-asr-inference_amd/m3asr/ops.py b/3m-asr-inference_amd/m3asr/ops.py
--- a/3m-asr-inference_amd/m3asr/ops.py
+++ b/3m-asr-inference_amd/m3asr/ops.py
@@ -104,7 +104,9 @@
     lib = _lib.load()
     assert w1.dtype == w2.dtype and w1.is_contiguous() and w2.is_contiguous()
     S, D = x.shape
-    E, F = w1.shape[0], w1.shape[1]
+    wfrag = w1.dim() == 6
+    assert not wfrag or (w1.dtype == torch.float32 and w2.dim() == 7)
+    E, F = w1.shape[0], w1.shape[1] * (16 if wfrag else 1)
     if workspace is None:
         workspace = torch.empty(max(moe_expert_workspace_size(S, E, D, F), 1), dtype=torch.uint8, device=x.device)
     y = out if out is not None else torch.empty_like(x)
@@ -136,6 +138,8 @@
               "m3_moe_expert_ffn_mxfp4")
     elif w1.dtype == torch.bfloat16:
         check(lib.m3_moe_expert_ffn_bf16(xi, gi, _p(w1), _f32(b1), _p(w2), _f32(b2), *tail), "m3_moe_expert_ffn_bf16")
+    elif wfrag:
+        check(lib.m3_moe_expert_ffn_wfrag(xi, gi, _f32(w1), _f32(b1), _f32(w2), _f32(b2), *tail), "m3_moe_expert_ffn_wfrag")
     else:
         check(lib.m3_moe_expert_ffn(xi, gi, _f32(w1), _f32(b1), _f32(w2), _f32(b2), *tail), "m3_moe_expert_ffn")
     return y
@@ -226,7 +230,9 @@
                          use_gate_value=True, resid=None, alpha=1.0, ln=None, workspace=None, out=None, taps=None):
     lib = _lib.load()
     S, D = x.shape
-    E, F = w1.shape[0], w1.shape[1]
+    wfrag = w1.dim() == 6
+    assert not wfrag or (w2.dim() == 7 and w2.is_contiguous())
+    E, F = w1.shape[0], w1.shape[1] * (16 if wfrag else 1)
     assert tuple(logits.shape) == (S, E) and w1.is_contiguous()
     if w2_sliced and w2.dim() == 3:
         from .plan import slice_major_w2
@@ -239,7 +245,7 @@
     g, b, eps = ln if ln is not None else (None, None, 0.0)
     taps, ptrs = _route_taps(S, E, x.device, taps)
     check(lib.m3_moe_route_expert_ffn(xp, ldx, _f32(logits), _i32(row_len), rows_per_batch, _f32(w1), _f32(b1), _f32(w2),
-                                      1 if w2_sliced else 0, _f32(b2), S, E, D, F, _f32(ng), _f32(nb), float(neps),
+                                      2 if wfrag else (1 if w2_sliced else 0), _f32(b2), S, E, D, F, _f32(ng), _f32(nb), float(neps),
                                       1 if use_gate_value else 0, _f32(resid), float(alpha), _f32(g), _f32(b), float(eps),
                                       *ptrs, _p(y), _p(workspace), workspace.numel() * workspace.element_size(), _stream()),
           "m3_moe_route_expert_ffn")
@@ -251,7 +257,12 @@
            copy_bf16=None, copy_stats=None, ln_stats=None, workspace=None, _kernel_only=False, _desc_only=False):
     lib = _lib.load()
     M, K1 = a.shape
-    N, K = w.shape
+    wfrag = w.dim() == 5
+    if wfrag:
+        assert tuple(w.shape[2:]) == (4, 16, 4) and w.dtype == torch.float32 and not split_k
+        N, K = 16 * w.shape[0], 16 * w.shape[1]
+    else:
+        N, K = w.shape
     n_out = N // 2 if act == _lib.ACT_GLU else N
     y = out if out is not None else torch.empty(M, n_out, dtype=out_dtype, device=a.device)
     for t in (a, a2, y, resid, copy_bf16):
@@ -296,8 +307,11 @@
     if _desc_only:
         return d, y
     if _kernel_only:
-        name = lib.m3_linear_kernel(C.byref(d), int(bool(split_k)))
+        name = lib.m3_linear_wfrag_kernel(C.byref(d)) if wfrag else lib.m3_linear_kernel(C.byref(d), int(bool(split_k)))
         return name.decode() if name else None
+    if wfrag:
+        check(lib.m3_linear_wfrag(C.byref(d), _stream()), "m3_linear_wfrag")
+        return y
     if split_k:
         need = lib.m3_linear_workspace_size(C.byref(d))
         ws = workspace if workspace is not None else torch.empty(max(need, 1), dtype=torch.uint8, device=a.device)
@@ -323,7 +337,10 @@
 
 def linear_pair(a, b):
     (da, ya), (db, yb) = _linear_desc(a), _linear_desc(b)
-    check(_lib.load().m3_linear_pair(C.byref(da), C.byref(db), _stream()), "m3_linear_pair")
+    nfrag = (a["w"].dim() == 5) + (b["w"].dim() == 5)
+    assert nfrag != 1, "linear_pair: the two problems must agree on the weight layout"
+    fn = "m3_linear_pair_wfrag" if nfrag else "m3_linear_pair"
+    check(getattr(_lib.load(), fn)(C.byref(da), C.byref(db), _stream()), fn)
     return ya, yb
 
 
diff --git a/3m-asr-inference_amd/m3asr/plan.py b/3m-asr-inference_amd/m3asr/plan.py
--- a/3m-asr-inference_amd/m3asr/plan.py
+++ b/3m-asr-inference_amd/m3asr/plan.py
@@ -25,6 +25,48 @@
 def slice_major_w2(t):
     E_, D_, F_ = t.shape
     return t.reshape(E_, D_, F_ // EXPERT_SLICE, EXPERT_SLICE).permute(0, 2, 1, 3).contiguous()
+
+
+def pack_wfrag(t):
+    *lead, N_, K_ = t.shape
+    assert N_ % 16 == 0 and K_ % 16 == 0, "pack_wfrag: N=%d and K=%d must be multiples of 16" % (N_, K_)
+    n = len(lead)
+    v = t.reshape(*lead, N_ // 16, 16, K_ // 16, 4, 4)
+    return v.permute(*range(n), n, n + 2, n + 3, n + 1, n + 4).contiguous()
+
+
+def unpack_wfrag(t):
+    *lead, nt, ns, kq, col, j = t.shape
+    assert (kq, col, j) == (4, 16, 4)
+    n = len(lead)
+    return t.permute(*range(n), n, n + 3, n + 1, n + 2, n + 4).reshape(*lead, nt * 16, ns * 16).contiguous()
+
+
+_FRAG_DENSE = ("feed_forward_macaron.w_1.ln.weight", "feed_forward_macaron.w_2.weight", "self_attn.qkv.ln.weight",
+               "self_attn.linear_out.weight", "conv_module.pointwise_conv1.ln.weight", "conv_module.pointwise_conv2.weight",
+               "feed_forward.w_1.ln.weight", "feed_forward.w_2.weight")
+
+
+def add_frag_weights(weights, cfg: EncoderConfig):
+    if not getattr(cfg, "weights_frag", True) or cfg.weight_dtype != "f32" or cfg.attention_dim < 256:
+        return []
+    added = []
+    for name in list(weights):
+        if not (name.startswith("blocks.") or name.startswith("embed.blocks.")):
+            continue
+        w, dst = weights[name], None
+        if w.dtype != torch.float32:
+            continue
+        if name.endswith(_FRAG_DENSE) and w.dim() == 2 and w.shape[0] % 16 == 0 and w.shape[1] % 16 == 0:
+            dst = name + "_frag"
+        elif name.endswith("feed_forward.experts.w_1.weight") and w.dim() == 3 and w.shape[1] % 16 == 0 and w.shape[2] % 16 == 0:
+            dst = name + "_frag"
+        elif name.endswith("feed_forward.experts.w_2.weight_sliced") and w.dim() == 4 and w.shape[2] % 16 == 0 and w.shape[3] % 16 == 0:
+            dst = name[:-len("_sliced")] + "_frag"
+        if dst is not None and dst not in weights:
+            weights[dst] = pack_wfrag(w)
+            added.append(dst)
+    return added
 
 
 def _pack_subsampling(sd, p, out):
@@ -327,6 +369,7 @@
 
 
 def save_plan(path, cfg: EncoderConfig, packed, extra=None):
+    packed = {k: v for k, v in packed.items() if not k.endswith("_frag")}
     index, off = {}, 0
     for k, v in packed.items():
         name = _DTYPE_NAME[v.dtype]
diff --git a/include/m3asr.h b/include/m3asr.h
--- a/include/m3asr.h
+++ b/include/m3asr.h
@@ -70,6 +70,11 @@
                       const float* gate_value, const float* resid, float alpha, const float* ln_gamma,
                       const float* ln_beta, float ln_eps, float* y, void* workspace, size_t workspace_bytes,
                       m3_stream stream);
+int m3_moe_expert_ffn_wfrag(const float* x, const int32_t* gate_idx, const float* w1, const float* b1,
+                            const float* w2, const float* b2, int S, int num_expert, int idim, int hidden_units,
+                            const float* gate_value, const float* resid, float alpha, const float* ln_gamma,
+                            const float* ln_beta, float ln_eps, float* y, void* workspace, size_t workspace_bytes,
+                            m3_stream stream);
 int m3_moe_expert_ffn_bf16(const float* x, const int32_t* gate_idx, const void* w1, const float* b1,
                            const void* w2, const float* b2, int S, int num_expert, int idim, int hidden_units,
                            const float* gate_value, const float* resid, float alpha, const float* ln_gamma,
@@ -155,6 +160,10 @@
 size_t m3_linear_workspace_size(const m3_linear_desc* desc);
 const char* m3_linear_kernel(const m3_linear_desc* desc, int with_workspace);
 int m3_linear_ws(const m3_linear_desc* desc, void* workspace, size_t workspace_bytes, m3_stream stream);
+int m3_pack_wfrag_host(const float* w, int N, int K, float* wf);
+int m3_linear_wfrag(const m3_linear_desc* desc, m3_stream stream);
+const char* m3_linear_wfrag_kernel(const m3_linear_desc* desc);
+int m3_linear_pair_wfrag(const m3_linear_desc* a, const m3_linear_desc* b, m3_stream stream);
 
 int m3_layer_norm(const float* x, const float* gamma, const float* beta, float eps, float* y, int rows, int dim,
                   m3_stream stream);
```
